# huggingface/open-muse

Hardware: AMD Instinct MI355X
Metric: images/sec/node (MaskGit train step, 256^2, bs=64/GPU) (higher is better)
Workload: dtype bf16 (transformer GEMM/attention operands; f32 accumulate, residual, norms, loss) + bf16x3 tokenizer (f32 activations, f32-class products as 3 bf16 MFMAs); parity of this mode was not measured in this run (a --full run measures it); 1 GPU; MaskGit train step: MaskGitVQGAN f16-256 encode (bf16x3) + cosine mask + MaskGitTransformer config B (configs/imagenet.yaml: hidden 768, 24 layers, 16 heads, vocab 2048, seq 257) fwd+bwd (bf16 MFMA, f32 accum/residual) + AdamW; global_batch=64, per_gpu_batch=64, resolution=256, seq_len=257, parallelism=dp1, vqgan_dtype=bf16x3, random_init=True, wgrad_stream=True

## Files before the change

include/muse_hip.h:

```cpp
#ifndef MUSE_HIP_H
#define MUSE_HIP_H
#include <stdint.h>

#ifdef __cplusplus
extern "C" {
#endif

enum { MUSE_F32 = 0, MUSE_BF16 = 1, MUSE_F16 = 2  };
enum { MUSE_ERR_BAD_ARG = -1, MUSE_ERR_ALIGN = -2, MUSE_ERR_UNSUPPORTED = -3 };

int muse_version(void);

typedef struct muse_gemm_desc {
  const void* A;
  const void* B;
  void* C;
  const void* bias;
  const void* rowvec;
  const void* residual;
  int32_t dtype;
  int32_t out_dtype;
  int32_t layout_a, layout_b;
  int32_t M, N, K;
  int32_t batch, zdiv;
// ... 44 lines not shown
  const void* v;
  void* o;
  int64_t ldq, ldk, ldv, ldo;
  int64_t bsq, bsk, bsv, bso;
  int32_t batch, heads, head_dim, seq_q, seq_kv;
  float alpha;
} muse_attn_desc;
int muse_attention_seq_pad(int32_t seq);
int muse_attention_fwd_ex(const muse_attn_desc* d, float* lse, void* stream);
int muse_attention_bwd_ex(const muse_attn_desc* d, const void* d_o, int64_t lddo, int64_t bsdo, const float* lse, float* dsum,
                          void* dq, int64_t lddq, int64_t bsdq, void* dk, int64_t lddk, int64_t bsdk, void* dv, int64_t lddv,
                          int64_t bsdv, void* stream);
int muse_attention_x3_fwd(const muse_attn_desc* d, float* lse, void* o_planes, int64_t o_lo, int32_t half, float scale, int32_t* stats,
                          void* stream);
int muse_attention_x3_bwd(const muse_attn_desc* d, const void* d_o, int64_t lddo, int64_t bsdo, const float* lse, void* dq,
                          int64_t lddq, int64_t bsdq, void* dk, int64_t lddk, int64_t bsdk, void* dv, int64_t lddv, int64_t bsdv,
                          void* dq_planes, int64_t dq_lo, void* dk_planes, int64_t dk_lo, void* dv_planes, int64_t dv_lo, int32_t half,
                          float scale, int32_t* stats, void* stream);
int muse_attention_x3_fwd_stream(const muse_attn_desc* d, float* lse, void* o_planes, int64_t o_lo, int32_t half, float scale,
                                 int32_t* stats, void* stream);
int muse_attention_x3_bwd_stream(const muse_attn_desc* d, const float* d_o, int64_t lddo, int64_t bsdo, const float* lse, float* dsum,
                                 float* dq, int64_t lddq, int64_t bsdq, float* dk, int64_t lddk, int64_t bsdk, float* dv, int64_t lddv,
                                 int64_t bsdv, void* dq_planes, int64_t dq_lo, void* dk_planes, int64_t dk_lo, void* dv_planes, int64_t dv_lo,
                                 int32_t half, float scale, int32_t* stats, void* stream);
int muse_attention_x3_merge(const float* part, int64_t part_stride, const float* lp, int64_t lp_stride, int32_t nk, float* out, float* lse,
                            void* out_planes, int64_t out_lo, int32_t batch, int32_t seq, int32_t heads, int32_t half, float scale,
                            int32_t* stats, void* stream);
int muse_sum_parts_strided(const float* parts, int64_t part_stride, int32_t n, int64_t rows, int32_t cols, float* out, int64_t ldo,
                           int32_t accumulate, void* stream);
int muse_attention_fwd(const void* qkv, void* ctx, float* lse, int32_t batch, int32_t seq, int32_t heads,
                       int32_t head_dim, float alpha, void* stream);
int muse_attention_bwd(const void* qkv, const void* ctx, const void* dctx, const float* lse, float* dsum, void* dqkv,
                       int32_t batch, int32_t seq, int32_t heads, int32_t head_dim, float alpha, void* stream);

int muse_glu_fwd(const void* ab, void* h, int32_t dtype, int64_t rows, int32_t inter, void* stream);
int muse_glu_bwd(const void* ab, const void* dh, void* dab, int32_t dtype, int64_t rows, int32_t inter, void* stream);
int muse_glu_fwd_x3(const float* ab, float* h, void* planes, int64_t rows, int32_t inter, int32_t half, float scale, int32_t* stats,
                    void* stream);
int muse_glu_bwd_x3(const float* ab, const float* dh, float* dab, void* planes, int64_t rows, int32_t inter, int32_t half, float scale,
                    int32_t* stats, void* stream);
int muse_ffn_mid_rows_per_block(void);
int muse_ffn_mid_fwd(const void* ab, const float* w, void* h, void* hm, float* mean, float* rstd, int32_t dtype,
                     int32_t rows, int32_t inter, float eps, void* stream);
int muse_ffn_mid_bwd(const void* dhm, const void* h, const void* ab, const float* w, const float* mean, const float* rstd,
                     void* dab, float* dw_partial, int32_t dtype, int32_t rows, int32_t inter, void* stream);
int muse_gelu_fwd(const void* x, void* y, int32_t dtype, int64_t n, void* stream);
int muse_gelu_bwd(const void* x, const void* dy, void* dx, int32_t dtype, int64_t n, void* stream);
int muse_gelu_bwd_f32_bf16(const float* x, const float* dy, void* dx_bf16, int64_t n, void* stream);

int muse_embed_fwd(const int64_t* ids, const float* word, const float* pos, float* out, int32_t batch, int32_t seq,
                   int32_t hidden, int32_t vocab, void* stream);
int muse_embed_bwd(const int64_t* ids, const float* dout, float* dword, float* dpos, float* scratch, int32_t batch,
                   int32_t seq, int32_t hidden, int32_t vocab, int32_t accumulate, void* stream);
int64_t muse_embed_bwd_scratch_floats(int32_t hidden, int32_t vocab);
int muse_embed_bwd2(const int64_t* ids, const float* dout, float* dword, float* dpos, void* scratch, int64_t scratch_bytes,
                    int32_t batch, int32_t seq, int32_t hidden, int32_t vocab, int32_t accumulate, void* stream);
int64_t muse_embed_bwd2_scratch_bytes(int32_t batch, int32_t seq, int32_t hidden, int32_t vocab);

int muse_cross_entropy_fwd(const void* logits, int32_t dtype, const int64_t* labels, float* row_loss, float* lse,
                           float* loss_out, int64_t rows, int32_t vocab, int64_t ld, float label_smoothing, void* stream);
int muse_cross_entropy_bwd(const void* logits, int32_t dtype, const int64_t* labels, const float* lse,
                           const float* loss_out, const float* grad_out, void* dlogits, int32_t dl_dtype, int64_t rows,
                           int32_t vocab, int64_t ld, float label_smoothing, void* stream);
int muse_soft_ce_fwd(const float* logits, const int64_t* labels, const float* soft, float* row_loss, float* lse, float* psum,
                     float* loss_out, int64_t rows, int32_t seq1, int32_t K, int64_t ld, void* stream);
int muse_soft_ce_bwd(const float* logits, const int64_t* labels, const float* soft, const float* lse, const float* psum,
                     const float* loss_out, const float* grad_out, void* dlogits, int32_t dl_dtype, int64_t rows, int32_t seq1,
                     int32_t K, int64_t ld, int64_t ldo, void* stream);

int muse_adamw_flat(float* p, const float* g, float* m, float* v, void* p_bf16, int64_t n, float lr, float beta1,
                    float beta2, float eps, float weight_decay, int32_t step, float grad_scale, const int32_t* skip, void* stream);
int muse_ema_multi(const int64_t* table, const int32_t* chunk_first, int32_t num_tensors, int32_t num_chunks, float one_minus_decay,
                   void* stream);
int muse_adamw_multi(const int64_t* table, const int32_t* chunk_first, int32_t num_tensors, int32_t num_chunks, float lr,
                     float beta1, float beta2, float eps, float weight_decay, int32_t step, float grad_scale, const int32_t* skip,
                     void* stream);
int muse_adamw_flat_groups(float* p, const float* g, float* m, float* v, void* p_bf16, int64_t n, int64_t base,
                           const int64_t* seg_end, const int32_t* seg_group, int32_t nseg, const float* group_hyper,
                           int32_t ngroups, int32_t step, float grad_scale, const int32_t* skip, void* stream);
int muse_adamw_multi_groups(const int64_t* table, const int32_t* chunk_first, int32_t num_tensors, int32_t num_chunks,
                            const float* group_hyper, int32_t ngroups, int32_t step, float grad_scale, const int32_t* skip, void* stream);

int muse_gradnorm_flat(const float* g_flat, int64_t base, int64_t n, const int64_t* ptab_host, const int32_t* chunk_first_host,
                       const int64_t* ptab, const int32_t* chunk_first, int32_t num_params, double* slab, void* stream);
int muse_gradnorm_multi(const int64_t* table, int32_t ncol, const int32_t* chunk_first, int32_t num_tensors, int32_t num_chunks,
                        double* slab, void* stream);
int muse_gradnorm_finalize(const double* slab, const int32_t* chunk_first, int32_t num_tensors, double* psum, float grad_scale,
                           float max_norm, float* out, void* stream);
int muse_grad_scale_flat(float* g, int64_t n, const float* scale, void* stream);
int muse_grad_scale_multi(const int64_t* table, int32_t ncol, const int32_t* chunk_first, int32_t num_tensors, int32_t num_chunks,
                          const float* scale, void* stream);
int muse_adamw_flat_dev(float* p, const float* g, float* m, float* v, void* p_bf16, int64_t n, float lr, float beta1, float beta2,
                        float eps, float weight_decay, int32_t step, const float* scale_dev, const int32_t* skip, void* stream);
int muse_adamw_multi_dev(const int64_t* table, const int32_t* chunk_first, int32_t num_tensors, int32_t num_chunks, float lr,
                         float beta1, float beta2, float eps, float weight_decay, int32_t step, const float* scale_dev,
                         const int32_t* skip, void* stream);
int muse_adamw_flat_groups_dev(float* p, const float* g, float* m, float* v, void* p_bf16, int64_t n, int64_t base,
                               const int64_t* seg_end, const int32_t* seg_group, int32_t nseg, const float* group_hyper,
                               int32_t ngroups, int32_t step, const float* scale_dev, const int32_t* skip, void* stream);
int muse_adamw_multi_groups_dev(const int64_t* table, const int32_t* chunk_first, int32_t num_tensors, int32_t num_chunks,
                                const float* group_hyper, int32_t ngroups, int32_t step, const float* scale_dev, const int32_t* skip,
                                void* stream);
int muse_sum_slices(const float* ws, float* out, int32_t nslices, int64_t n, int64_t stride, int32_t accumulate, void* stream);
int muse_sum_multi(const void* const* ws, void* const* out, const int32_t* nslices, const int64_t* n, const int64_t* stride,
                   const int32_t* accumulate, const int32_t* kind, int32_t njobs, void* stream);
int muse_split_f32_to_bf16x2(const float* in, void* hi, void* lo, int64_t n, void* stream);
int muse_sum_slices_epilogue(const float* ws, int32_t nslices, int64_t stride, const float* bias, const void* residual, int64_t ldr,
                             void* out, int32_t out_dtype, int64_t ldc, int64_t rows, int32_t cols, void* stream);
int muse_split_f32_to_bf16_cat3(const float* in, void* out, int64_t rows, int32_t cols, int64_t ld_in, int64_t ld_out, int32_t mode,
                                int32_t lo_pos, void* stream);
int muse_cast_f32_to_bf16(const float* in, void* out, int64_t n, void* stream);
int muse_cast_f32_to_f16(const float* in, void* out, int64_t n, float scale, int32_t* stats, void* stream);
int muse_cast_bf16_to_f32(const void* in, float* out, int64_t n, void* stream);

int muse_mask_sample(const int64_t* tokens, const int64_t* class_ids, const float* timesteps, const float* noise,
                     int64_t* input_ids, int64_t* labels, float* mask_prob, int32_t batch, int32_t seq, int64_t mask_id,
                     int64_t codebook_size, float min_masking_rate, void* stream);

int muse_sample_step(const float* cond_logits, const float* uncond_logits, float guidance_scale, int64_t img_stride, int64_t ld,
                     int32_t vocab,
                     const int64_t* input_ids, int64_t mask_id, const float* noise_exp, const float* noise_u, uint64_t seed,
                     uint32_t step, float temperature, int32_t sched_mask_len, int32_t batch, int32_t seq, int64_t* raw_sampled,
                     int64_t* sampled, int64_t* next_ids, float* conf_scratch, void* stream);

int muse_mask_tokens(const int64_t* tokens, const float* timesteps, const float* mask_prob_in, const float* noise,
                     const int32_t* rects, int64_t* input_ids, int64_t* labels, float* loss_weight, float* mask_prob,
                     int32_t batch, int32_t seq, int64_t mask_id, float min_masking_rate, int32_t all_labels, float weight_min,
                     void* stream);

int muse_dropout(const void* x, void* y, int32_t dtype, int64_t n, float p, uint64_t seed, uint64_t offset, void* stream);

int muse_cond_dropout(const float* x, const float* empty, const float* uniforms, float* out, int32_t batch, int64_t per_image,
                      float prob, void* stream);


int muse_conv2d_nhwc(const void* in, const void* weight, const float* bias, const void* residual, void* out,
                     int32_t dtype, int32_t batch, int32_t H, int32_t W, int32_t Cin, int32_t Cout, int32_t KS,
                     int32_t upsample, void* stream);
int muse_conv2d_nhwc_split(const float* in, const void* w_hi, const void* w_lo, const float* bias, const float* residual,
                           float* out, double* gn_partial, int32_t gn_groups, int32_t batch, int32_t H, int32_t W,
                           int32_t Cin, int32_t Cout, int32_t KS, int32_t upsample, void* stream);
int muse_conv2d_nhwc_split2(const void* in_hi, const void* in_lo, const void* w_hi, const void* w_lo, const float* bias,
                            const float* residual, float* out, double* gn_partial, int32_t gn_groups, int32_t batch,
                            int32_t H, int32_t W, int32_t Cin, int32_t Cout, int32_t KS, void* stream);
int muse_groupnorm_silu_nhwc(const void* x, void* y, int32_t dtype, const float* gamma, const float* beta,
                             double* partial, int32_t batch, int32_t HW, int32_t C, int32_t groups, float eps,
                             int32_t apply_silu, void* stream);
int muse_groupnorm_nchunk(int32_t HW);
int muse_conv2d_nhwc_gn_split2_ok(int32_t batch, int32_t H, int32_t W, int32_t Cin, int32_t Cout, int32_t KS);
int muse_conv2d_nhwc_gn_split2(const float* x, const float* gn_scale, const float* gn_shift, const void* w_hi, const void* w_lo,
                               const float* bias, const float* residual, float* out, double* gn_partial, int32_t gn_groups,
                               int32_t batch, int32_t H, int32_t W, int32_t Cin, int32_t Cout, int32_t KS, int32_t persistent,
                               void* stream);
int muse_groupnorm_scale_shift(const double* partial, int32_t nchunk, const float* gamma, const float* beta, float* scale,
                               float* shift, int32_t batch, int32_t HW, int32_t C, int32_t groups, float eps, void* stream);
int muse_conv_in_direct(const float* x, const float* w4, const float* bias, float* out, double* gn_partial, int32_t gn_groups,
                        int32_t batch, int32_t H, int32_t W, int32_t Cin, int32_t Cpad, int32_t Cout, void* stream);
int muse_conv_out_direct(const float* x, const float* scale, const float* shift, const float* w, const float* bias, float* out,
                         int32_t batch, int32_t H, int32_t W, int32_t C, int32_t Cout, void* stream);
int muse_upsample2x_nhwc(const void* x, void* y, int32_t dtype, int32_t batch, int32_t H, int32_t W, int32_t C, void* stream);
int muse_upsample2x_split_nhwc(const float* x, void* y_hi, void* y_lo, int32_t batch, int32_t H, int32_t W, int32_t C, void* stream);
int muse_groupnorm_silu_nhwc_split(const float* x, void* y_hi, void* y_lo, const float* gamma, const float* beta,
                                   double* partial, int32_t stats_nchunk, int32_t batch, int32_t HW, int32_t C,
                                   int32_t groups, float eps, int32_t apply_silu, void* stream);
int muse_avgpool2x2_nhwc(const void* x, void* y, int32_t dtype, int32_t batch, int32_t H, int32_t W, int32_t C,
                         void* stream);
int muse_avgpool2x2_nhwc_stats(const float* x, float* y, double* partial, int32_t groups, int32_t batch, int32_t H, int32_t W,
                               int32_t C, void* stream);
int muse_nchw_to_nhwc(const float* in, void* out, int32_t out_dtype, int32_t batch, int32_t C, int32_t HW, int32_t Cpad,
                      void* stream);
int muse_nhwc_to_nchw(const void* in, int32_t in_dtype, float* out, int32_t batch, int32_t C, int32_t HW, int32_t Cpad,
                      void* stream);
int muse_argmin_rows(const float* dist, int64_t* idx, int64_t rows, int32_t ncodes, int64_t ld, void* stream);
int muse_row_sumsq(const float* x, float* out, int64_t rows, int32_t cols, int64_t ld, void* stream);
int muse_gather_rows(const float* table, const int64_t* idx, void* out, int32_t out_dtype, int64_t rows, int32_t cols,
                     void* stream);

int muse_probe_tr16(const int32_t* addr, int32_t* out, void* stream);

int muse_norm_res_fwd(const float* x, const float* res, const float* w, float* y, float* pre, int64_t rows, int32_t cols,
                      float eps, int32_t mode, void* stream);
int muse_adaln_fwd(const float* x, const float* ss, float* y, int32_t batch, int64_t rows_per_batch, int32_t C, void* stream);
int muse_adaln_fwd_ex(const float* x, const float* ss, float* y, void* y_bf16, int32_t batch, int64_t rows_per_batch, int32_t C,
                      void* stream);
int muse_silu_fwd(const float* x, float* y, int64_t n, void* stream);
int muse_dwconv3x3_nhwc(const float* x, const float* w, float* y, int32_t batch, int32_t H, int32_t W, int32_t C, void* stream);
int muse_space_to_depth2_nhwc(const float* x, float* y, int32_t batch, int32_t H, int32_t W, int32_t C, int32_t inverse, void* stream);
int muse_grn_fwd(const float* x, const float* gamma, const float* beta, float* y, float* scratch, int32_t batch, int64_t S,
                 int32_t C, void* stream);
int muse_grn_fwd_ex(const float* x, const float* gamma, const float* beta, float* y, void* y_bf16, float* scratch, int32_t batch,
                    int64_t S, int32_t C, void* stream);
int muse_sinusoidal_encode(const float* f, float* out, int64_t n, int32_t dim, float max_positions, void* stream);
int muse_weighted_mean(const float* v, const float* w, float* out, int64_t n, void* stream);
int muse_norm_res_bwd_nblk(int64_t rows);
int muse_norm_res_bwd(const float* dy, const float* dpre, const float* v, const float* w, float* dv, float* dw_partial,
                      int64_t rows, int32_t cols, float eps, int32_t mode, void* stream);
int muse_norm_res_bwd_ex(const float* dy, const float* dpre, const float* v, const float* w, float* dv, void* dv_bf16,
                         float* dw_partial, int64_t rows, int32_t cols, float eps, int32_t mode, void* stream);
int muse_norm_adaln_fwd(const float* x, const float* res, const float* w, const float* ss, float* pre, float* m, void* m_bf16,
                        int32_t batch, int64_t rows_per_batch, int32_t cols, float eps, int32_t mode, void* stream);
int muse_norm_adaln_bwd(const float* dm, const float* dpre, const float* v, const float* w, const float* ss, float* dv, void* dv_bf16,
                        float* dw_partial, float* dss_partial, int32_t batch, int64_t rows_per_batch, int32_t cols, float eps,
                        int32_t mode, void* stream);
int muse_norm_adaln_fwd_x3(const float* x, const float* res, const float* w, const float* ss, float* pre, float* m, void* planes,
                           int32_t batch, int64_t rows_per_batch, int32_t cols, float eps, int32_t mode, int32_t half, float scale,
                           int32_t* stats, void* stream);
int muse_norm_adaln_bwd_x3(const float* dm, const float* dpre, const float* v, const float* w, const float* ss, float* dv, void* planes,
                           float* dw_partial, float* dss_partial, int32_t batch, int64_t rows_per_batch, int32_t cols, float eps,
                           int32_t mode, int32_t half, float scale, int32_t* stats, void* stream);
int muse_colsum_segments(const float* part, float* out, int32_t nseg, int32_t seg_rows, int32_t cols, void* stream);
int muse_adaln_bwd(const float* dy, const float* x, const float* ss, float* dx, float* dss, int32_t batch,
                   int64_t rows_per_batch, int32_t C, void* stream);
int muse_silu_bwd(const float* x, const float* dy, float* dx, int64_t n, void* stream);
int muse_dwconv3x3_bwd_nchunk(int64_t pixels);
int muse_dwconv3x3_bwd(const float* dy, const float* x, const float* w, float* dx, float* dw_partial, int32_t batch, int32_t H,
                       int32_t W, int32_t C, void* stream);
int muse_grn_bwd(const float* dy, const float* x, const float* gamma, const float* stats, float* dx, float* work,
                 int32_t batch, int64_t S, int32_t C, void* stream);
int muse_scale_rows(float* x, const float* w, const float* num, const float* den, int64_t rows, int32_t cols, int64_t ld,
                    void* stream);

#ifdef __cplusplus
}
#endif
#endif
```

open-muse_amd/csrc/conv_dma.hip:

```cpp
#include "gemm256.h"
#include "../../include/muse_hip.h"

namespace cdma {
using g256::lds_read128;
using g256::lds_void_t;

constexpr int BM = 256, BN = 128, BK = 32, NT = 512, MI = 4, NI = 4, NSTAGE = 3;
constexpr int AH = 0, AL = 16384, BH = 32768, BL = 40960, STAGE = 49152, LDS_BYTES = NSTAGE * STAGE;

struct Params {
  const bf16_t *xh, *xl, *wh, *wl;
  const float* bias;
  const float* residual;
  float* out;
  double* gn_partial;
  int gn_cpg, gn_groups;
  int M, N, K, H, W, Cin;
  const float *xf, *gsc, *gsh;
};

__device__ __forceinline__ int sw4(int q) { return (4 - q) & 3; }

struct Frag16 { bf16x8 ah[MI], al[MI], bh[NI], bl[NI]; };

// ... 100 lines not shown
#endif
#ifndef CDMA_ABLATE_NO_DMA
#define CDMA_ISSUE(S, Q)                             \
  if constexpr ((Q) == 0) issue_a((S) * STAGE, 0);   \
  if constexpr ((Q) == 1) issue_a((S) * STAGE, 1);   \
  if constexpr ((Q) == 2) issue_b((S) * STAGE);
#define CDMA_TOP_WAIT "s_waitcnt vmcnt(6) lgkmcnt(0)"
#else
#define CDMA_ISSUE(S, Q)
#define CDMA_TOP_WAIT "s_waitcnt vmcnt(0) lgkmcnt(0)"
#endif
#define CDMA_SLOT(CUR, NXT, S, SN, Q)                          \
  CDMA_PAIR(CUR, Q)                                            \
  __builtin_amdgcn_sched_barrier(0);                           \
  CDMA_ISSUE(S, Q)                                             \
  CDMA_READ(NXT, SN, Q)                                        \
  __builtin_amdgcn_sched_barrier(0);
#define CDMA_TILE(CUR, NXT, S, SN)                                                     \
  asm volatile(CDMA_TOP_WAIT ::: "memory");                                            \
  __builtin_amdgcn_s_barrier();                                                        \
  __builtin_amdgcn_sched_barrier(0);                                                   \
  CDMA_SLOT(CUR, NXT, S, SN, 0) CDMA_SLOT(CUR, NXT, S, SN, 1) CDMA_SLOT(CUR, NXT, S, SN, 2) CDMA_SLOT(CUR, NXT, S, SN, 3)     \
  CDMA_SLOT(CUR, NXT, S, SN, 4) CDMA_SLOT(CUR, NXT, S, SN, 5) CDMA_SLOT(CUR, NXT, S, SN, 6) CDMA_SLOT(CUR, NXT, S, SN, 7)     \
  CDMA_SLOT(CUR, NXT, S, SN, 8) CDMA_SLOT(CUR, NXT, S, SN, 9) CDMA_SLOT(CUR, NXT, S, SN, 10) CDMA_SLOT(CUR, NXT, S, SN, 11)   \
  CDMA_SLOT(CUR, NXT, S, SN, 12) CDMA_SLOT(CUR, NXT, S, SN, 13) CDMA_SLOT(CUR, NXT, S, SN, 14) CDMA_SLOT(CUR, NXT, S, SN, 15)

  issue_a(0 * STAGE, 0); issue_a(0 * STAGE, 1); issue_b(0 * STAGE);
  issue_a(1 * STAGE, 0); issue_a(1 * STAGE, 1); issue_b(1 * STAGE);
  issue_a(2 * STAGE, 0); issue_a(2 * STAGE, 1); issue_b(2 * STAGE);
  asm volatile("s_waitcnt vmcnt(12)" ::: "memory");
  __builtin_amdgcn_s_barrier();
  __builtin_amdgcn_sched_barrier(0);
  CDMA_READ(f0, 0, 0) CDMA_READ(f0, 0, 1) CDMA_READ(f0, 0, 2) CDMA_READ(f0, 0, 3)
  CDMA_READ(f0, 0, 4) CDMA_READ(f0, 0, 5) CDMA_READ(f0, 0, 6) CDMA_READ(f0, 0, 7)
  CDMA_READ(f0, 0, 8) CDMA_READ(f0, 0, 9) CDMA_READ(f0, 0, 10) CDMA_READ(f0, 0, 11)
  CDMA_READ(f0, 0, 12) CDMA_READ(f0, 0, 13) CDMA_READ(f0, 0, 14) CDMA_READ(f0, 0, 15)
  __builtin_amdgcn_sched_barrier(0);

  const int nkt = (p.K + BK - 1) / BK, ngroups = (nkt + 5) / 6;
  for (int grp = 0; grp < ngroups; ++grp) {
    CDMA_TILE(f0, f1, 0, 1)
    CDMA_TILE(f1, f0, 1, 2)
    CDMA_TILE(f0, f1, 2, 0)
    CDMA_TILE(f1, f0, 0, 1)
    CDMA_TILE(f0, f1, 1, 2)
    CDMA_TILE(f1, f0, 2, 0)
  }
#undef CDMA_TILE
#undef CDMA_ISSUE
#undef CDMA_TOP_WAIT
#undef CDMA_SLOT
#undef CDMA_PAIR
#undef CDMA_READ
  asm volatile("s_waitcnt vmcnt(0) lgkmcnt(0)" ::: "memory");
  __builtin_amdgcn_sched_barrier(0);

  constexpr int CST = BN * 4 + 16;
  float bias_v[NI][4];
#pragma unroll
  for (int j = 0; j < NI; ++j)
#pragma unroll
    for (int r = 0; r < 4; ++r) {
      const int n = n0 + wn * 64 + j * 16 + 4 * (lane >> 4) + r;
      bias_v[j][r] = (p.bias && n < p.N) ? p.bias[n] : 0.f;
    }
  double gs = 0.0, gq = 0.0;
  __syncthreads();
#pragma unroll
  for (int i = 0; i < MI; ++i) {
    const int lr = wm * 64 + i * 16 + (lane & 15);
#pragma unroll
    for (int j = 0; j < NI; ++j) {
      const int nl = wn * 64 + j * 16 + 4 * (lane >> 4);
      const f32x4 v = {acc[i][j][0] + bias_v[j][0], acc[i][j][1] + bias_v[j][1], acc[i][j][2] + bias_v[j][2], acc[i][j][3] + bias_v[j][3]};
      *(f32x4*)(smem + lr * CST + nl * 4) = v;
    }
  }
  __syncthreads();
  constexpr int NIT = (BM * 32) / NT;
  const int col = (threadIdx.x & 31) * 4, n = n0 + col, rbase = threadIdx.x >> 5;
  if (n < p.N) {
    f32x4 rv[NIT];
    if (p.residual) {
#pragma unroll
      for (int it = 0; it < NIT; ++it) {
        const int m = m0 + rbase + 16 * it;
        rv[it] = m < p.M ? *(const f32x4*)(p.residual + (long)m * p.N + n) : f32x4{0.f, 0.f, 0.f, 0.f};
      }
    }
#pragma unroll
    for (int it = 0; it < NIT; ++it) {
      const int row = rbase + 16 * it, m = m0 + row;
      if (m < p.M) {
        f32x4 w = *(const f32x4*)(smem + row * CST + col * 4);
        if (p.residual) w += rv[it];
        *(f32x4*)(p.out + (long)m * p.N + n) = w;
        if (p.gn_partial) {
#pragma unroll
          for (int e = 0; e < 4; ++e) { gs += (double)w[e]; gq += (double)w[e] * (double)w[e]; }
        }
      }
    }
  }
  if (p.gn_partial) {
    gs += __shfl_xor(gs, 32, 64);
    gq += __shfl_xor(gq, 32, 64);
    __syncthreads();
    double* red = (double*)smem;
    if (lane < 32) { red[(wave * 32 + lane) * 2] = gs; red[(wave * 32 + lane) * 2 + 1] = gq; }
    __syncthreads();
    if (threadIdx.x < 32) {
      double cs = 0.0, cq = 0.0;
#pragma unroll
      for (int w8 = 0; w8 < 8; ++w8) { cs += red[(w8 * 32 + threadIdx.x) * 2]; cq += red[(w8 * 32 + threadIdx.x) * 2 + 1]; }
      const int cpc = p.gn_cpg >> 2;
      for (int o = 1; o < cpc; o <<= 1) { cs += __shfl_xor(cs, o, 64); cq += __shfl_xor(cq, o, 64); }
      const int n = n0 + (int)threadIdx.x * 4;
      if ((threadIdx.x & (cpc - 1)) == 0 && n < p.N) {
        const int hw = p.H * p.W, b = m0 / hw, chunk = (m0 - b * hw) >> 8, nchunk = hw >> 8;
        double* o2 = p.gn_partial + (((long)b * nchunk + chunk) * p.gn_groups + n / p.gn_cpg) * 2;
        o2[0] = cs; o2[1] = cq;
      }
    }
  }
}

}


namespace cslab {
using g256::lds_read128;
using g256::lds_void_t;
using cdma::Params;
using cdma::sw4;

constexpr int BM = 256, BN = 128, NT = 512, MI = 4, NI = 4;
constexpr int PLANE = 21 * 1024;
constexpr int SLAB = 2 * PLANE;
constexpr int B_BASE = 2 * SLAB, BSTAGE = 16384;
constexpr int CST = BN * 4 + 16;
constexpr int LDS_BYTES = BM * CST;
static_assert(B_BASE + 3 * BSTAGE <= LDS_BYTES, "LDS map");

struct Frag16 { bf16x8 ah[MI], al[MI], bh[NI], bl[NI]; };

#ifdef CDMA_TIMESTAMPS
__device__ long* g_conv_ts = nullptr;
#define CDMA_TS(IDX) if (g_conv_ts && threadIdx.x == 0) g_conv_ts[(long)blockIdx.x * 8 + (IDX)] = (long)__builtin_amdgcn_s_memtime();
#define CDMA_TSV(V, IDX) if (g_conv_ts && threadIdx.x == 0) g_conv_ts[(long)(V) * 8 + (IDX)] = (long)__builtin_amdgcn_s_memtime();
#else
#define CDMA_TS(IDX)
#define CDMA_TSV(V, IDX)
#endif
template <bool GN>
__global__ __launch_bounds__(512, 2) void conv_slab_kernel(Params p) {
  extern __shared__ __attribute__((aligned(16))) unsigned char smem[];
  CDMA_TS(0)
  const int H = p.H, W = p.W, Cin = p.Cin;
  const int tpr = W >> 4, tpi = (H >> 4) * tpr;
  const int ntm = p.M >> 8, ntn = (p.N + BN - 1) / BN, ntiles = ntm * ntn;
  const int bq = ntiles >> 3, br = ntiles & 7, xcd = blockIdx.x & 7, bi = blockIdx.x >> 3;
  const int tid_ = (xcd < br ? xcd * (bq + 1) : br * (bq + 1) + (xcd - br) * bq) + bi;
  const int mt = tid_ / ntn, n0 = (tid_ % ntn) * BN;
  const int img = mt / tpi, prem = mt - img * tpi, ty = prem / tpr, tx = prem - ty * tpr;
  const int y0 = ty << 4, x0 = tx << 4;

  const int lane = threadIdx.x & 63, wave = __builtin_amdgcn_readfirstlane(threadIdx.x >> 6);
  const int wm = wave >> 1, wn = wave & 1;

  constexpr int XE = GN ? 4 : 2;
  const unsigned bytesA = (unsigned)((long)p.M * Cin * XE);
  const rsrc_t rs_xh = make_rsrc(GN ? (const void*)p.xf : (const void*)p.xh, bytesA), rs_xl = make_rsrc(GN ? (const void*)p.xf : (const void*)p.xl, bytesA);
  const unsigned oobA = (bytesA + 15u) & ~15u;
  unsigned slab_off[3];
  int slab_piece[3];
  const int srcchunk = (lane & 3) ^ (((lane >> 4) & 1) << 1);
  {
#pragma unroll
    for (int k = 0; k < 3; ++k) {
      int piece = wave + 8 * k;
      if (piece > 20) piece -= 8;
      slab_piece[k] = piece;
      const int r = piece * 16 + (lane >> 2), sy = r / 18, sx = r - sy * 18;
      const int y = y0 - 1 + sy, x = x0 - 1 + sx;
      const bool ok = r < 324 && y >= 0 && y < H && x >= 0 && x < W;
      slab_off[k] = ok ? (unsigned)(((((long)img * H + y) * W + x) * Cin + srcchunk * 8) * XE) : oobA;
    }
  }
  float* const gss = (float*)(smem + LDS_BYTES);
  if constexpr (GN) {
    for (int c = threadIdx.x; c < Cin; c += NT) { gss[c] = p.gsc[(long)img * Cin + c]; gss[Cin + c] = p.gsh[(long)img * Cin + c]; }
    __syncthreads();
  }
  u32x4 xr[2];
  float scv[4], shv[4];
  auto issue_slab_f = [&](u32x4 (&r)[2], int k, int chunk) {
    const unsigned vo = chunk * 32 < Cin ? slab_off[k] : oobA;
    r[0] = buf_load16(rs_xh, vo, (unsigned)(chunk * 128));
    r[1] = buf_load16(rs_xh, vo + 16u, (unsigned)(chunk * 128));
  };
  auto load_gss = [&](int chunk, int h) {
    const float* q = gss + chunk * 32 + srcchunk * 8 + h * 4;
#pragma unroll
#ifndef GNX_CONST_SS
    for (int j = 0; j < 4; ++j) { scv[j] = q[j]; shv[j] = q[Cin + j]; }
#else
    for (int j = 0; j < 4; ++j) { scv[j] = 1.25f; shv[j] = 0.125f; }
    (void)q;
#endif
  };
  auto xform_elem = [&](u32x4 (&r)[2], int e) {
    float t = fmaf(__uint_as_float(r[e >> 2][e & 3]), scv[e & 3], shv[e & 3]);
#ifndef GNX_NO_SILU
    t = gn_silu(t);
#endif
    asm volatile("" : "+v"(t));
    r[e >> 2][e & 3] = __float_as_uint(t);
  };
  auto store_slab_f = [&](u32x4 (&r)[2], int buf, int k) {
    u32x4 hi4, lo4;
#pragma unroll
    for (int h = 0; h < 2; ++h) {
      u32x2 hi, lo;
      split4(r[h], hi, lo);
      hi4[2 * h] = hi[0]; hi4[2 * h + 1] = hi[1];
      lo4[2 * h] = lo[0]; lo4[2 * h + 1] = lo[1];
    }
    if (slab_off[k] == oobA) { hi4 = u32x4{0u, 0u, 0u, 0u}; lo4 = hi4; }
    unsigned char* dst = smem + buf * SLAB + slab_piece[k] * 1024 + lane * 16;
    *(u32x4*)dst = hi4;
    *(u32x4*)(dst + PLANE) = lo4;
  };

  auto issue_slab = [&](int buf, int k, int chunk) {
    const unsigned vo = chunk * 32 < Cin ? slab_off[k] : oobA;
    const int soff = chunk * 64;
    unsigned char* dst = smem + buf * SLAB + slab_piece[k] * 1024;
    __builtin_amdgcn_raw_ptr_buffer_load_lds(rs_xh, (lds_void_t*)dst, 16, (int)vo, soff, 0, 0);
    __builtin_amdgcn_raw_ptr_buffer_load_lds(rs_xl, (lds_void_t*)(dst + PLANE), 16, (int)vo, soff, 0, 0);
  };

  const int wimg = wave >> 2;
  const unsigned bytesB = (unsigned)((long)p.N * p.K * 2);
  const rsrc_t rs_w = make_rsrc(wimg ? p.wl : p.wh, bytesB);
  const unsigned oobB = (bytesB + 15u) & ~15u;
  unsigned voffB[2];
  {
    const int srcchunk = (lane & 3) ^ sw4((lane >> 4) & 3);
#pragma unroll
    for (int j = 0; j < 2; ++j) {
      const int n = n0 + ((wave & 3) * 2 + j) * 16 + (lane >> 2);
      voffB[j] = n < p.N ? (unsigned)(((long)n * p.K + srcchunk * 8) * 2) : oobB;
    }
  }
  auto issue_b = [&](int stage, int chunk, int tap) {
    const bool ok = chunk * 32 < Cin;
    const int soff = (tap * Cin + chunk * 32) * 2;
#pragma unroll
    for (int j = 0; j < 2; ++j)
      __builtin_amdgcn_raw_ptr_buffer_load_lds(rs_w, (lds_void_t*)(smem + B_BASE + stage * BSTAGE + wimg * 8192 + ((wave & 3) * 2 + j) * 1024),
                                               16, (int)(ok ? voffB[j] : oobB), soff, 0, 0);
  };

  unsigned baseA[4][2], addrB;
  {
    const int pr = lane & 15, g = lane >> 4, P = 72 * wm + pr;
#pragma unroll
    for (int e = 0; e < 4; ++e)
#pragma unroll
      for (int b = 0; b < 2; ++b) {
        const int bit2 = ((P >> 2) & 1) ^ (((P & 3) + e) >> 2) ^ b;
        baseA[e][b] = (unsigned)((P << 6) | ((g << 4) ^ (bit2 << 5)));
      }
    addrB = (unsigned)(B_BASE + (wn * 64 + pr) * 64 + ((g ^ sw4((pr >> 2) & 3)) << 4));
  }

  auto flip_base = [&](int d) {
#pragma unroll
    for (int e = 0; e < 4; ++e) { baseA[e][0] += d; baseA[e][1] += d; }
  };

  f32x4 acc[MI][NI];
#pragma unroll
  for (int i = 0; i < MI; ++i)
#pragma unroll
    for (int j = 0; j < NI; ++j) acc[i][j] = f32x4{0.f, 0.f, 0.f, 0.f};
  Frag16 f0, f1;

#define SLAB_CP(TAP, I) (((I) + (TAP) / 3) * 18 + (TAP) % 3)
#define SLAB_READ(F, ST, TAP, Q)                                                                                             \
  {                                                                                                                               \
    constexpr int q_ = (Q) & 3;                                                                                                   \
    constexpr int cp_ = SLAB_CP(TAP, q_);                                                                                         \
    if constexpr ((Q) < 4) lds_read128<cp_ * 64>(F.ah[q_], baseA[cp_ & 3][(cp_ >> 2) & 1]);                                       \
    else if constexpr ((Q) < 8) lds_read128<PLANE + cp_ * 64>(F.al[q_], baseA[cp_ & 3][(cp_ >> 2) & 1]);                          \
    else if constexpr ((Q) < 12) lds_read128<(ST) * BSTAGE + q_ * 1024>(F.bh[q_], addrB);                                         \
    else lds_read128<(ST) * BSTAGE + 8192 + q_ * 1024>(F.bl[q_], addrB);                                                          \
  }
#if defined(CDMA_TWO_PRODUCTS)
#define SLAB_PAIR(F, Q)                                                                                                        \
  {                                                                                                                            \
    constexpr int i_ = (Q) >> 2, j_ = (Q) & 3;                                                                                 \
    if constexpr (CDMA_TWO_PRODUCTS == 1) acc[i_][j_] = __builtin_amdgcn_mfma_f32_16x16x32_bf16(F.bh[j_], F.al[i_], acc[i_][j_], 0, 0, 0);   \
    else acc[i_][j_] = __builtin_amdgcn_mfma_f32_16x16x32_bf16(F.bl[j_], F.ah[i_], acc[i_][j_], 0, 0, 0);                        \
    acc[i_][j_] = __builtin_amdgcn_mfma_f32_16x16x32_bf16(F.bh[j_], F.ah[i_], acc[i_][j_], 0, 0, 0);                            \
  }
#elif !defined(CDMA_ABLATE_NO_MFMA)
#define SLAB_PAIR(F, Q)                                                                                                        \
  {                                                                                                                            \
    constexpr int i_ = (Q) >> 2, j_ = (Q) & 3;                                                                                 \
    acc[i_][j_] = __builtin_amdgcn_mfma_f32_16x16x32_bf16(F.bl[j_], F.ah[i_], acc[i_][j_], 0, 0, 0);                            \
    acc[i_][j_] = __builtin_amdgcn_mfma_f32_16x16x32_bf16(F.bh[j_], F.al[i_], acc[i_][j_], 0, 0, 0);                            \
    acc[i_][j_] = __builtin_amdgcn_mfma_f32_16x16x32_bf16(F.bh[j_], F.ah[i_], acc[i_][j_], 0, 0, 0);                            \
  }
#else
#define SLAB_PAIR(F, Q) asm volatile("" ::"v"(F.ah[(Q) >> 2]), "v"(F.al[(Q) >> 2]), "v"(F.bh[(Q) & 3]), "v"(F.bl[(Q) & 3]));
#endif
#ifndef CDMA_ABLATE_NO_DMA
#define SLAB_ISSUE(T, Q)                                                                          \
  if constexpr (!GN && (Q) == 0 && ((T) % 9) < 3) issue_slab(1 - (T) / 9, (T) % 9, chunk0 + (T) / 9 + 1);  \
  if constexpr (GN && (Q) == 0 && ((T) % 9) == 0) issue_slab_f(xr, 0, chunk0 + (T) / 9 + 1);           \
  if constexpr (GN && (Q) == 12 && (((T) % 9) == 2 || ((T) % 9) == 4)) issue_slab_f(xr, ((T) % 9) / 2, chunk0 + (T) / 9 + 1);  \
  if constexpr ((Q) == 2) issue_b(((T) + 3) % 3, chunk0 + ((T) + 3) / 9, ((T) + 3) % 9);
#define SLAB_XF(T, Q)                                                                             \
  if constexpr (GN && ((T) % 9) >= 2 && ((T) % 9) <= 6 && ((T) % 9) % 2 == 0) {                    \
    constexpr int k_ = ((T) % 9) / 2 - 1;                                                         \
    if constexpr ((Q) == 1) load_gss(chunk0 + (T) / 9 + 1, 0);                                    \
    if constexpr ((Q) >= 2 && (Q) < 6) xform_elem(xr, (Q) - 2);                                   \
    if constexpr ((Q) == 6) load_gss(chunk0 + (T) / 9 + 1, 1);                                    \
    if constexpr ((Q) >= 7 && (Q) < 11) xform_elem(xr, (Q) - 3);                                  \
    if constexpr ((Q) == 11) store_slab_f(xr, 1 - (T) / 9, k_);                                   \
  }
#else
#define SLAB_ISSUE(T, Q)
#define SLAB_XF(T, Q)
#endif
#define SLAB_SLOT(CUR, NXT, T, Q)                                                   \
  SLAB_PAIR(CUR, Q)                                                                 \
  __builtin_amdgcn_sched_barrier(0);                                                \
  SLAB_ISSUE(T, Q)                                                                  \
  SLAB_READ(NXT, (((T) + 1) % 3), (((T) + 1) % 9), Q)                               \
  SLAB_XF(T, Q)                                                                     \
  __builtin_amdgcn_sched_barrier(0);
#ifndef CDMA_ABLATE_NO_DMA
#define SLAB_WAIT(T)                                                                     \
  if constexpr (GN ? (((T) % 9) == 1 || (((T) % 9) >= 3 && ((T) % 9) <= 6)) : (((T) % 9) >= 1 && ((T) % 9) <= 3))  \
    asm volatile("s_waitcnt vmcnt(4) lgkmcnt(0)" ::: "memory");                          \
  else asm volatile("s_waitcnt vmcnt(2) lgkmcnt(0)" ::: "memory");
#else
#define SLAB_WAIT(T) asm volatile("s_waitcnt vmcnt(0) lgkmcnt(0)" ::: "memory");
#endif
#define SLAB_TAP(CUR, NXT, T)                                                                         \
  SLAB_WAIT(T)                                                                                        \
  __builtin_amdgcn_s_barrier();                                                                       \
  if constexpr ((T) == 8) flip_base(SLAB);                                                            \
  if constexpr ((T) == 17) flip_base(-SLAB);                                                          \
  __builtin_amdgcn_sched_barrier(0);                                                                  \
  SLAB_SLOT(CUR, NXT, T, 0) SLAB_SLOT(CUR, NXT, T, 1) SLAB_SLOT(CUR, NXT, T, 2) SLAB_SLOT(CUR, NXT, T, 3)     \
  SLAB_SLOT(CUR, NXT, T, 4) SLAB_SLOT(CUR, NXT, T, 5) SLAB_SLOT(CUR, NXT, T, 6) SLAB_SLOT(CUR, NXT, T, 7)     \
  SLAB_SLOT(CUR, NXT, T, 8) SLAB_SLOT(CUR, NXT, T, 9) SLAB_SLOT(CUR, NXT, T, 10) SLAB_SLOT(CUR, NXT, T, 11)   \
  SLAB_SLOT(CUR, NXT, T, 12) SLAB_SLOT(CUR, NXT, T, 13) SLAB_SLOT(CUR, NXT, T, 14) SLAB_SLOT(CUR, NXT, T, 15)

  int chunk0 = 0;
  u32x4 pr[GN ? 3 : 1][2];
  if constexpr (GN) { issue_slab_f(pr[0], 0, 0); issue_slab_f(pr[GN ? 1 : 0], 1, 0); issue_slab_f(pr[GN ? 2 : 0], 2, 0); }
  else { issue_slab(0, 0, 0); issue_slab(0, 1, 0); issue_slab(0, 2, 0); }
  issue_b(0, 0, 0); issue_b(1, 0, 1); issue_b(2, 0, 2);
  CDMA_TS(1)
  if constexpr (GN) {
#pragma unroll
    for (int h = 0; h < 2; ++h) {
      load_gss(0, h);
#pragma unroll
      for (int k = 0; k < 3; ++k)
#pragma unroll
        for (int e = 0; e < 4; ++e) xform_elem(pr[GN ? k : 0], h * 4 + e);
    }
#pragma unroll
    for (int k = 0; k < 3; ++k) store_slab_f(pr[GN ? k : 0], 0, k);
  }
  asm volatile("s_waitcnt vmcnt(4) lgkmcnt(0)" ::: "memory");
  __builtin_amdgcn_s_barrier();
  __builtin_amdgcn_sched_barrier(0);
  CDMA_TS(2)
  SLAB_READ(f0, 0, 0, 0) SLAB_READ(f0, 0, 0, 1) SLAB_READ(f0, 0, 0, 2) SLAB_READ(f0, 0, 0, 3)
  SLAB_READ(f0, 0, 0, 4) SLAB_READ(f0, 0, 0, 5) SLAB_READ(f0, 0, 0, 6) SLAB_READ(f0, 0, 0, 7)
  SLAB_READ(f0, 0, 0, 8) SLAB_READ(f0, 0, 0, 9) SLAB_READ(f0, 0, 0, 10) SLAB_READ(f0, 0, 0, 11)
  SLAB_READ(f0, 0, 0, 12) SLAB_READ(f0, 0, 0, 13) SLAB_READ(f0, 0, 0, 14) SLAB_READ(f0, 0, 0, 15)
  __builtin_amdgcn_sched_barrier(0);

  const int nchunks = Cin >> 5;
  for (; chunk0 < nchunks; chunk0 += 2) {
    SLAB_TAP(f0, f1, 0) SLAB_TAP(f1, f0, 1) SLAB_TAP(f0, f1, 2) SLAB_TAP(f1, f0, 3) SLAB_TAP(f0, f1, 4) SLAB_TAP(f1, f0, 5)
    SLAB_TAP(f0, f1, 6) SLAB_TAP(f1, f0, 7) SLAB_TAP(f0, f1, 8) SLAB_TAP(f1, f0, 9) SLAB_TAP(f0, f1, 10) SLAB_TAP(f1, f0, 11)
    SLAB_TAP(f0, f1, 12) SLAB_TAP(f1, f0, 13) SLAB_TAP(f0, f1, 14) SLAB_TAP(f1, f0, 15) SLAB_TAP(f0, f1, 16) SLAB_TAP(f1, f0, 17)
  }
#undef SLAB_TAP
#undef SLAB_WAIT
#undef SLAB_SLOT
#undef SLAB_XF
#undef SLAB_ISSUE
#undef SLAB_PAIR
#undef SLAB_READ
#undef SLAB_CP
  asm volatile("s_waitcnt vmcnt(0) lgkmcnt(0)" ::: "memory");
  __builtin_amdgcn_sched_barrier(0);
  CDMA_TS(3)

  float bias_v[NI][4];
#pragma unroll
  for (int j = 0; j < NI; ++j)
#pragma unroll
    for (int r = 0; r < 4; ++r) {
      const int n = n0 + wn * 64 + j * 16 + 4 * (lane >> 4) + r;
      bias_v[j][r] = (p.bias && n < p.N) ? p.bias[n] : 0.f;
    }
  double gs = 0.0, gq = 0.0;
  __syncthreads();
#pragma unroll
  for (int i = 0; i < MI; ++i) {
    const int lr = wm * 64 + i * 16 + (lane & 15);
#pragma unroll
    for (int j = 0; j < NI; ++j) {
      const int nl = wn * 64 + j * 16 + 4 * (lane >> 4);
      const f32x4 v = {acc[i][j][0] + bias_v[j][0], acc[i][j][1] + bias_v[j][1], acc[i][j][2] + bias_v[j][2], acc[i][j][3] + bias_v[j][3]};
      *(f32x4*)(smem + lr * CST + nl * 4) = v;
    }
  }
  __syncthreads();
  CDMA_TS(4)
  constexpr int NIT = (BM * 32) / NT;
  const int col = (threadIdx.x & 31) * 4, n = n0 + col, rbase = threadIdx.x >> 5;
  const long pix0 = ((long)img * H + y0) * W + x0 + rbase;
  if (n < p.N) {
    f32x4 rv[NIT];
    if (p.residual) {
#pragma unroll
      for (int it = 0; it < NIT; ++it) rv[it] = *(const f32x4*)(p.residual + (pix0 + (long)it * W) * p.N + n);
    }
#pragma unroll
    for (int it = 0; it < NIT; ++it) {
      f32x4 w = *(const f32x4*)(smem + (rbase + 16 * it) * CST + col * 4);
      if (p.residual) w += rv[it];
#ifndef CDMA_ABLATE_NO_STORE
      *(f32x4*)(p.out + (pix0 + (long)it * W) * p.N + n) = w;
#else
      if (w[0] == 123.456f) p.out[0] = w[1];
#endif
      if (p.gn_partial) {
#pragma unroll
        for (int e = 0; e < 4; ++e) { gs += (double)w[e]; gq += (double)w[e] * (double)w[e]; }
      }
    }
  }
  if (p.gn_partial) {
    gs += __shfl_xor(gs, 32, 64);
    gq += __shfl_xor(gq, 32, 64);
    __syncthreads();
    double* red = (double*)smem;
    if (lane < 32) { red[(wave * 32 + lane) * 2] = gs; red[(wave * 32 + lane) * 2 + 1] = gq; }
    __syncthreads();
    if (threadIdx.x < 32) {
      double cs = 0.0, cq = 0.0;
#pragma unroll
      for (int w8 = 0; w8 < 8; ++w8) { cs += red[(w8 * 32 + threadIdx.x) * 2]; cq += red[(w8 * 32 + threadIdx.x) * 2 + 1]; }
      const int cpc = p.gn_cpg >> 2;
      for (int o = 1; o < cpc; o <<= 1) { cs += __shfl_xor(cs, o, 64); cq += __shfl_xor(cq, o, 64); }
      const int nn = n0 + (int)threadIdx.x * 4;
      if ((threadIdx.x & (cpc - 1)) == 0 && nn < p.N) {
        double* o2 = p.gn_partial + (((long)img * tpi + prem) * p.gn_groups + nn / p.gn_cpg) * 2;
        o2[0] = cs; o2[1] = cq;
      }
    }
  }
  CDMA_TS(5)
}


constexpr int P_BUF1 = 92160, P_BBASE = 43008, P_STAGING = P_BUF1, P_HALF_ROWS = 128;
constexpr int P_LDS_BYTES = P_STAGING + P_HALF_ROWS * CST;
constexpr int P_GSS = P_LDS_BYTES, P_GSS_MAX_CIN = 256, P_LDS_BYTES_GN = P_LDS_BYTES + 2 * 2 * P_GSS_MAX_CIN * 4;
__host__ __device__ constexpr int p_stage_off(int st) { return st == 0 ? 32768 : (st - 1) * 16384; }
static_assert(P_BBASE + 3 * BSTAGE == P_BUF1 && P_BUF1 + SLAB <= P_LDS_BYTES && P_LDS_BYTES_GN <= 163840, "LDS map");

template <bool GN>
__global__ __launch_bounds__(512, 2) void conv_slab_persist_kernel(Params p) {
  extern __shared__ __attribute__((aligned(16))) unsigned char smem[];
  const int H = p.H, W = p.W, Cin = p.Cin;
  const int tpr = W >> 4, tpi = (H >> 4) * tpr;
  const int ntm = p.M >> 8, ntn = (p.N + BN - 1) / BN, ntiles = ntm * ntn;
  const int bq = ntiles >> 3, br = ntiles & 7;
  const int nblocks = gridDim.x;

  const int lane = threadIdx.x & 63, wave = __builtin_amdgcn_readfirstlane(threadIdx.x >> 6);
  const int wm = wave >> 1, wn = wave & 1;

  constexpr int XE = GN ? 4 : 2;
  const unsigned bytesA = (unsigned)((long)p.M * Cin * XE);
  const rsrc_t rs_xh = make_rsrc(GN ? (const void*)p.xf : (const void*)p.xh, bytesA), rs_xl = make_rsrc(GN ? (const void*)p.xf : (const void*)p.xl, bytesA);
  const unsigned oobA = (bytesA + 15u) & ~15u;
  const int wimg = wave >> 2;
  const unsigned bytesB = (unsigned)((long)p.N * p.K * 2);
  const rsrc_t rs_w = make_rsrc(wimg ? p.wl : p.wh, bytesB);
  const unsigned oobB = (bytesB + 15u) & ~15u;
  const int nchunks = Cin >> 5;
  const unsigned bytesO = (unsigned)((long)p.M * p.N * 4);
  const rsrc_t rs_out = make_rsrc(p.out, bytesO), rs_res = make_rsrc(p.residual ? (const void*)p.residual : (const void*)p.out, bytesO);

  int slab_piece[3];
#pragma unroll
  for (int k = 0; k < 3; ++k) { int piece = wave + 8 * k; if (piece > 20) piece -= 8; slab_piece[k] = piece; }
  const int srcchunkA = (lane & 3) ^ (((lane >> 4) & 1) << 1);

  struct Geo { int img, prem, y0, x0, n0; };
  auto geo_of = [&](int v) {
    const int xcd = v & 7, bi = v >> 3;
    const int tid_ = (xcd < br ? xcd * (bq + 1) : br * (bq + 1) + (xcd - br) * bq) + bi;
    const int mt = tid_ / ntn;
    Geo g;
    g.n0 = (tid_ - mt * ntn) * BN;
    g.img = mt / tpi; g.prem = mt - g.img * tpi;
    const int ty = g.prem / tpr, tx = g.prem - ty * tpr;
    g.y0 = ty << 4; g.x0 = tx << 4;
    return g;
  };
  auto offsets_of = [&](const Geo& g, bool valid, unsigned (&so)[3], unsigned (&vb)[2], int ln) {
    const int srcchunkA = (ln & 3) ^ (((ln >> 4) & 1) << 1);
    const int srcchunkB = (ln & 3) ^ sw4((ln >> 4) & 3);
#pragma unroll
    for (int k = 0; k < 3; ++k) {
      const int r = slab_piece[k] * 16 + (ln >> 2), sy = r / 18, sx = r - sy * 18;
      const int y = g.y0 - 1 + sy, x = g.x0 - 1 + sx;
      const bool ok = valid && r < 324 && y >= 0 && y < H && x >= 0 && x < W;
      so[k] = ok ? (unsigned)(((((long)g.img * H + y) * W + x) * Cin + srcchunkA * 8) * XE) : oobA;
    }
#pragma unroll
    for (int j = 0; j < 2; ++j) {
      const int n = g.n0 + ((wave & 3) * 2 + j) * 16 + (ln >> 2);
      vb[j] = (valid && n < p.N) ? (unsigned)(((long)n * p.K + srcchunkB * 8) * 2) : oobB;
    }
  };

  unsigned slab_off[3], voffB[2], slab_off_n[3], voffB_n[2];
  auto issue_slab = [&](int buf, int k, int chunk) {
    const bool cur = chunk < nchunks;
    const unsigned vo = cur ? slab_off[k] : slab_off_n[k];
    const int soff = cur ? chunk * 64 : 0;
    unsigned char* dst = smem + (buf ? P_BUF1 : 0) + slab_piece[k] * 1024;
    __builtin_amdgcn_raw_ptr_buffer_load_lds(rs_xh, (lds_void_t*)dst, 16, (int)vo, soff, 0, 0);
    __builtin_amdgcn_raw_ptr_buffer_load_lds(rs_xl, (lds_void_t*)(dst + PLANE), 16, (int)vo, soff, 0, 0);
  };
  auto issue_b = [&](int stage_off, int chunk, int tap) {
    const bool cur = chunk < nchunks;
    const int soff = (tap * Cin + (cur ? chunk * 32 : 0)) * 2;
#pragma unroll
    for (int j = 0; j < 2; ++j)
      __builtin_amdgcn_raw_ptr_buffer_load_lds(rs_w, (lds_void_t*)(smem + P_BBASE + stage_off + wimg * 8192 + ((wave & 3) * 2 + j) * 1024),
                                               16, (int)(cur ? voffB[j] : voffB_n[j]), soff, 0, 0);
  };

  float* gss_cur = (float*)(smem + P_GSS);
  float* gss_nxt = gss_cur + 2 * P_GSS_MAX_CIN;
  u32x4 xr[2];
  float scv[4], shv[4];
  auto issue_slab_f = [&](u32x4 (&r)[2], int k, int chunk) {
    const bool cur = chunk < nchunks;
    const unsigned vo = cur ? slab_off[k] : slab_off_n[k];
    const unsigned soff = cur ? (unsigned)(chunk * 128) : 0u;
    r[0] = buf_load16(rs_xh, vo, soff);
    r[1] = buf_load16(rs_xh, vo + 16u, soff);
  };
  auto load_gss = [&](int chunk, int h) {
    const float* q = (chunk < nchunks ? gss_cur + chunk * 32 : gss_nxt) + srcchunkA * 8 + h * 4;
#pragma unroll
    for (int j = 0; j < 4; ++j) { scv[j] = q[j]; shv[j] = q[Cin + j]; }
  };
  auto xform_elem = [&](u32x4 (&r)[2], int e) {
    float t = fmaf(__uint_as_float(r[e >> 2][e & 3]), scv[e & 3], shv[e & 3]);
    t = gn_silu(t);
    asm volatile("" : "+v"(t));
    r[e >> 2][e & 3] = __float_as_uint(t);
  };
  auto store_slab_f = [&](u32x4 (&r)[2], int buf, int k, int chunk) {
    u32x4 hi4, lo4;
#pragma unroll
    for (int h = 0; h < 2; ++h) {
      u32x2 hi, lo;
      split4(r[h], hi, lo);
      hi4[2 * h] = hi[0]; hi4[2 * h + 1] = hi[1];
      lo4[2 * h] = lo[0]; lo4[2 * h + 1] = lo[1];
    }
    if ((chunk < nchunks ? slab_off[k] : slab_off_n[k]) == oobA) { hi4 = u32x4{0u, 0u, 0u, 0u}; lo4 = hi4; }
    unsigned char* dst = smem + (buf ? P_BUF1 : 0) + slab_piece[k] * 1024 + lane * 16;
    *(u32x4*)dst = hi4;
    *(u32x4*)(dst + PLANE) = lo4;
  };
  auto issue_gss = [&](float* dst, int img) {
    const int npc = Cin >> 6, piece = wave % (2 * npc), isshift = piece >= npc ? 1 : 0, pc = piece - isshift * npc;
    const int batch = p.M / (H * W);
    const rsrc_t rs = make_rsrc(isshift ? p.gsh : p.gsc, (unsigned)((long)batch * Cin * 4));
    __builtin_amdgcn_raw_ptr_buffer_load_lds(rs, (lds_void_t*)(dst + isshift * Cin + pc * 64), 4, (int)((unsigned)((long)img * Cin + pc * 64 + lane) * 4u), 0, 0, 0);
  };

  unsigned baseA[4][2], addrB;
  {
    const int pr = lane & 15, g = lane >> 4, P = 72 * wm + pr;
#pragma unroll
    for (int e = 0; e < 4; ++e)
#pragma unroll
      for (int b = 0; b < 2; ++b) {
        const int bit2 = ((P >> 2) & 1) ^ (((P & 3) + e) >> 2) ^ b;
        baseA[e][b] = (unsigned)((P << 6) | ((g << 4) ^ (bit2 << 5)));
      }
    addrB = (unsigned)(P_BBASE + (wn * 64 + pr) * 64 + ((g ^ sw4((pr >> 2) & 3)) << 4));
  }
  auto flip_base = [&](int d) {
#pragma unroll
    for (int e = 0; e < 4; ++e) { baseA[e][0] += d; baseA[e][1] += d; }
  };

  auto lds_barrier = [&]() {
    asm volatile("s_waitcnt lgkmcnt(0)" ::: "memory");
    __builtin_amdgcn_s_barrier();
    __builtin_amdgcn_sched_barrier(0);
  };

  f32x4 acc[MI][NI];
  Frag16 f0, f1;

#define SLAB_CP(TAP, I) (((I) + (TAP) / 3) * 18 + (TAP) % 3)
#define SLAB_READ(F, ST, TAP, Q)                                                                                                  \
  {                                                                                                                               \
    constexpr int q_ = (Q) & 3;                                                                                                   \
    constexpr int cp_ = SLAB_CP(TAP, q_);                                                                                         \
    if constexpr ((Q) < 4) lds_read128<cp_ * 64>(F.ah[q_], baseA[cp_ & 3][(cp_ >> 2) & 1]);                                       \
    else if constexpr ((Q) < 8) lds_read128<PLANE + cp_ * 64>(F.al[q_], baseA[cp_ & 3][(cp_ >> 2) & 1]);                          \
    else if constexpr ((Q) < 12) lds_read128<p_stage_off(ST) + q_ * 1024>(F.bh[q_], addrB);                                       \
    else lds_read128<p_stage_off(ST) + 8192 + q_ * 1024>(F.bl[q_], addrB);                                                        \
  }
#define SLAB_PAIR(F, Q)                                                                                                        \
  {                                                                                                                            \
    constexpr int i_ = (Q) >> 2, j_ = (Q) & 3;                                                                                 \
    acc[i_][j_] = __builtin_amdgcn_mfma_f32_16x16x32_bf16(F.bl[j_], F.ah[i_], acc[i_][j_], 0, 0, 0);                            \
    acc[i_][j_] = __builtin_amdgcn_mfma_f32_16x16x32_bf16(F.bh[j_], F.al[i_], acc[i_][j_], 0, 0, 0);                            \
    acc[i_][j_] = __builtin_amdgcn_mfma_f32_16x16x32_bf16(F.bh[j_], F.ah[i_], acc[i_][j_], 0, 0, 0);                            \
  }
#define SLAB_ISSUE(T, Q)                                                                          \
  if constexpr (!GN && (Q) == 0 && ((T) % 9) < 3) issue_slab(1 - (T) / 9, (T) % 9, chunk0 + (T) / 9 + 1);  \
  if constexpr (GN && (Q) == 0 && ((T) % 9) == 0) issue_slab_f(xr, 0, chunk0 + (T) / 9 + 1);           \
  if constexpr (GN && (Q) == 12 && (((T) % 9) == 2 || ((T) % 9) == 4)) issue_slab_f(xr, ((T) % 9) / 2, chunk0 + (T) / 9 + 1);  \
  if constexpr (GN && (T) == 3 && (Q) == 5) { if (first) issue_gss(gss_nxt, gn.img); }               \
  if constexpr ((Q) == 2) issue_b(p_stage_off(((T) + 3) % 3), chunk0 + ((T) + 3) / 9, ((T) + 3) % 9);
#define SLAB_XF(T, Q)                                                                             \
  if constexpr (GN && ((T) % 9) >= 2 && ((T) % 9) <= 6 && ((T) % 9) % 2 == 0) {                    \
    constexpr int k_ = ((T) % 9) / 2 - 1;                                                         \
    if constexpr ((Q) == 1) load_gss(chunk0 + (T) / 9 + 1, 0);                                    \
    if constexpr ((Q) >= 2 && (Q) < 6) xform_elem(xr, (Q) - 2);                                   \
    if constexpr ((Q) == 6) load_gss(chunk0 + (T) / 9 + 1, 1);                                    \
    if constexpr ((Q) >= 7 && (Q) < 11) xform_elem(xr, (Q) - 3);                                  \
    if constexpr ((Q) == 11) store_slab_f(xr, 1 - (T) / 9, k_, chunk0 + (T) / 9 + 1);             \
  }
#define SLAB_SLOT(CUR, NXT, T, Q)                                                   \
  SLAB_PAIR(CUR, Q)                                                                 \
  __builtin_amdgcn_sched_barrier(0);                                                \
  SLAB_ISSUE(T, Q)                                                                  \
  SLAB_READ(NXT, (((T) + 1) % 3), (((T) + 1) % 9), Q)                               \
  SLAB_XF(T, Q)                                                                     \
  __builtin_amdgcn_sched_barrier(0);
#define SLAB_WAIT(T)                                                                                                        \
  if constexpr ((T) < 2) {                                                                                                  \
    if (first) asm volatile("s_waitcnt lgkmcnt(0)" ::: "memory");                                                          \
    else if constexpr ((T) == 1) asm volatile("s_waitcnt vmcnt(4) lgkmcnt(0)" ::: "memory");                               \
    else asm volatile("s_waitcnt vmcnt(2) lgkmcnt(0)" ::: "memory");                                                        \
  } else if constexpr (GN ? (((T) % 9) == 1 || (((T) % 9) >= 3 && ((T) % 9) <= 6)) : (((T) % 9) >= 1 && ((T) % 9) <= 3))   \
    asm volatile("s_waitcnt vmcnt(4) lgkmcnt(0)" ::: "memory");                                                             \
  else asm volatile("s_waitcnt vmcnt(2) lgkmcnt(0)" ::: "memory");
#define SLAB_TAP(CUR, NXT, T)                                                                         \
  SLAB_WAIT(T)                                                                                        \
  __builtin_amdgcn_s_barrier();                                                                       \
  if constexpr ((T) == 8) flip_base(P_BUF1);                                                          \
  if constexpr ((T) == 17) flip_base(-P_BUF1);                                                        \
  __builtin_amdgcn_sched_barrier(0);                                                                  \
  SLAB_SLOT(CUR, NXT, T, 0) SLAB_SLOT(CUR, NXT, T, 1) SLAB_SLOT(CUR, NXT, T, 2) SLAB_SLOT(CUR, NXT, T, 3)     \
  SLAB_SLOT(CUR, NXT, T, 4) SLAB_SLOT(CUR, NXT, T, 5) SLAB_SLOT(CUR, NXT, T, 6) SLAB_SLOT(CUR, NXT, T, 7)     \
  SLAB_SLOT(CUR, NXT, T, 8) SLAB_SLOT(CUR, NXT, T, 9) SLAB_SLOT(CUR, NXT, T, 10) SLAB_SLOT(CUR, NXT, T, 11)   \
  SLAB_SLOT(CUR, NXT, T, 12) SLAB_SLOT(CUR, NXT, T, 13) SLAB_SLOT(CUR, NXT, T, 14) SLAB_SLOT(CUR, NXT, T, 15)

  int v = blockIdx.x;
  Geo g = geo_of(v);
  offsets_of(g, true, slab_off_n, voffB_n, lane);
  if constexpr (GN) {
    for (int c = threadIdx.x; c < Cin; c += NT) { gss_nxt[c] = p.gsc[(long)g.img * Cin + c]; gss_nxt[Cin + c] = p.gsh[(long)g.img * Cin + c]; }
    u32x4 pr[3][2];
    issue_slab_f(pr[0], 0, nchunks); issue_slab_f(pr[1], 1, nchunks); issue_slab_f(pr[2], 2, nchunks);
    issue_b(p_stage_off(0), nchunks, 0); issue_b(p_stage_off(1), nchunks, 1); issue_b(p_stage_off(2), nchunks, 2);
    __syncthreads();
#pragma unroll
    for (int h = 0; h < 2; ++h) {
      load_gss(nchunks, h);
#pragma unroll
      for (int k = 0; k < 3; ++k)
#pragma unroll
        for (int e = 0; e < 4; ++e) xform_elem(pr[k], h * 4 + e);
    }
#pragma unroll
    for (int k = 0; k < 3; ++k) store_slab_f(pr[k], 0, k, nchunks);
  } else {
    issue_slab(0, 0, nchunks); issue_slab(0, 1, nchunks); issue_slab(0, 2, nchunks);
    issue_b(p_stage_off(0), nchunks, 0); issue_b(p_stage_off(1), nchunks, 1); issue_b(p_stage_off(2), nchunks, 2);
  }
  asm volatile("s_waitcnt vmcnt(0) lgkmcnt(0)" ::: "memory");
  __builtin_amdgcn_s_barrier();
  __builtin_amdgcn_sched_barrier(0);
  SLAB_READ(f0, 0, 0, 0) SLAB_READ(f0, 0, 0, 1) SLAB_READ(f0, 0, 0, 2) SLAB_READ(f0, 0, 0, 3)
  SLAB_READ(f0, 0, 0, 4) SLAB_READ(f0, 0, 0, 5) SLAB_READ(f0, 0, 0, 6) SLAB_READ(f0, 0, 0, 7)
  SLAB_READ(f0, 0, 0, 8) SLAB_READ(f0, 0, 0, 9) SLAB_READ(f0, 0, 0, 10) SLAB_READ(f0, 0, 0, 11)
  SLAB_READ(f0, 0, 0, 12) SLAB_READ(f0, 0, 0, 13) SLAB_READ(f0, 0, 0, 14) SLAB_READ(f0, 0, 0, 15)
  __builtin_amdgcn_sched_barrier(0);

  for (;;) {
#pragma unroll
    for (int k = 0; k < 3; ++k) slab_off[k] = slab_off_n[k];
    voffB[0] = voffB_n[0]; voffB[1] = voffB_n[1];
    if constexpr (GN) { float* t = gss_cur; gss_cur = gss_nxt; gss_nxt = t; }
    const int vn = v + nblocks;
    const bool has_next = vn < ntiles;
    const Geo gn = geo_of(has_next ? vn : v);
    {
      int ln = lane;
      asm volatile("" : "+v"(ln));
      offsets_of(gn, has_next, slab_off_n, voffB_n, ln);
    }
#pragma unroll
    for (int i = 0; i < MI; ++i)
#pragma unroll
      for (int j = 0; j < NI; ++j) acc[i][j] = f32x4{0.f, 0.f, 0.f, 0.f};

    CDMA_TSV(v, 0)
    bool first = true;
    for (int chunk0 = 0; chunk0 < nchunks; chunk0 += 2) {
      SLAB_TAP(f0, f1, 0) SLAB_TAP(f1, f0, 1) SLAB_TAP(f0, f1, 2) SLAB_TAP(f1, f0, 3) SLAB_TAP(f0, f1, 4) SLAB_TAP(f1, f0, 5)
      SLAB_TAP(f0, f1, 6) SLAB_TAP(f1, f0, 7) SLAB_TAP(f0, f1, 8) SLAB_TAP(f1, f0, 9) SLAB_TAP(f0, f1, 10) SLAB_TAP(f1, f0, 11)
      SLAB_TAP(f0, f1, 12) SLAB_TAP(f1, f0, 13) SLAB_TAP(f0, f1, 14) SLAB_TAP(f1, f0, 15) SLAB_TAP(f0, f1, 16) SLAB_TAP(f1, f0, 17)
      first = false;
    }

    CDMA_TSV(v, 1)
    const int n0 = g.n0;
    constexpr int NITH = (P_HALF_ROWS * 32) / NT;
    int tx = threadIdx.x;
    asm volatile("" : "+v"(tx));
    const int lane_e = tx & 63;
    const int col = (tx & 31) * 4, n = n0 + col, rbase = tx >> 5;
    const long pixp = ((long)g.img * H + g.y0) * W + g.x0;
    const unsigned obase = (unsigned)(((pixp + rbase) * p.N + n) * 4);
    const unsigned rowstep = (unsigned)((long)W * p.N * 4);
    asm volatile("s_waitcnt vmcnt(0) lgkmcnt(0)" ::: "memory");
    __builtin_amdgcn_sched_barrier(0);
    CDMA_TSV(v, 2)
    {
      const int nf = n0 + wn * 64 + 4 * (lane_e >> 4);
      f32x4 bj[NI];
#pragma unroll
      for (int j = 0; j < NI; ++j)
        bj[j] = (p.bias && (nf + j * 16) < p.N) ? *(const f32x4*)(p.bias + nf + j * 16) : f32x4{0.f, 0.f, 0.f, 0.f};
      if (p.residual) {
        const unsigned fbase = (unsigned)((((pixp + (long)(wm * 4) * W + (lane_e & 15)) * p.N) + nf) * 4);
        u32x4 rr[2][NI];
#pragma unroll
        for (int j = 0; j < NI; ++j)
          rr[0][j] = (nf + j * 16) < p.N ? __builtin_amdgcn_raw_buffer_load_b128(rs_res, (int)(fbase + j * 64), 0, 0) : u32x4{0u, 0u, 0u, 0u};
#pragma unroll
        for (int i = 0; i < MI; ++i) {
          if (i + 1 < MI) {
#pragma unroll
            for (int j = 0; j < NI; ++j)
              rr[(i + 1) & 1][j] = (nf + j * 16) < p.N ? __builtin_amdgcn_raw_buffer_load_b128(rs_res, (int)(fbase + j * 64), (int)(rowstep * (i + 1)), 0)
                                                       : u32x4{0u, 0u, 0u, 0u};
          }
#pragma unroll
          for (int j = 0; j < NI; ++j) acc[i][j] = (acc[i][j] + bj[j]) + __builtin_bit_cast(f32x4, rr[i & 1][j]);
        }
      } else {
#pragma unroll
        for (int i = 0; i < MI; ++i)
#pragma unroll
          for (int j = 0; j < NI; ++j) acc[i][j] += bj[j];
      }
    }
    __builtin_amdgcn_s_waitcnt(0x0F70);
    __builtin_amdgcn_sched_barrier(0);
    CDMA_TSV(v, 3)
    double gs = 0.0, gq = 0.0;
#pragma unroll
    for (int half = 0; half < 2; ++half) {
      lds_barrier();
      if ((wm >> 1) == half) {
#pragma unroll
        for (int i = 0; i < MI; ++i) {
          const int lr = (wm & 1) * 64 + i * 16 + (lane_e & 15);
#pragma unroll
          for (int j = 0; j < NI; ++j) {
            const int nl = wn * 64 + j * 16 + 4 * (lane_e >> 4);
            *(f32x4*)(smem + P_STAGING + lr * CST + nl * 4) = acc[i][j];
          }
        }
      }
      lds_barrier();
      if (n < p.N) {
#pragma unroll
        for (int it = 0; it < NITH; ++it) {
          const f32x4 w = *(const f32x4*)(smem + P_STAGING + (rbase + 16 * it) * CST + col * 4);
          __builtin_amdgcn_raw_buffer_store_b128(__builtin_bit_cast(u32x4, w), rs_out, (int)obase, (int)(rowstep * (half * NITH + it)), 0);
          if (p.gn_partial) {
#pragma unroll
            for (int e = 0; e < 4; ++e) { gs += (double)w[e]; gq += (double)w[e] * (double)w[e]; }
          }
        }
      }
    }
    CDMA_TSV(v, 4)
    if (p.gn_partial) {
      gs += __shfl_xor(gs, 32, 64);
      gq += __shfl_xor(gq, 32, 64);
      lds_barrier();
      double* red = (double*)(smem + P_STAGING);
      if (lane_e < 32) { red[(wave * 32 + lane_e) * 2] = gs; red[(wave * 32 + lane_e) * 2 + 1] = gq; }
      lds_barrier();
      if (tx < 32) {
        double cs = 0.0, cq = 0.0;
#pragma unroll
        for (int w8 = 0; w8 < 8; ++w8) { cs += red[(w8 * 32 + tx) * 2]; cq += red[(w8 * 32 + tx) * 2 + 1]; }
        const int cpc = p.gn_cpg >> 2;
        for (int o = 1; o < cpc; o <<= 1) { cs += __shfl_xor(cs, o, 64); cq += __shfl_xor(cq, o, 64); }
        const int nn = n0 + tx * 4;
        if ((tx & (cpc - 1)) == 0 && nn < p.N) {
          double* o2 = p.gn_partial + (((long)g.img * tpi + g.prem) * p.gn_groups + (nn >> __builtin_ctz(p.gn_cpg))) * 2;
          o2[0] = cs; o2[1] = cq;
        }
      }
    }
    CDMA_TSV(v, 5)
    if (!has_next) break;
    v = vn; g = gn;
    asm volatile("s_waitcnt lgkmcnt(0)" ::: "memory");
    __builtin_amdgcn_sched_barrier(0);
    SLAB_READ(f0, 0, 0, 0) SLAB_READ(f0, 0, 0, 1) SLAB_READ(f0, 0, 0, 2) SLAB_READ(f0, 0, 0, 3)
    SLAB_READ(f0, 0, 0, 4) SLAB_READ(f0, 0, 0, 5) SLAB_READ(f0, 0, 0, 6) SLAB_READ(f0, 0, 0, 7)
    SLAB_READ(f0, 0, 0, 8) SLAB_READ(f0, 0, 0, 9) SLAB_READ(f0, 0, 0, 10) SLAB_READ(f0, 0, 0, 11)
    SLAB_READ(f0, 0, 0, 12) SLAB_READ(f0, 0, 0, 13) SLAB_READ(f0, 0, 0, 14) SLAB_READ(f0, 0, 0, 15)
    __builtin_amdgcn_sched_barrier(0);
  }
#undef SLAB_TAP
#undef SLAB_WAIT
#undef SLAB_SLOT
#undef SLAB_XF
#undef SLAB_ISSUE
#undef SLAB_PAIR
#undef SLAB_READ
#undef SLAB_CP
}

}

#ifdef CDMA_TIMESTAMPS
extern "C" int muse_debug_conv_ts(long* buf) { return (int)hipMemcpyToSymbol(HIP_SYMBOL(cslab::g_conv_ts), &buf, sizeof(buf)); }
#endif
extern "C" int muse_conv2d_nhwc_split2(const void* in_hi, const void* in_lo, const void* w_hi, const void* w_lo, const float* bias,
                                       const float* residual, float* out, double* gn_partial, int32_t gn_groups, int32_t batch,
                                       int32_t H, int32_t W, int32_t Cin, int32_t Cout, int32_t KS, void* stream) {
  if (KS != 3) return MUSE_ERR_UNSUPPORTED;
  if ((Cin % 32) || (Cout % 4)) return MUSE_ERR_ALIGN;
  if ((((uintptr_t)in_hi) | ((uintptr_t)in_lo) | ((uintptr_t)w_hi) | ((uintptr_t)w_lo) | ((uintptr_t)out) | ((uintptr_t)residual)) & 15)
    return MUSE_ERR_ALIGN;
  const long M = (long)batch * H * W;
  if (M <= 0 || Cout <= 0) return 0;
  if (M * Cin * 2 >= (1L << 32) - 64 || (long)Cout * 9 * Cin * 2 >= (1L << 32) - 64 || M >= (1L << 31) - 256) return MUSE_ERR_UNSUPPORTED;
  cdma::Params p;
  p.xh = (const bf16_t*)in_hi; p.xl = (const bf16_t*)in_lo; p.wh = (const bf16_t*)w_hi; p.wl = (const bf16_t*)w_lo;
  p.bias = bias; p.residual = residual; p.out = out;
  p.gn_partial = gn_partial; p.gn_groups = gn_groups; p.gn_cpg = gn_groups > 0 ? Cout / gn_groups : 0;
  if (gn_partial) {
    const int cpg = p.gn_cpg;
    if (gn_groups <= 0 || (Cout % gn_groups) || ((H * W) % 256) || cpg < 4 || cpg > 128 || (cpg & (cpg - 1))) return MUSE_ERR_UNSUPPORTED;
  }
  p.M = (int)M; p.N = Cout; p.K = 9 * Cin; p.H = H; p.W = W; p.Cin = Cin;
  const int ntm = (p.M + cdma::BM - 1) / cdma::BM, ntn = (p.N + cdma::BN - 1) / cdma::BN;
  static const int use_slab = []() { const char* e = getenv("MUSE_CONV_SLAB"); return e ? atoi(e) : 1; }();
  if (use_slab && (H % 16) == 0 && (W % 16) == 0 && (Cin % 64) == 0) {
    set_max_dynamic_lds((const void*)cslab::conv_slab_kernel<false>, cslab::LDS_BYTES);
    const int nslab = (p.M >> 8) * ntn;
    if (use_slab >= 2 && (long)p.M * p.N * 4 < (1L << 32) - 64) {
      const int ncu = device_cus();
      if (!ncu) return MUSE_ERR_UNSUPPORTED;
      set_max_dynamic_lds((const void*)cslab::conv_slab_persist_kernel<false>, cslab::P_LDS_BYTES);
      hipLaunchKernelGGL(cslab::conv_slab_persist_kernel<false>, dim3(nslab < ncu ? nslab : ncu), dim3(512), cslab::P_LDS_BYTES, (hipStream_t)stream, p);
      return (int)hipGetLastError();
    }
    hipLaunchKernelGGL(cslab::conv_slab_kernel<false>, dim3(nslab), dim3(512), cslab::LDS_BYTES, (hipStream_t)stream, p);
    return (int)hipGetLastError();
  }
  set_max_dynamic_lds((const void*)cdma::conv_dma_kernel, cdma::LDS_BYTES);
  hipLaunchKernelGGL(cdma::conv_dma_kernel, dim3(ntm * ntn), dim3(512), cdma::LDS_BYTES, (hipStream_t)stream, p);
  return (int)hipGetLastError();
}

extern "C" int muse_conv2d_nhwc_gn_split2_ok(int32_t batch, int32_t H, int32_t W, int32_t Cin, int32_t Cout, int32_t KS) {
  const long M = (long)batch * H * W;
  return KS == 3 && (H % 16) == 0 && (W % 16) == 0 && (Cin % 64) == 0 && Cin <= 2048 && (Cout % 4) == 0 && M > 0 &&
         M * Cin * 4 < (1L << 32) - 64 && (long)Cout * 9 * Cin * 2 < (1L << 32) - 64 && M < (1L << 31) - 256;
}
extern "C" int muse_conv2d_nhwc_gn_split2(const float* x, const float* gn_scale, const float* gn_shift, const void* w_hi, const void* w_lo,
                                          const float* bias, const float* residual, float* out, double* gn_partial, int32_t gn_groups,
                                          int32_t batch, int32_t H, int32_t W, int32_t Cin, int32_t Cout, int32_t KS, int32_t persistent,
                                          void* stream) {
  const long M = (long)batch * H * W;
  if (M <= 0 || Cout <= 0) return 0;
  if (!muse_conv2d_nhwc_gn_split2_ok(batch, H, W, Cin, Cout, KS)) return MUSE_ERR_UNSUPPORTED;
  if ((((uintptr_t)x) | ((uintptr_t)w_hi) | ((uintptr_t)w_lo) | ((uintptr_t)out) | ((uintptr_t)residual)) & 15) return MUSE_ERR_ALIGN;
  cdma::Params p;
  p.xh = p.xl = nullptr; p.xf = x; p.gsc = gn_scale; p.gsh = gn_shift;
  p.wh = (const bf16_t*)w_hi; p.wl = (const bf16_t*)w_lo;
  p.bias = bias; p.residual = residual; p.out = out;
  p.gn_partial = gn_partial; p.gn_groups = gn_groups; p.gn_cpg = gn_groups > 0 ? Cout / gn_groups : 0;
  if (gn_partial) {
    const int cpg = p.gn_cpg;
    if (gn_groups <= 0 || (Cout % gn_groups) || cpg < 4 || cpg > 128 || (cpg & (cpg - 1))) return MUSE_ERR_UNSUPPORTED;
  }
  p.M = (int)M; p.N = Cout; p.K = 9 * Cin; p.H = H; p.W = W; p.Cin = Cin;
  const int ntn = (p.N + cslab::BN - 1) / cslab::BN;
  if (persistent && Cin <= cslab::P_GSS_MAX_CIN && (long)p.M * p.N * 4 < (1L << 32) - 64) {
    static const int grid_env = []() { const char* e = getenv("MUSE_CONV_PERSIST_GRID"); return e ? (atoi(e) < 1 ? 1 : atoi(e)) : 0; }();
    static const char* const min_env = getenv("MUSE_CONV_PERSIST_MIN");
    static const int min_tiles = min_env ? atoi(min_env) : 2, min_given = min_env != nullptr;
    const int ncu = device_cus();
    if (!ncu) return MUSE_ERR_UNSUPPORTED;
    const int grid = grid_env ? grid_env : ncu;
    set_max_dynamic_lds((const void*)cslab::conv_slab_persist_kernel<true>, cslab::P_LDS_BYTES_GN);
    const int nslab = (p.M >> 8) * ntn;
    static const int per_wg = []() { const char* e = getenv("MUSE_CONV_PERSIST_TILES"); return e ? atoi(e) : 0; }();
    if (per_wg > 0) {
      if (nslab >= (min_given ? (min_tiles > 1 ? min_tiles : 1) * per_wg : 2 * per_wg * ncu)) {
        hipLaunchKernelGGL(cslab::conv_slab_persist_kernel<true>, dim3((nslab + per_wg - 1) / per_wg), dim3(512), cslab::P_LDS_BYTES_GN, (hipStream_t)stream, p);
        return (int)hipGetLastError();
      }
    } else if (nslab >= min_tiles * grid) {
      hipLaunchKernelGGL(cslab::conv_slab_persist_kernel<true>, dim3(nslab < grid ? nslab : grid), dim3(512), cslab::P_LDS_BYTES_GN, (hipStream_t)stream, p);
      return (int)hipGetLastError();
    }
  }
  set_max_dynamic_lds((const void*)cslab::conv_slab_kernel<true>, cslab::LDS_BYTES + 2 * 2048 * 4);
  hipLaunchKernelGGL(cslab::conv_slab_kernel<true>, dim3((p.M >> 8) * ntn), dim3(512), cslab::LDS_BYTES + 2 * Cin * 4, (hipStream_t)stream, p);
  return (int)hipGetLastError();
}
```

open-muse_amd/csrc/vqgan.hip:

```cpp
#include "gemm_core.h"
#include "../../include/muse_hip.h"

extern "C" int muse_conv2d_nhwc(const void* in, const void* weight, const float* bias, const void* residual, void* out,
                                int32_t dtype, int32_t batch, int32_t H, int32_t W, int32_t Cin, int32_t Cout, int32_t KS,
                                int32_t upsample, void* stream) {
  const int esz = dtype == MUSE_BF16 ? 2 : 4, ch = 16 / esz;
  if (Cin % ch) return MUSE_ERR_ALIGN;
  if ((((uintptr_t)in) & 15) || (((uintptr_t)weight) & 15)) return MUSE_ERR_ALIGN;
  if (KS != 1 && KS != 3) return MUSE_ERR_UNSUPPORTED;
  if (upsample < 0 || upsample > 2 || (upsample == 2 && KS != 3)) return MUSE_ERR_BAD_ARG;
  if (upsample == 1 && ((H | W) & 1)) return MUSE_ERR_BAD_ARG;
  GemmParams p;
  p.A = in; p.B = weight; p.C = out;
  p.bias = bias; p.rowvec = nullptr; p.residual = residual;
  p.M = batch * H * W; p.N = Cout; p.K = KS * KS * Cin;
  p.lda = 0; p.ldb = p.K; p.ldc = Cout; p.ldr = Cout;
  p.zdiv = 1; p.sA0 = p.sA1 = p.sB0 = p.sB1 = p.sC0 = p.sC1 = 0;
  p.alpha = 1.0f; p.accumulate = 0; p.act = 0; p.split_k = 1; p.split_stride = 0;
  p.cH = H; p.cW = W; p.cCin = Cin; p.cKS = KS; p.cUps = upsample;
  p.cCinShift = -1;
  if ((Cin & (Cin - 1)) == 0) { int sh = 0; while ((1 << sh) < Cin) ++sh; p.cCinShift = sh; }
  hipStream_t s = (hipStream_t)stream;
  const bool big = use_bm256(p, 1);
  if (dtype == MUSE_BF16)
// ... 186 lines not shown
  } else {
    hipLaunchKernelGGL((gn_stats_kernel<bf16_t, 8>), grid, dim3(256), 0, s, (const bf16_t*)x, partial, HW, C, groups);
    hipLaunchKernelGGL((gn_apply_kernel<bf16_t, 8>), grid, dim3(256), 0, s, (const bf16_t*)x, (bf16_t*)y, gamma, beta,
                       (const double*)partial, HW, C, groups, nchunk, eps, apply_silu, (bf16_t*)nullptr, (bf16_t*)nullptr);
  }
  return (int)hipGetLastError();
}

__global__ __launch_bounds__(256) void gn_apply_split8_kernel(const float* __restrict__ x, const float* __restrict__ gamma,
                                                              const float* __restrict__ beta, const double* __restrict__ partial,
                                                              int HW, int C, int G, int nchunk, float eps, int silu,
                                                              bf16_t* __restrict__ y_hi, bf16_t* __restrict__ y_lo) {
  __shared__ float sc[1024], sh[1024];
  __shared__ float gmean[64], grstd[64];
  __shared__ double gs_[64], gq_[64];
  const int chunk = blockIdx.x, b = blockIdx.y;
  const int cpg = C / G;
  {
    const int tpg = 256 / G, g = threadIdx.x / tpg, sub = threadIdx.x % tpg;
    double s = 0.0, q = 0.0;
    for (int c = sub; c < nchunk; c += tpg) {
      const double* o = partial + (((long)b * nchunk + c) * G + g) * 2;
      s += o[0]; q += o[1];
    }
    for (int o = 1; o < tpg; o <<= 1) { s += __shfl_xor(s, o, 64); q += __shfl_xor(q, o, 64); }
    if (sub == 0) { gs_[g] = s; gq_[g] = q; }
  }
  __syncthreads();
  if (threadIdx.x < G) {
    const double s = gs_[threadIdx.x], q = gq_[threadIdx.x];
    const double n = (double)HW * (double)cpg;
    const double mean = s / n;
    double var = q / n - mean * mean;
    if (var < 0.0) var = 0.0;
    gmean[threadIdx.x] = (float)mean;
    grstd[threadIdx.x] = (float)(1.0 / sqrt(var + (double)eps));
  }
  __syncthreads();
  for (int c = threadIdx.x; c < C; c += 256) {
    const int g = c / cpg;
    const float scale = grstd[g] * gamma[c];
    sc[c] = scale;
    sh[c] = beta[c] - scale * gmean[g];
  }
  __syncthreads();
  const int vpp = C >> 3, vc = threadIdx.x % vpp, ppi = 256 / vpp;
  float scv[8], shv[8];
#pragma unroll
  for (int j = 0; j < 8; ++j) { scv[j] = sc[vc * 8 + j]; shv[j] = sh[vc * 8 + j]; }
  const int p0 = chunk * GN_PIX_PER_CHUNK, p1 = min(HW, p0 + GN_PIX_PER_CHUNK);
  constexpr int UN = 4;
  for (int pb = p0 + threadIdx.x / vpp; pb < p1; pb += UN * ppi) {
    f32x4 v[UN][2];
#pragma unroll
    for (int u = 0; u < UN; ++u) {
      const int p = pb + u * ppi;
      if (p < p1) {
        const float* src = x + ((long)b * HW + p) * C + vc * 8;
        v[u][0] = *(const f32x4*)src;
        v[u][1] = *(const f32x4*)(src + 4);
      }
    }
#pragma unroll
    for (int u = 0; u < UN; ++u) {
      const int p = pb + u * ppi;
      if (p >= p1) break;
      const long off = ((long)b * HW + p) * C + vc * 8;
      u32x4 hi4, lo4;
#pragma unroll
      for (int h = 0; h < 2; ++h) {
        u32x4 raw;
#pragma unroll
        for (int j = 0; j < 4; ++j) {
          float t = fmaf(v[u][h][j], scv[h * 4 + j], shv[h * 4 + j]);
          if (silu) t = gn_silu(t);
          raw[j] = __float_as_uint(t);
        }
        u32x2 hi, lo;
        split4(raw, hi, lo);
        hi4[2 * h] = hi[0]; hi4[2 * h + 1] = hi[1];
        lo4[2 * h] = lo[0]; lo4[2 * h + 1] = lo[1];
      }
      *(u32x4*)(y_hi + off) = hi4;
      *(u32x4*)(y_lo + off) = lo4;
    }
  }
}

__global__ __launch_bounds__(256) void gn_scale_shift_kernel(const double* __restrict__ partial, const float* __restrict__ gamma,
                                                             const float* __restrict__ beta, float* __restrict__ scale,
                                                             float* __restrict__ shift, int HW, int C, int G, int nchunk, float eps) {
  __shared__ float gmean[64], grstd[64];
  __shared__ double gs_[64], gq_[64];
  const int b = blockIdx.x, cpg = C / G;
  {
    const int tpg = 256 / G, g = threadIdx.x / tpg, sub = threadIdx.x % tpg;
    double s = 0.0, q = 0.0;
    for (int c = sub; c < nchunk; c += tpg) {
      const double* o = partial + (((long)b * nchunk + c) * G + g) * 2;
      s += o[0]; q += o[1];
    }
    for (int o = 1; o < tpg; o <<= 1) { s += __shfl_xor(s, o, 64); q += __shfl_xor(q, o, 64); }
    if (sub == 0) { gs_[g] = s; gq_[g] = q; }
  }
  __syncthreads();
  if (threadIdx.x < G) {
    const double s = gs_[threadIdx.x], q = gq_[threadIdx.x];
    const double n = (double)HW * (double)cpg;
    const double mean = s / n;
    double var = q / n - mean * mean;
    if (var < 0.0) var = 0.0;
    gmean[threadIdx.x] = (float)mean;
    grstd[threadIdx.x] = (float)(1.0 / sqrt(var + (double)eps));
  }
  __syncthreads();
  for (int c = threadIdx.x; c < C; c += 256) {
    const int g = c / cpg;
    const float sc = grstd[g] * gamma[c];
    scale[(long)b * C + c] = sc;
    shift[(long)b * C + c] = beta[c] - sc * gmean[g];
  }
}
extern "C" int muse_groupnorm_scale_shift(const double* partial, int32_t nchunk, const float* gamma, const float* beta, float* scale,
                                          float* shift, int32_t batch, int32_t HW, int32_t C, int32_t groups, float eps, void* stream) {
  if ((groups != 32 && groups != 64) || (C % groups) || nchunk <= 0) return MUSE_ERR_UNSUPPORTED;
  if (batch <= 0) return 0;
  hipLaunchKernelGGL(gn_scale_shift_kernel, dim3(batch), dim3(256), 0, (hipStream_t)stream, partial, gamma, beta, scale, shift, HW, C,
                     groups, nchunk, eps);
  return (int)hipGetLastError();
}

extern "C" int muse_groupnorm_silu_nhwc_split(const float* x, void* y_hi, void* y_lo, const float* gamma, const float* beta,
                                              double* partial, int32_t stats_nchunk, int32_t batch, int32_t HW, int32_t C,
                                              int32_t groups, float eps, int32_t apply_silu, void* stream) {
  if ((groups != 32 && groups != 64) || C > 1024 || (C % groups) || (C % 4)) return MUSE_ERR_UNSUPPORTED;
  const int vpp = C / 4;
  if (256 % vpp) return MUSE_ERR_UNSUPPORTED;
  if (batch <= 0) return 0;
  hipStream_t s = (hipStream_t)stream;
  const int nchunk = muse_groupnorm_nchunk(HW);
  dim3 grid(nchunk, batch);
  if (stats_nchunk <= 0) hipLaunchKernelGGL((gn_stats_kernel<float, 4>), grid, dim3(256), 0, s, x, partial, HW, C, groups);
  static const int wide = []() { const char* e = getenv("MUSE_GN_SPLIT8"); return e ? atoi(e) : 1; }();
  if (wide && (C % 8) == 0 && (256 % (C / 8)) == 0 && !((((uintptr_t)x) | ((uintptr_t)y_hi) | ((uintptr_t)y_lo)) & 15))
    hipLaunchKernelGGL(gn_apply_split8_kernel, grid, dim3(256), 0, s, x, gamma, beta, (const double*)partial, HW, C, groups,
                       stats_nchunk > 0 ? stats_nchunk : nchunk, eps, apply_silu, (bf16_t*)y_hi, (bf16_t*)y_lo);
  else
    hipLaunchKernelGGL((gn_apply_kernel<float, 4>), grid, dim3(256), 0, s, x, (float*)nullptr, gamma, beta, (const double*)partial,
                       HW, C, groups, stats_nchunk > 0 ? stats_nchunk : nchunk, eps, apply_silu, (bf16_t*)y_hi, (bf16_t*)y_lo);
  return (int)hipGetLastError();
}

typedef __attribute__((ext_vector_type(2))) float f32x2_t;
template <int CIN>
__global__ __launch_bounds__(256) void conv_in_direct_kernel(const float* __restrict__ x, const float* __restrict__ w4,
                                                             const float* __restrict__ bias, float* __restrict__ out,
                                                             double* __restrict__ gn_partial, int H, int W, int Cpad, int Cout) {
  __shared__ double red[2][256];
  const int qpp = Cout >> 2;
  const int cq = threadIdx.x % qpp, px0 = threadIdx.x / qpp, pstep = 256 / qpp;
  const int row = blockIdx.x, yy = row % H;
  f32x2_t wk[9][CIN][2];
#pragma unroll
  for (int t = 0; t < 9; ++t)
#pragma unroll
    for (int c = 0; c < CIN; ++c)
#pragma unroll
      for (int jp = 0; jp < 2; ++jp)
        wk[t][c][jp] = f32x2_t{w4[((long)(cq * 4 + 2 * jp) * 9 + t) * 4 + c], w4[((long)(cq * 4 + 2 * jp + 1) * 9 + t) * 4 + c]};
  f32x4 bv = {0.f, 0.f, 0.f, 0.f};
  if (bias) bv = *(const f32x4*)(bias + cq * 4);
  extern __shared__ __attribute__((aligned(16))) unsigned char cin_smem[];
  f32x4* xs = (f32x4*)cin_smem;
  for (int i = threadIdx.x; i < 3 * (W + 2); i += 256) {
    const int ky = i / (W + 2), ix = i - ky * (W + 2) - 1;
    const bool ok = (ky == 1 || (ky == 0 ? yy > 0 : yy + 1 < H)) && ix >= 0 && ix < W;
    xs[i] = ok ? *(const f32x4*)(x + ((long)(row + ky - 1) * W + ix) * Cpad) : f32x4{0.f, 0.f, 0.f, 0.f};
  }
  __syncthreads();
  double gs = 0.0, gq = 0.0;
  auto pixel = [&](int xx) {
    f32x2_t a01 = {bv[0], bv[1]}, a23 = {bv[2], bv[3]};
#pragma unroll
    for (int ky = 0; ky < 3; ++ky)
#pragma unroll
      for (int kx = 0; kx < 3; ++kx) {
        const f32x4 v = xs[ky * (W + 2) + xx + kx];
#pragma unroll
        for (int c = 0; c < CIN; ++c) {
          const f32x2_t in2 = {v[c], v[c]};
          a01 = __builtin_elementwise_fma(in2, wk[ky * 3 + kx][c][0], a01);
          a23 = __builtin_elementwise_fma(in2, wk[ky * 3 + kx][c][1], a23);
        }
      }
    const f32x4 acc = {a01[0], a01[1], a23[0], a23[1]};
    *(f32x4*)(out + ((long)row * W + xx) * Cout + cq * 4) = acc;
    if (gn_partial) {
#pragma unroll
      for (int j = 0; j < 4; ++j) { gs += (double)acc[j]; gq += (double)acc[j] * (double)acc[j]; }
    }
  };
  for (int xx = px0; xx < W; xx += pstep) pixel(xx);
  if (gn_partial) {
    red[0][threadIdx.x] = gs; red[1][threadIdx.x] = gq;
    __syncthreads();
    if (threadIdx.x < qpp) {
      double s = 0.0, q = 0.0;
      for (int k = 0; k < pstep; ++k) { s += red[0][k * qpp + threadIdx.x]; q += red[1][k * qpp + threadIdx.x]; }
      double* o = gn_partial + ((long)row * qpp + threadIdx.x) * 2;
      o[0] = s; o[1] = q;
    }
  }
}
extern "C" int muse_conv_in_direct(const float* x, const float* w4, const float* bias, float* out, double* gn_partial, int32_t gn_groups,
                                   int32_t batch, int32_t H, int32_t W, int32_t Cin, int32_t Cpad, int32_t Cout, void* stream) {
  const int qpp = Cout >> 2;
  if ((Cout & 3) || qpp > 256 || (256 % qpp) || Cpad < 4 || (Cpad & 3) || Cin < 1 || Cin > 4) return MUSE_ERR_UNSUPPORTED;
  if (gn_partial && gn_groups * 4 != Cout) return MUSE_ERR_UNSUPPORTED;
  if ((((uintptr_t)x) | ((uintptr_t)w4) | ((uintptr_t)bias) | ((uintptr_t)out)) & 15) return MUSE_ERR_ALIGN;
  if ((long)batch * H <= 0) return 0;
  if ((long)batch * H >= (1L << 31)) return MUSE_ERR_UNSUPPORTED;
  const size_t lds = (size_t)3 * (W + 2) * 16;
  if (lds > 48 * 1024) return MUSE_ERR_UNSUPPORTED;
#define CID(N) hipLaunchKernelGGL(conv_in_direct_kernel<N>, dim3((unsigned)(batch * H)), dim3(256), lds, (hipStream_t)stream, x, w4, bias, out, \
                                  gn_partial, H, W, Cpad, Cout)
  if (Cin == 3) CID(3); else if (Cin == 4) CID(4); else if (Cin == 1) CID(1); else CID(2);
#undef CID
  return (int)hipGetLastError();
}

template <int COUT>
__global__ __launch_bounds__(256) void conv_out_direct_kernel(const float* __restrict__ x, const float* __restrict__ scale,
                                                              const float* __restrict__ shift, const float* __restrict__ w,
                                                              const float* __restrict__ bias, float* __restrict__ out,
                                                              int H, int W, int C) {
  constexpr int PS = 36;
  __shared__ __attribute__((aligned(16))) float xs[18 * 18 * PS];
  __shared__ __attribute__((aligned(16))) float ws[COUT * 9 * 32];
  const int tiles_x = W >> 4, tiles_y = H >> 4;
  const int t = blockIdx.x, b = t / (tiles_x * tiles_y), ti = t - b * (tiles_x * tiles_y);
  const int y0 = (ti / tiles_x) << 4, x0 = (ti % tiles_x) << 4;
  const int py = threadIdx.x >> 4, px = threadIdx.x & 15;
  float acc[COUT];
#pragma unroll
  for (int o = 0; o < COUT; ++o) acc[o] = bias ? bias[o] : 0.f;
  for (int c0 = 0; c0 < C; c0 += 32) {
    __syncthreads();
    for (int i = threadIdx.x; i < 18 * 18 * 8; i += 256) {
      const int pix = i >> 3, q = i & 7;
      const int yy = y0 + pix / 18 - 1, xx = x0 + pix % 18 - 1;
      f32x4 v = {0.f, 0.f, 0.f, 0.f};
      if (yy >= 0 && yy < H && xx >= 0 && xx < W) {
        const f32x4 r = *(const f32x4*)(x + (((long)b * H + yy) * W + xx) * C + c0 + q * 4);
        const f32x4 sc = *(const f32x4*)(scale + (long)b * C + c0 + q * 4);
        const f32x4 sh = *(const f32x4*)(shift + (long)b * C + c0 + q * 4);
#pragma unroll
        for (int j = 0; j < 4; ++j) v[j] = gn_silu(fmaf(r[j], sc[j], sh[j]));
      }
      *(f32x4*)(xs + pix * PS + q * 4) = v;
    }
    for (int i = threadIdx.x; i < COUT * 9 * 8; i += 256) {
      const int ot = i >> 3, q = i & 7;
      *(f32x4*)(ws + ot * 32 + q * 4) = *(const f32x4*)(w + (long)ot * C + c0 + q * 4);
    }
    __syncthreads();
#pragma unroll
    for (int ky = 0; ky < 3; ++ky)
#pragma unroll
      for (int kx = 0; kx < 3; ++kx) {
        const float* xp = xs + ((py + ky) * 18 + px + kx) * PS;
#pragma unroll
        for (int q = 0; q < 8; ++q) {
          const f32x4 v = *(const f32x4*)(xp + q * 4);
#pragma unroll
          for (int o = 0; o < COUT; ++o) {
            const f32x4 wv = *(const f32x4*)(ws + (o * 9 + ky * 3 + kx) * 32 + q * 4);
            acc[o] = fmaf(v[0], wv[0], acc[o]);
            acc[o] = fmaf(v[1], wv[1], acc[o]);
            acc[o] = fmaf(v[2], wv[2], acc[o]);
            acc[o] = fmaf(v[3], wv[3], acc[o]);
          }
        }
      }
  }
  float* op = out + (((long)b * H + y0 + py) * W + x0 + px) * COUT;
#pragma unroll
  for (int o = 0; o < COUT; ++o) op[o] = acc[o];
}
extern "C" int muse_conv_out_direct(const float* x, const float* scale, const float* shift, const float* w, const float* bias, float* out,
                                    int32_t batch, int32_t H, int32_t W, int32_t C, int32_t Cout, void* stream) {
  if ((H & 15) || (W & 15) || (C & 31) || C < 32 || Cout < 1 || Cout > 4) return MUSE_ERR_UNSUPPORTED;
  if ((((uintptr_t)x) | ((uintptr_t)scale) | ((uintptr_t)shift) | ((uintptr_t)w)) & 15) return MUSE_ERR_ALIGN;
  const long tiles = (long)batch * (H >> 4) * (W >> 4);
  if (tiles <= 0) return 0;
  if (tiles >= (1L << 31)) return MUSE_ERR_UNSUPPORTED;
#define COD(N) hipLaunchKernelGGL(conv_out_direct_kernel<N>, dim3((unsigned)tiles), dim3(256), 0, (hipStream_t)stream, x, scale, shift, w, bias, out, H, W, C)
  if (Cout == 3) COD(3); else if (Cout == 4) COD(4); else if (Cout == 1) COD(1); else COD(2);
#undef COD
  return (int)hipGetLastError();
}

__global__ __launch_bounds__(256) void upsample2x_split_kernel(const float* __restrict__ x, bf16_t* __restrict__ y_hi,
                                                               bf16_t* __restrict__ y_lo, long npix, int H, int W, int C) {
  const int vpp = C >> 3;
  const long n = npix * vpp;
  for (long i = (long)blockIdx.x * 256 + threadIdx.x; i < n; i += (long)gridDim.x * 256) {
    const int vc = (int)(i % vpp);
    long p = i / vpp;
    const int xx = (int)(p % W); p /= W;
    const int yy = (int)(p % H);
    const long b = p / H;
    const float* src = x + (((b * H + yy) * W + xx) * (long)C) + vc * 8;
    const u32x4 v0 = *(const u32x4*)src, v1 = *(const u32x4*)(src + 4);
    u32x2 h0, l0, h1, l1;
    split4(v0, h0, l0);
    split4(v1, h1, l1);
    const u32x4 hv = {h0[0], h0[1], h1[0], h1[1]}, lv = {l0[0], l0[1], l1[0], l1[1]};
    const long W2 = 2L * W;
    const long o00 = (((b * 2 * H + 2 * yy) * W2 + 2 * xx) * (long)C) + vc * 8;
#pragma unroll
    for (int dy = 0; dy < 2; ++dy)
#pragma unroll
      for (int dx = 0; dx < 2; ++dx) {
        const long o = o00 + ((long)dy * W2 + dx) * C;
        *(u32x4*)(y_hi + o) = hv;
        *(u32x4*)(y_lo + o) = lv;
      }
  }
}
template <typename T, int VEC>
__global__ __launch_bounds__(256) void upsample2x_kernel(const T* __restrict__ x, T* __restrict__ y, long npix, int H, int W, int C) {
  const int vpp = C / VEC;
  const long n = npix * vpp;
  for (long i = (long)blockIdx.x * 256 + threadIdx.x; i < n; i += (long)gridDim.x * 256) {
    const int vc = (int)(i % vpp);
    long p = i / vpp;
    const int xx = (int)(p % W); p /= W;
    const int yy = (int)(p % H);
    const long b = p / H;
    const u32x4 v = *(const u32x4*)(x + (((b * H + yy) * W + xx) * (long)C) + vc * VEC);
    const long W2 = 2L * W;
    const long o00 = (((b * 2 * H + 2 * yy) * W2 + 2 * xx) * (long)C) + vc * VEC;
#pragma unroll
    for (int dy = 0; dy < 2; ++dy)
#pragma unroll
      for (int dx = 0; dx < 2; ++dx) *(u32x4*)(y + o00 + ((long)dy * W2 + dx) * C) = v;
  }
}
extern "C" int muse_upsample2x_nhwc(const void* x, void* y, int32_t dtype, int32_t batch, int32_t H, int32_t W, int32_t C, void* stream) {
  const int vec = dtype == MUSE_BF16 ? 8 : 4;
  if (C % vec) return MUSE_ERR_UNSUPPORTED;
  if ((((uintptr_t)x) | ((uintptr_t)y)) & 15) return MUSE_ERR_ALIGN;
  const long npix = (long)batch * H * W;
  if (npix <= 0) return 0;
  long g = (npix * (C / vec) + 255) / 256; if (g > 65536) g = 65536;
  if (dtype == MUSE_F32) hipLaunchKernelGGL((upsample2x_kernel<float, 4>), dim3((unsigned)g), dim3(256), 0, (hipStream_t)stream, (const float*)x, (float*)y, npix, H, W, C);
  else hipLaunchKernelGGL((upsample2x_kernel<bf16_t, 8>), dim3((unsigned)g), dim3(256), 0, (hipStream_t)stream, (const bf16_t*)x, (bf16_t*)y, npix, H, W, C);
  return (int)hipGetLastError();
}
extern "C" int muse_upsample2x_split_nhwc(const float* x, void* y_hi, void* y_lo, int32_t batch, int32_t H, int32_t W, int32_t C,
                                          void* stream) {
  if (C & 7) return MUSE_ERR_UNSUPPORTED;
  if ((((uintptr_t)x) | ((uintptr_t)y_hi) | ((uintptr_t)y_lo)) & 15) return MUSE_ERR_ALIGN;
  const long npix = (long)batch * H * W;
  if (npix <= 0) return 0;
  long g = (npix * (C >> 3) + 255) / 256; if (g > 65536) g = 65536;
  hipLaunchKernelGGL(upsample2x_split_kernel, dim3((unsigned)g), dim3(256), 0, (hipStream_t)stream, x, (bf16_t*)y_hi, (bf16_t*)y_lo, npix, H, W, C);
  return (int)hipGetLastError();
}

template <typename T, int VEC>
__global__ void avgpool_kernel(const T* __restrict__ x, T* __restrict__ y, int B, int H, int W, int C) {
  const int oh = H >> 1, ow = W >> 1, vpp = C / VEC;
  const long n = (long)B * oh * ow * vpp;
  for (long i = (long)blockIdx.x * blockDim.x + threadIdx.x; i < n; i += (long)gridDim.x * blockDim.x) {
    const int vc = (int)(i % vpp);
    long t = i / vpp;
    const int ox = (int)(t % ow); t /= ow;
// ... 206 lines not shown
```

open-muse_amd/muse/_hip.py:

```python
from __future__ import annotations

import ctypes as C
import os

import torch

F32, BF16, F16 = 0, 1, 2
_HERE = os.path.dirname(os.path.abspath(__file__))
LIB_PATH = os.environ.get("MUSE_HIP_LIB") or os.path.join(_HERE, "libmuse_hip.so")
_lib = None

c_void_p, c_int, c_i64, c_float = C.c_void_p, C.c_int32, C.c_int64, C.c_float


class GemmDesc(C.Structure):
    _fields_ = [
        ("A", c_void_p), ("B", c_void_p), ("C", c_void_p),
        ("bias", c_void_p), ("rowvec", c_void_p), ("residual", c_void_p),
        ("dtype", c_int), ("out_dtype", c_int), ("layout_a", c_int), ("layout_b", c_int),
        ("M", c_int), ("N", c_int), ("K", c_int), ("batch", c_int), ("zdiv", c_int),
        ("lda", c_i64), ("ldb", c_i64), ("ldc", c_i64), ("ldr", c_i64),
        ("sA0", c_i64), ("sA1", c_i64), ("sB0", c_i64), ("sB1", c_i64), ("sC0", c_i64), ("sC1", c_i64),
        ("alpha", c_float), ("accumulate", c_int), ("act", c_int), ("split_k", c_int), ("split_stride", c_i64),
    ]


class AttnDesc(C.Structure):
    _fields_ = [
        ("q", c_void_p), ("k", c_void_p), ("v", c_void_p), ("o", c_void_p),
        ("ldq", c_i64), ("ldk", c_i64), ("ldv", c_i64), ("ldo", c_i64),
        ("bsq", c_i64), ("bsk", c_i64), ("bsv", c_i64), ("bso", c_i64),
        ("batch", c_int), ("heads", c_int), ("head_dim", c_int), ("seq_q", c_int), ("seq_kv", c_int),
        ("alpha", c_float),
    ]


_IMG = (c_int, c_float, c_void_p)

SIGNATURES = {
    "muse_version": [],
    "muse_gemm": [C.POINTER(GemmDesc), c_void_p],
    "muse_gemm_x3": [C.POINTER(GemmDesc), c_i64, c_i64, c_void_p],
    "muse_gemm_tile": [C.POINTER(GemmDesc)],
    "muse_gemm_path": [C.POINTER(GemmDesc)],
    "muse_transpose": [c_void_p, c_void_p, c_int, c_int, c_int, c_i64, c_i64, c_int, c_i64, c_i64, c_void_p],
    "muse_layernorm_fwd": [c_void_p, c_int, c_void_p, c_void_p, c_void_p, c_int, c_void_p, c_void_p, c_int, c_int,
                           c_float, c_void_p],
    "muse_layernorm_bwd": [c_void_p, c_int, c_void_p, c_int, c_void_p, c_void_p, c_void_p, c_void_p, c_void_p, c_int,
                           c_void_p, c_void_p, c_int, c_int, c_int, c_void_p],
    "muse_layernorm_bwd_nblk": [c_int],
    "muse_layernorm_pair_fwd": [c_void_p] * 10 + [c_int, c_int, c_float, c_void_p],
    "muse_layernorm_pair_bwd": [c_void_p] * 14 + [c_int, c_int, c_int, c_void_p],
    "muse_colsum": [c_void_p, c_void_p, c_int, c_int, c_int, c_void_p],
    "muse_add_rowvec": [c_void_p, c_void_p, c_i64, c_int, c_void_p],
    "muse_bias_grad_rows_per_block": [],
    "muse_bias_grad_partial": [c_void_p, c_int, c_void_p, c_i64, c_int, c_i64, c_void_p],
    "muse_softmax_fwd": [c_void_p, c_void_p, c_int, c_i64, c_int, c_i64, c_void_p],
    "muse_softmax_bwd": [c_void_p, c_void_p, c_void_p, c_int, c_i64, c_int, c_i64, c_void_p],
    "muse_attention_seq_pad": [c_int],
    "muse_attention_fwd_ex": [C.POINTER(AttnDesc), c_void_p, c_void_p],
    "muse_attention_bwd_ex": [C.POINTER(AttnDesc), c_void_p, c_i64, c_i64, c_void_p, c_void_p, c_void_p, c_i64, c_i64, c_void_p,
                              c_i64, c_i64, c_void_p, c_i64, c_i64, c_void_p],
    "muse_attention_x3_fwd": [C.POINTER(AttnDesc), c_void_p, c_void_p, c_i64, *_IMG, c_void_p],
    "muse_attention_x3_bwd": [C.POINTER(AttnDesc), c_void_p, c_i64, c_i64, c_void_p, c_void_p, c_i64, c_i64, c_void_p, c_i64, c_i64, c_void_p,
                              c_i64, c_i64, c_void_p, c_i64, c_void_p, c_i64, c_void_p, c_i64, *_IMG, c_void_p],
    "muse_attention_x3_fwd_stream": [C.POINTER(AttnDesc), c_void_p, c_void_p, c_i64, *_IMG, c_void_p],
    "muse_attention_x3_bwd_stream": [C.POINTER(AttnDesc), c_void_p, c_i64, c_i64, c_void_p, c_void_p, c_void_p, c_i64, c_i64, c_void_p, c_i64, c_i64,
                                     c_void_p, c_i64, c_i64, c_void_p, c_i64, c_void_p, c_i64, c_void_p, c_i64, *_IMG, c_void_p],
    "muse_attention_x3_merge": [c_void_p, c_i64, c_void_p, c_i64, c_int, c_void_p, c_void_p, c_void_p, c_i64, c_int, c_int, c_int, *_IMG,
                                c_void_p],
    "muse_sum_parts_strided": [c_void_p, c_i64, c_int, c_i64, c_int, c_void_p, c_i64, c_int, c_void_p],
    "muse_attention_fwd": [c_void_p, c_void_p, c_void_p, c_int, c_int, c_int, c_int, c_float, c_void_p],
    "muse_attention_bwd": [c_void_p, c_void_p, c_void_p, c_void_p, c_void_p, c_void_p, c_int, c_int, c_int, c_int, c_float,
                           c_void_p],
    "muse_glu_fwd": [c_void_p, c_void_p, c_int, c_i64, c_int, c_void_p],
    "muse_glu_bwd": [c_void_p, c_void_p, c_void_p, c_int, c_i64, c_int, c_void_p],
    "muse_glu_fwd_x3": [c_void_p, c_void_p, c_void_p, c_i64, c_int, *_IMG, c_void_p],
    "muse_glu_bwd_x3": [c_void_p, c_void_p, c_void_p, c_void_p, c_i64, c_int, *_IMG, c_void_p],
    "muse_ffn_mid_rows_per_block": [],
    "muse_ffn_mid_fwd": [c_void_p, c_void_p, c_void_p, c_void_p, c_void_p, c_void_p, c_int, c_int, c_int, c_float, c_void_p],
    "muse_ffn_mid_bwd": [c_void_p, c_void_p, c_void_p, c_void_p, c_void_p, c_void_p, c_void_p, c_void_p, c_int, c_int, c_int,
                         c_void_p],
    "muse_gelu_fwd": [c_void_p, c_void_p, c_int, c_i64, c_void_p],
    "muse_gelu_bwd": [c_void_p, c_void_p, c_void_p, c_int, c_i64, c_void_p],
    "muse_gelu_bwd_f32_bf16": [c_void_p, c_void_p, c_void_p, c_i64, c_void_p],
    "muse_embed_fwd": [c_void_p, c_void_p, c_void_p, c_void_p, c_int, c_int, c_int, c_int, c_void_p],
    "muse_embed_bwd": [c_void_p, c_void_p, c_void_p, c_void_p, c_void_p, c_int, c_int, c_int, c_int, c_int, c_void_p],
    "muse_embed_bwd_scratch_floats": [c_int, c_int],
    "muse_embed_bwd2": [c_void_p, c_void_p, c_void_p, c_void_p, c_void_p, c_i64, c_int, c_int, c_int, c_int, c_int, c_void_p],
    "muse_embed_bwd2_scratch_bytes": [c_int, c_int, c_int, c_int],
    "muse_cross_entropy_fwd": [c_void_p, c_int, c_void_p, c_void_p, c_void_p, c_void_p, c_i64, c_int, c_i64, c_float,
                               c_void_p],
    "muse_cross_entropy_bwd": [c_void_p, c_int, c_void_p, c_void_p, c_void_p, c_void_p, c_void_p, c_int, c_i64, c_int,
                               c_i64, c_float, c_void_p],
    "muse_soft_ce_fwd": [c_void_p, c_void_p, c_void_p, c_void_p, c_void_p, c_void_p, c_void_p, c_i64, c_int, c_int, c_i64, c_void_p],
    "muse_soft_ce_bwd": [c_void_p, c_void_p, c_void_p, c_void_p, c_void_p, c_void_p, c_void_p, c_void_p, c_int, c_i64, c_int, c_int,
                         c_i64, c_i64, c_void_p],
    "muse_adamw_flat": [c_void_p, c_void_p, c_void_p, c_void_p, c_void_p, c_i64, c_float, c_float, c_float, c_float,
                        c_float, c_int, c_float, c_void_p, c_void_p],
    "muse_adamw_multi": [c_void_p, c_void_p, c_int, c_int, c_float, c_float, c_float, c_float, c_float, c_int, c_float, c_void_p,
                         c_void_p],
    "muse_ema_multi": [c_void_p, c_void_p, c_int, c_int, c_float, c_void_p],
    "muse_adamw_flat_groups": [c_void_p, c_void_p, c_void_p, c_void_p, c_void_p, c_i64, c_i64, c_void_p, c_void_p, c_int, c_void_p,
                               c_int, c_int, c_float, c_void_p, c_void_p],
    "muse_adamw_multi_groups": [c_void_p, c_void_p, c_int, c_int, c_void_p, c_int, c_int, c_float, c_void_p, c_void_p],
    "muse_gradnorm_flat": [c_void_p, c_i64, c_i64, c_void_p, c_void_p, c_void_p, c_void_p, c_int, c_void_p, c_void_p],
    "muse_gradnorm_multi": [c_void_p, c_int, c_void_p, c_int, c_int, c_void_p, c_void_p],
    "muse_gradnorm_finalize": [c_void_p, c_void_p, c_int, c_void_p, c_float, c_float, c_void_p, c_void_p],
    "muse_grad_scale_flat": [c_void_p, c_i64, c_void_p, c_void_p],
    "muse_grad_scale_multi": [c_void_p, c_int, c_void_p, c_int, c_int, c_void_p, c_void_p],
    "muse_adamw_flat_dev": [c_void_p, c_void_p, c_void_p, c_void_p, c_void_p, c_i64, c_float, c_float, c_float, c_float,
                            c_float, c_int, c_void_p, c_void_p, c_void_p],
    "muse_adamw_multi_dev": [c_void_p, c_void_p, c_int, c_int, c_float, c_float, c_float, c_float, c_float, c_int, c_void_p, c_void_p,
                             c_void_p],
    "muse_adamw_flat_groups_dev": [c_void_p, c_void_p, c_void_p, c_void_p, c_void_p, c_i64, c_i64, c_void_p, c_void_p, c_int, c_void_p,
                                   c_int, c_int, c_void_p, c_void_p, c_void_p],
    "muse_adamw_multi_groups_dev": [c_void_p, c_void_p, c_int, c_int, c_void_p, c_int, c_int, c_void_p, c_void_p, c_void_p],
    "muse_gemm_group_ok": [c_void_p, c_int, c_int],
    "muse_gemm_group": [c_void_p, c_int, c_int, c_void_p],
    "muse_sum_multi": [c_void_p, c_void_p, c_void_p, c_void_p, c_void_p, c_void_p, c_void_p, c_int, c_void_p],
    "muse_conv_out_direct": [c_void_p, c_void_p, c_void_p, c_void_p, c_void_p, c_void_p, c_int, c_int, c_int, c_int, c_int, c_void_p],
    "muse_upsample2x_split_nhwc": [c_void_p, c_void_p, c_void_p, c_int, c_int, c_int, c_int, c_void_p],
    "muse_split_f32_to_bf16x2": [c_void_p, c_void_p, c_void_p, c_i64, c_void_p],
    "muse_upsample2x_nhwc": [c_void_p, c_void_p, c_int, c_int, c_int, c_int, c_int, c_void_p],
    "muse_sum_slices_epilogue": [c_void_p, c_int, c_i64, c_void_p, c_void_p, c_i64, c_void_p, c_int, c_i64, c_i64, c_int, c_void_p],
    "muse_split_f32_to_bf16_cat3": [c_void_p, c_void_p, c_i64, c_int, c_i64, c_i64, c_int, c_int, c_void_p],
    "muse_sum_slices": [c_void_p, c_void_p, c_int, c_i64, c_i64, c_int, c_void_p],
    "muse_cast_f32_to_bf16": [c_void_p, c_void_p, c_i64, c_void_p],
    "muse_cast_bf16_to_f32": [c_void_p, c_void_p, c_i64, c_void_p],
    "muse_cast_f32_to_f16": [c_void_p, c_void_p, c_i64, c_float, c_void_p, c_void_p],
    "muse_mask_sample": [c_void_p, c_void_p, c_void_p, c_void_p, c_void_p, c_void_p, c_void_p, c_int, c_int, c_i64,
                         c_i64, c_float, c_void_p],
    "muse_sample_step": [c_void_p, c_void_p, c_float, c_i64, c_i64, c_int, c_void_p, c_i64, c_void_p, c_void_p, C.c_uint64, C.c_uint32,
                         c_float, c_int, c_int, c_int, c_void_p, c_void_p, c_void_p, c_void_p, c_void_p],
    "muse_mask_tokens": [c_void_p, c_void_p, c_void_p, c_void_p, c_void_p, c_void_p, c_void_p, c_void_p, c_void_p, c_int, c_int,
                         c_i64, c_float, c_int, c_float, c_void_p],
    "muse_dropout": [c_void_p, c_void_p, c_int, c_i64, c_float, C.c_uint64, C.c_uint64, c_void_p],
    "muse_cond_dropout": [c_void_p, c_void_p, c_void_p, c_void_p, c_int, c_i64, c_float, c_void_p],
    "muse_conv2d_nhwc": [c_void_p, c_void_p, c_void_p, c_void_p, c_void_p, c_int, c_int, c_int, c_int, c_int, c_int,
                         c_int, c_int, c_void_p],
    "muse_conv2d_nhwc_split": [c_void_p, c_void_p, c_void_p, c_void_p, c_void_p, c_void_p, c_void_p, c_int, c_int, c_int, c_int,
                               c_int, c_int, c_int, c_int, c_void_p],
    "muse_conv2d_nhwc_split2": [c_void_p, c_void_p, c_void_p, c_void_p, c_void_p, c_void_p, c_void_p, c_void_p, c_int, c_int, c_int,
                                c_int, c_int, c_int, c_int, c_void_p],
    "muse_conv_in_direct": [c_void_p, c_void_p, c_void_p, c_void_p, c_void_p, c_int, c_int, c_int, c_int, c_int, c_int, c_int, c_void_p],
    "muse_conv2d_nhwc_gn_split2_ok": [c_int, c_int, c_int, c_int, c_int, c_int],
    "muse_conv2d_nhwc_gn_split2": [c_void_p] * 9 + [c_int] * 8 + [c_void_p],
    "muse_groupnorm_scale_shift": [c_void_p, c_int, c_void_p, c_void_p, c_void_p, c_void_p, c_int, c_int, c_int, c_int, c_float, c_void_p],
    "muse_groupnorm_silu_nhwc_split": [c_void_p, c_void_p, c_void_p, c_void_p, c_void_p, c_void_p, c_int, c_int, c_int, c_int,
                                       c_int, c_float, c_int, c_void_p],
    "muse_groupnorm_silu_nhwc": [c_void_p, c_void_p, c_int, c_void_p, c_void_p, c_void_p, c_int, c_int, c_int, c_int,
                                 c_float, c_int, c_void_p],
    "muse_groupnorm_nchunk": [c_int],
    "muse_avgpool2x2_nhwc": [c_void_p, c_void_p, c_int, c_int, c_int, c_int, c_int, c_void_p],
    "muse_avgpool2x2_nhwc_stats": [c_void_p, c_void_p, c_void_p, c_int, c_int, c_int, c_int, c_int, c_void_p],
    "muse_nchw_to_nhwc": [c_void_p, c_void_p, c_int, c_int, c_int, c_int, c_int, c_void_p],
    "muse_nhwc_to_nchw": [c_void_p, c_int, c_void_p, c_int, c_int, c_int, c_int, c_void_p],
    "muse_argmin_rows": [c_void_p, c_void_p, c_i64, c_int, c_i64, c_void_p],
    "muse_row_sumsq": [c_void_p, c_void_p, c_i64, c_int, c_i64, c_void_p],
    "muse_gather_rows": [c_void_p, c_void_p, c_void_p, c_int, c_i64, c_int, c_void_p],
    "muse_norm_res_fwd": [c_void_p, c_void_p, c_void_p, c_void_p, c_void_p, c_i64, c_int, c_float, c_int, c_void_p],
    "muse_adaln_fwd": [c_void_p, c_void_p, c_void_p, c_int, c_i64, c_int, c_void_p],
    "muse_adaln_fwd_ex": [c_void_p, c_void_p, c_void_p, c_void_p, c_int, c_i64, c_int, c_void_p],
    "muse_silu_fwd": [c_void_p, c_void_p, c_i64, c_void_p],
    "muse_dwconv3x3_nhwc": [c_void_p, c_void_p, c_void_p, c_int, c_int, c_int, c_int, c_void_p],
    "muse_space_to_depth2_nhwc": [c_void_p, c_void_p, c_int, c_int, c_int, c_int, c_int, c_void_p],
    "muse_grn_fwd": [c_void_p, c_void_p, c_void_p, c_void_p, c_void_p, c_int, c_i64, c_int, c_void_p],
    "muse_grn_fwd_ex": [c_void_p, c_void_p, c_void_p, c_void_p, c_void_p, c_void_p, c_int, c_i64, c_int, c_void_p],
    "muse_sinusoidal_encode": [c_void_p, c_void_p, c_i64, c_int, c_float, c_void_p],
    "muse_weighted_mean": [c_void_p, c_void_p, c_void_p, c_i64, c_void_p],
    "muse_norm_res_bwd_nblk": [c_i64],
    "muse_norm_res_bwd": [c_void_p, c_void_p, c_void_p, c_void_p, c_void_p, c_void_p, c_i64, c_int, c_float, c_int, c_void_p],
    "muse_norm_res_bwd_ex": [c_void_p, c_void_p, c_void_p, c_void_p, c_void_p, c_void_p, c_void_p, c_i64, c_int, c_float, c_int, c_void_p],
    "muse_adaln_bwd": [c_void_p, c_void_p, c_void_p, c_void_p, c_void_p, c_int, c_i64, c_int, c_void_p],
    "muse_norm_adaln_fwd": [c_void_p] * 7 + [c_int, c_i64, c_int, c_float, c_int, c_void_p],
    "muse_norm_adaln_bwd": [c_void_p] * 9 + [c_int, c_i64, c_int, c_float, c_int, c_void_p],
    "muse_norm_adaln_fwd_x3": [c_void_p] * 7 + [c_int, c_i64, c_int, c_float, c_int, *_IMG, c_void_p],
    "muse_norm_adaln_bwd_x3": [c_void_p] * 9 + [c_int, c_i64, c_int, c_float, c_int, *_IMG, c_void_p],
    "muse_colsum_segments": [c_void_p, c_void_p, c_int, c_int, c_int, c_void_p],
    "muse_silu_bwd": [c_void_p, c_void_p, c_void_p, c_i64, c_void_p],
    "muse_dwconv3x3_bwd_nchunk": [c_i64],
    "muse_dwconv3x3_bwd": [c_void_p, c_void_p, c_void_p, c_void_p, c_void_p, c_int, c_int, c_int, c_int, c_void_p],
    "muse_grn_bwd": [c_void_p, c_void_p, c_void_p, c_void_p, c_void_p, c_void_p, c_int, c_i64, c_int, c_void_p],
    "muse_scale_rows": [c_void_p, c_void_p, c_void_p, c_void_p, c_i64, c_int, c_i64, c_void_p],
    "muse_probe_tr16": [c_void_p, c_void_p, c_void_p],
}
_RESTYPES = {"muse_embed_bwd_scratch_floats": c_i64, "muse_embed_bwd2_scratch_bytes": c_i64}


class MuseHipError(RuntimeError):
    pass


def lib():
    global _lib
    if _lib is None:
        if not os.path.exists(LIB_PATH):
            raise MuseHipError(
                f"{LIB_PATH} not found: build it with `python __graft_entry__.py` (or `make -C open-muse_amd/csrc`). "
                "This package has no CPU / eager fallback.")
        handle = C.CDLL(LIB_PATH)
        for name, argtypes in SIGNATURES.items():
            fn = getattr(handle, name)
            fn.argtypes = argtypes
            fn.restype = _RESTYPES.get(name, C.c_int)
        _lib = handle
    return _lib


def check(code: int, what: str) -> None:
    if code != 0:
        raise MuseHipError(f"{what} failed with code {code} "
                           f"({'hipError' if code > 0 else {-1: 'bad argument', -2: 'alignment', -3: 'unsupported'}.get(code, '?')})")


def stream() -> int:
    return torch.cuda.current_stream().cuda_stream


def dt(t: torch.Tensor) -> int:
    if t.dtype == torch.float32:
        return F32
    if t.dtype == torch.bfloat16:
        return BF16
    raise MuseHipError(f"unsupported dtype {t.dtype}")


def ptr(t):
    return None if t is None else t.data_ptr()


def require_gpu(*tensors):
    for t in tensors:
        if t is not None and not t.is_cuda:
            raise MuseHipError("muse (MI355X build): tensors must live on the GPU; there is no CPU compute path")
```

open-muse_amd/muse/modeling_maskgit_vqgan.py:

```python
from __future__ import annotations

import math
import os
from typing import Tuple

import torch
import torch.nn.functional as F
from torch import nn

from . import ops
from ._hip import MuseHipError
from .modeling_utils import ConfigMixin, ModelMixin, register_to_config


class _Conv(nn.Module):
    def __init__(self, cin, cout, k, bias):
        super().__init__()
        self.weight = nn.Parameter(torch.empty(cout, cin, k, k))
        self.bias = nn.Parameter(torch.empty(cout)) if bias else None
        nn.init.kaiming_uniform_(self.weight, a=math.sqrt(5))
        if bias:
            bound = 1.0 / math.sqrt(cin * k * k)
            nn.init.uniform_(self.bias, -bound, bound)


class _GNInput:
    __slots__ = ("x", "scale", "shift")

    def __init__(self, x, scale, shift):
        self.x, self.scale, self.shift = x, scale, shift


class _Norm(nn.Module):
    def __init__(self, c):
        super().__init__()
        self.weight = nn.Parameter(torch.ones(c))
        self.bias = nn.Parameter(torch.zeros(c))


class _Res(nn.Module):
    def __init__(self, cin, cout):
        super().__init__()
        self.norm1 = _Norm(cin)
        self.conv1 = _Conv(cin, cout, 3, False)
        self.norm2 = _Norm(cout)
        self.conv2 = _Conv(cout, cout, 3, False)
        if cin != cout:
            self.nin_shortcut = _Conv(cout, cout, 1, False)


class _Down(nn.Module):
    def __init__(self, cin, cout, nb):
        super().__init__()
        self.block = nn.ModuleList([_Res(cin if i == 0 else cout, cout) for i in range(nb)])


class _Up(nn.Module):
    def __init__(self, cin, cout, nb, upsample):
        super().__init__()
        self.block = nn.ModuleList([_Res(cin if i == 0 else cout, cout) for i in range(nb)])
        if upsample:
            self.upsample_conv = _Conv(cout, cout, 3, True)


class _Encoder(nn.Module):
    def __init__(self, cfg):
        super().__init__()
        hc, mult, nb = cfg.hidden_channels, tuple(cfg.channel_mult), cfg.num_res_blocks
        self.conv_in = _Conv(cfg.num_channels, hc, 3, False)
        in_mult = (1,) + mult
        self.down = nn.ModuleList([_Down(hc * in_mult[i], hc * mult[i], nb) for i in range(len(mult))])
        mid = hc * mult[-1]
        self.mid = nn.ModuleList([_Res(mid, mid) for _ in range(nb)])
        self.norm_out = _Norm(mid)
        self.conv_out = _Conv(mid, cfg.z_channels, 1, True)


class _Decoder(nn.Module):
    def __init__(self, cfg):
        super().__init__()
        hc, mult, nb = cfg.hidden_channels, tuple(cfg.channel_mult), cfg.num_res_blocks
        nres = len(mult)
        mid = hc * mult[-1]
        self.conv_in = _Conv(cfg.z_channels, mid, 3, True)
        self.mid = nn.ModuleList([_Res(mid, mid) for _ in range(nb)])
        ups = []
        for lvl in range(nres):
            cin = hc * mult[-1] if lvl == nres - 1 else hc * mult[lvl + 1]
            ups.append(_Up(cin, hc * mult[lvl], nb, lvl != 0))
        self.up = nn.ModuleList(ups)
        self.norm_out = _Norm(hc * mult[0])
        self.conv_out = _Conv(hc * mult[0], cfg.num_channels, 3, True)


class _Quantizer(nn.Module):
    def __init__(self, n, d):
        super().__init__()
        self.embedding = nn.Embedding(n, d)
        self.embedding.weight.data.uniform_(-1.0 / n, 1.0 / n)


class _ConvEngine:

    def _init_engine(self):
        self.compute_dtype = torch.float32
        self.fuse_gn_stats = True
        self.fuse_gn_apply = os.environ.get("MUSE_GN_FUSE", "1") != "0"
        self.direct_conv_in = os.environ.get("MUSE_CONV_IN_DIRECT", "1") != "0"
        self.dma_conv = True
        self.direct_conv_out = os.environ.get("MUSE_CONV_OUT_DIRECT", "1") != "0"
        self.upsample_split = os.environ.get("MUSE_UPSAMPLE_SPLIT", "1") != "0"
        self._packed = {}

    def _check(self, t):
        if not t.is_cuda:
            raise MuseHipError(f"{type(self).__name__} (MI355X build) has no CPU path: move the model and inputs to the GPU")

    def set_compute_dtype(self, dtype):
        if dtype not in (torch.float32, torch.bfloat16, "bf16x3"):
            raise ValueError('compute dtype must be torch.float32, torch.bfloat16 or "bf16x3"')
        self.compute_dtype = dtype
        return self

    def _act_dtype(self):
        return torch.bfloat16 if self.compute_dtype == torch.bfloat16 else torch.float32

    def _apply(self, fn, recurse=True):
        self._packed = {}
        return super()._apply(fn, recurse)

    def load_state_dict(self, state_dict, strict: bool = True, assign: bool = False):
        self._packed = {}
        return super().load_state_dict(state_dict, strict=strict, assign=assign)

    def _cpad(self, c, cd):
        q = 4 if cd == torch.float32 else 8
        return (c + q - 1) // q * q

    def _w(self, conv: _Conv, cd):
        key = (id(conv), cd)
        hit = self._packed.get(key)
        if hit is None:
            w = conv.weight.data
            cout, cin, k, _ = w.shape
            cp = self._cpad(cin, cd)
            wp = torch.zeros((cout, k, k, cp), dtype=torch.float32, device=w.device)
            wp[..., :cin] = w.permute(0, 2, 3, 1)
            wp = wp.contiguous()
            if cd == torch.bfloat16:
                wp = ops.cast_to_bf16(wp)
            elif cd == "bf16x3":
                wp = ops.split_bf16(wp)
            hit = (wp, cp, cout, k, None if conv.bias is None else conv.bias.data.float().contiguous())
            self._packed[key] = hit
        return hit

    def _conv_in(self, x, conv, B, H, W, cd, cpad):
        cout, cin, k, _ = conv.weight.shape
        if cd == "bf16x3" and self.direct_conv_in and ops.conv_in_direct_ok(cin, cout, k, cpad, W):
            key = (id(conv), "direct")
            hit = self._packed.get(key)
            if hit is None:
                w4 = torch.zeros((cout, 9, 4), dtype=torch.float32, device=conv.weight.device)
                w4[:, :, :cin] = conv.weight.data.float().permute(0, 2, 3, 1).reshape(cout, 9, cin)
                hit = (w4.contiguous(), None if conv.bias is None else conv.bias.data.float().contiguous())
                self._packed[key] = hit
            return ops.conv_in_direct(x, hit[0], B, H, W, cin, cpad, cout, bias=hit[1], gn_groups=32 if self.fuse_gn_stats else 0)
        return self._conv(x, conv, B, H, W, cd, gn_next=True)

    def _conv(self, x, conv, B, H, W, cd, residual=None, upsample=False, gn_next=False):
        wp, cp, cout, k, bias = self._w(conv, cd)
        if isinstance(x, _GNInput):
            return ops.conv2d_nhwc_gn_split2(x.x, x.scale, x.shift, wp[0], wp[1], B, H, W, cp, cout, bias=bias, residual=residual,
                                             gn_groups=32 if (gn_next and self.fuse_gn_stats) else 0)
        if isinstance(x, tuple):
            return ops.conv2d_nhwc_split2(x[0], x[1], wp[0], wp[1], B, H, W, cp, cout, bias=bias, residual=residual,
                                          gn_groups=32 if (gn_next and self.fuse_gn_stats) else 0)
        if cd == "bf16x3":
            if (self.dma_conv and self.upsample_split and not upsample and k == 3 and x.dtype == torch.float32 and x.is_contiguous()
                    and cp == x.shape[-1] and ops.conv_split2_ok(B, H, W, cp, cout, k) and ops.conv_slab_ok(H, W, cp)):
                hi, lo = ops.split_f32(x)
                return ops.conv2d_nhwc_split2(hi, lo, wp[0], wp[1], B, H, W, cp, cout, bias=bias, residual=residual,
                                              gn_groups=32 if (gn_next and self.fuse_gn_stats) else 0)
            return ops.conv2d_nhwc_split(x, wp[0], wp[1], B, H, W, cp, cout, k, bias=bias, residual=residual, upsample=upsample,
                                         gn_groups=32 if (gn_next and self.fuse_gn_stats) else 0)
        return ops.conv2d_nhwc(x, wp, B, H, W, cp, cout, k, bias=bias, residual=residual, upsample=upsample)

    def _upsample_conv(self, h, conv: _Conv, B, H, W, cd):
        cout, cin, k, _ = conv.weight.shape
        if (cd == "bf16x3" and self.dma_conv and self.upsample_split and cin % 8 == 0 and h.dtype == torch.float32
                and ops.conv_split2_ok(B, H, W, cin, cout, k)):
            planes = ops.upsample2x_split(h, B, H // 2, W // 2, cin)
            return self._conv(planes, conv, B, H, W, cd, gn_next=True)
        return self._conv(h, conv, B, H, W, cd, upsample=True, gn_next=True)

    def _conv_out(self, h, norm: _Norm, conv: _Conv, B, H, W, cd):
        cout, cin, k, _ = conv.weight.shape
        stats = getattr(h, "_gn_stats", None)
        if (cd == "bf16x3" and self.direct_conv_out and stats is not None and h.dtype == torch.float32
                and ops.conv_out_direct_ok(H, W, cin, cout, k)):
            key = (id(conv), "direct_out")
            hit = self._packed.get(key)
            if hit is None:
                hit = (conv.weight.data.float().permute(0, 2, 3, 1).reshape(cout, 9, cin).contiguous(),
                       None if conv.bias is None else conv.bias.data.float().contiguous())
                self._packed[key] = hit
            sc, sh = ops.groupnorm_scale_shift(stats, norm.weight.data, norm.bias.data, B, H * W, cin, groups=32, eps=1e-6)
            return ops.conv_out_direct(h, sc, sh, hit[0], hit[1], B, H, W, cin, cout)
        return self._conv(self._gn_for(h, norm, conv, B, H, W, cd), conv, B, H, W, cd)

    def _gn(self, x, norm: _Norm, B, HW, C, silu=True):
        return ops.groupnorm_silu_nhwc(x, norm.weight.data, norm.bias.data, B, HW, C, groups=32, eps=1e-6, silu=silu)

    def _gn_for(self, x, norm: _Norm, conv: _Conv, B, H, W, cd):
        cout, cin, k, _ = conv.weight.shape
        stats = getattr(x, "_gn_stats", None)
        if (cd == "bf16x3" and self.dma_conv and self.fuse_gn_apply and stats is not None and ops.conv_slab_ok(H, W, cin)
                and ops.conv_gn_split2_ok(B, H, W, cin, cout, k)):
            sc, sh = ops.groupnorm_scale_shift(stats, norm.weight.data, norm.bias.data, B, H * W, cin, groups=32, eps=1e-6)
            return _GNInput(x, sc, sh)
        if cd == "bf16x3" and self.dma_conv and ops.conv_split2_ok(B, H, W, cin, cout, k) and (256 % (cin // 4)) == 0:
            return ops.groupnorm_silu_nhwc_split(x, norm.weight.data, norm.bias.data, B, H * W, cin, groups=32, eps=1e-6, silu=True,
                                                 stats=getattr(x, "_gn_stats", None))
        return self._gn(x, norm, B, H * W, cin)


class MaskGitVQGAN(_ConvEngine, ModelMixin, ConfigMixin):
    _cast_selects_compute_mode = True

    def _compute_mode_for(self, dtype):
        if dtype is None or not dtype.is_floating_point:
            return False
        self.set_compute_dtype("bf16x3" if dtype in (torch.float16, torch.bfloat16) else torch.float32)
        return True

    @register_to_config
    def __init__(
        self,
        resolution: int = 256,
        num_channels: int = 3,
        hidden_channels: int = 128,
        channel_mult: Tuple = (1, 1, 2, 2, 4),
        num_res_blocks: int = 2,
        attn_resolutions: int = (16,),
        z_channels: int = 256,
        num_embeddings: int = 1024,
        quantized_embed_dim: int = 256,
        dropout: float = 0.0,
        resample_with_conv: bool = True,
        commitment_cost: float = 0.25,
    ):
        super().__init__()
        if dropout != 0.0:
            raise NotImplementedError("dropout > 0 in the VQGAN is outside the MI355X hot-path build")
        if z_channels != quantized_embed_dim:
            raise ValueError("z_channels must equal quantized_embed_dim")
        self.config.num_resolutions = len(channel_mult)
        self.config.reduction_factor = 2 ** (self.config.num_resolutions - 1)
        self.config.latent_size = resolution // self.config.reduction_factor
        self.encoder = _Encoder(self.config)
        self.decoder = _Decoder(self.config)
        self.quantize = _Quantizer(num_embeddings, quantized_embed_dim)
        self._init_engine()

    def _res(self, x, blk: _Res, B, H, W, cd):
        cin = blk.conv1.weight.shape[1]
        cout = blk.conv1.weight.shape[0]
        h = self._conv(self._gn_for(x, blk.norm1, blk.conv1, B, H, W, cd), blk.conv1, B, H, W, cd, gn_next=True)
        if cin == cout:
            return self._conv(self._gn_for(h, blk.norm2, blk.conv2, B, H, W, cd), blk.conv2, B, H, W, cd, residual=x, gn_next=True)
        h = self._conv(self._gn_for(h, blk.norm2, blk.conv2, B, H, W, cd), blk.conv2, B, H, W, cd)
        return self._conv(h, blk.nin_shortcut, B, H, W, cd, residual=h, gn_next=True)

    @torch.no_grad()
    def _encode_nhwc(self, pixel_values):
        self._check(pixel_values)
        cd = self.compute_dtype
        enc = self.encoder
        B, C, H, W = pixel_values.shape
        x = ops.nchw_to_nhwc(pixel_values.float(), self._act_dtype(), self._cpad(C, cd))
        h = self._conv_in(x, enc.conv_in, B, H, W, cd, self._cpad(C, cd))
        nres = self.config.num_resolutions
        for lvl, down in enumerate(enc.down):
            for blk in down.block:
                h = self._res(h, blk, B, H, W, cd)
            if lvl != nres - 1:
                h = ops.avgpool2x2_nhwc(h, B, H, W, h.shape[-1], gn_groups=32 if (cd == "bf16x3" and self.fuse_gn_stats) else 0)
                H, W = H // 2, W // 2
        for blk in enc.mid:
            h = self._res(h, blk, B, H, W, cd)
        h = self._gn_for(h, enc.norm_out, enc.conv_out, B, H, W, cd)
        z = self._conv(h, enc.conv_out, B, H, W, cd)
        z = z.view(B * H * W, -1)
        if z.dtype != torch.float32:
            z = ops.cast_to_f32(z)
        return z, (B, H, W)

    @torch.no_grad()
    def _decode_nhwc(self, zq, B, H, W):
        cd = self.compute_dtype
        dec = self.decoder
        nres = self.config.num_resolutions
        h = self._conv(zq, dec.conv_in, B, H, W, cd, gn_next=True)
        for blk in dec.mid:
            h = self._res(h, blk, B, H, W, cd)
        for lvl in reversed(range(nres)):
            up = dec.up[lvl]
            for blk in up.block:
                h = self._res(h, blk, B, H, W, cd)
            if lvl != 0:
                H, W = H * 2, W * 2
                h = self._upsample_conv(h, up.upsample_conv, B, H, W, cd)
        out = self._conv_out(h, dec.norm_out, dec.conv_out, B, H, W, cd)
        return ops.nhwc_to_nchw(out, self.config.num_channels)

    def _codebook(self):
        return self.quantize.embedding.weight.data

    @torch.no_grad()
    def encode(self, pixel_values, return_loss=False):
        z, (B, H, W) = self._encode_nhwc(pixel_values)
        cb = self._codebook()
        idx = ops.vq_nearest(z, cb)
        zq_rows = ops.gather_rows(cb, idx, torch.float32)
        zq = ops.nhwc_to_nchw(zq_rows.view(B, H, W, -1), zq_rows.shape[1])
        out = (zq, idx.view(B, H * W))
        if return_loss:
            zc = ops.nhwc_to_nchw(z.view(B, H, W, -1), z.shape[1])
            mse = torch.mean((zq - zc) ** 2)
            out = out + (mse + self.config.commitment_cost * mse,)
        return out

    @torch.no_grad()
    def decode(self, quantized_states):
        self._check(quantized_states)
        B, C, H, W = quantized_states.shape
        cd = self.compute_dtype
        zq = ops.nchw_to_nhwc(quantized_states.float(), self._act_dtype(), C)
        return self._decode_nhwc(zq, B, H, W)

    @torch.no_grad()
    def decode_code(self, codebook_indices):
        self._check(codebook_indices)
        B, T = codebook_indices.shape
        side = int(math.sqrt(T))
        zq = ops.gather_rows(self._codebook(), codebook_indices.contiguous().view(-1), self._act_dtype())
        return self._decode_nhwc(zq.view(B, side, side, -1), B, side, side)

    @torch.no_grad()
    def get_code(self, pixel_values):
        z, (B, H, W) = self._encode_nhwc(pixel_values)
        return ops.vq_nearest(z, self._codebook()).view(B, H * W)

    @torch.no_grad()
    def get_soft_code(self, pixel_values, temp=1.0, stochastic=False):
        z, (B, H, W) = self._encode_nhwc(pixel_values)
        cb = self._codebook()
        soft = ops.vq_neg_distances_scaled(z, cb, 1.0 / float(temp))
        ops.softmax_(soft, soft.shape[0], soft.shape[1], soft.shape[1])
        code = torch.multinomial(soft, 1) if stochastic else ops.vq_nearest(z, cb)
        return soft.view(B, H * W, -1), code.view(B, H * W)

    def forward(self, pixel_values, return_loss=False):
        enc = self.encode(pixel_values, return_loss)
        rec = self.decode(enc[0])
        out = (rec, enc[0], enc[1])
        if return_loss:
            out = out + (enc[2],)
        return out
```

open-muse_amd/muse/ops.py:

```python
from __future__ import annotations

import ctypes as C
import math
import os
import weakref

import torch

from . import _hip
from ._hip import BF16, F16, F32, GemmDesc, check, dt, lib, ptr, require_gpu, stream

USE_TR = os.environ.get("MUSE_GEMM_TR", "1") != "0"


def _esz(t):
    return t.element_size()


_PROF = None


PROF_BYTES = {}


# ... 1459 lines not shown
    input_ids = torch.empty((B, S + 1), dtype=torch.int64, device=tokens.device)
    labels = torch.empty((B, S + 1), dtype=torch.int64, device=tokens.device)
    mask_prob = torch.empty(B, dtype=torch.float32, device=tokens.device)
    check(lib().muse_mask_sample(tokens.data_ptr(), class_ids.data_ptr(), timesteps.data_ptr(), noise.data_ptr(),
                                 input_ids.data_ptr(), labels.data_ptr(), mask_prob.data_ptr(), B, S, mask_id, codebook_size,
                                 min_masking_rate, stream()), "muse_mask_sample")
    return input_ids, labels, mask_prob


def sample_step(cond_logits, input_ids, mask_id, vocab, temperature, sched_mask_len, *, uncond_logits=None, guidance_scale=0.0,
                noise_exp=None, noise_u=None, seed=0, step=0, want_raw=False):
    require_gpu(cond_logits, input_ids)
    B, S = input_ids.shape

    def layout(t):
        if t.dim() != 3 or t.shape[0] != B or t.shape[1] != S or t.stride(2) != 1 or t.dtype != torch.float32 or t.shape[2] < vocab:
            raise _hip.MuseHipError("sample_step: logits must be a float32 [B, S, >= vocab] view with a contiguous last dim")
        return t.stride(0), t.stride(1)

    lay = layout(cond_logits)
    if uncond_logits is not None and layout(uncond_logits) != lay:
        raise _hip.MuseHipError("sample_step: cond / uncond logits must share a layout")
    ids = input_ids.contiguous()
    sampled, nxt = torch.empty_like(ids), torch.empty_like(ids)
    raw = torch.empty_like(ids) if want_raw else None
    conf = torch.empty(B * S, dtype=torch.float32, device=ids.device)
    if noise_exp is not None:
        noise_exp = noise_exp.reshape(B * S, vocab).to(device=ids.device, dtype=torch.float32).contiguous()
    if noise_u is not None:
        noise_u = noise_u.reshape(B * S).to(device=ids.device, dtype=torch.float32).contiguous()
    check(lib().muse_sample_step(cond_logits.data_ptr(), ptr(uncond_logits), float(guidance_scale), lay[0], lay[1], int(vocab),
                                 ids.data_ptr(), int(mask_id), ptr(noise_exp), ptr(noise_u), int(seed) & (2 ** 64 - 1), int(step),
                                 float(temperature), int(sched_mask_len), B, S, ptr(raw), sampled.data_ptr(), nxt.data_ptr(),
                                 conf.data_ptr(), stream()), "muse_sample_step")
    return sampled, nxt, raw


def mask_tokens(tokens, mask_id, *, timesteps=None, mask_prob=None, noise=None, rects=None, min_masking_rate=0.0, all_labels=False,
                want_weight=False, weight_min=0.3):
    require_gpu(tokens)
    B, S = tokens.shape
    dev = tokens.device
    tokens = tokens.contiguous()
    input_ids, labels = torch.empty_like(tokens), torch.empty_like(tokens)
    lw = torch.empty((B, S), dtype=torch.float32, device=dev) if want_weight else None
    mp = torch.empty(B, dtype=torch.float32, device=dev)
    f = lambda t: None if t is None else t.to(device=dev, dtype=torch.float32).contiguous()
    timesteps, mask_prob, noise = f(timesteps), f(mask_prob), f(noise)
    if rects is not None:
        rects = rects.to(device=dev, dtype=torch.int32).contiguous()
    check(lib().muse_mask_tokens(tokens.data_ptr(), ptr(timesteps), ptr(mask_prob), ptr(noise), ptr(rects), input_ids.data_ptr(),
                                 labels.data_ptr(), ptr(lw), mp.data_ptr(), B, S, int(mask_id), float(min_masking_rate),
                                 1 if all_labels else 0, float(weight_min), stream()), "muse_mask_tokens")
    return input_ids, labels, lw, mp


def dropout(x, p, seed, offset, out=None):
    require_gpu(x)
    if not x.is_contiguous():
        raise _hip.MuseHipError("dropout expects a contiguous tensor")
    y = out if out is not None else torch.empty_like(x)
    check(lib().muse_dropout(x.data_ptr(), y.data_ptr(), dt(x), x.numel(), float(p), int(seed) & (2 ** 64 - 1), int(offset) & (2 ** 64 - 1),
                             stream()), "muse_dropout")
    return _touched(y) if out is not None else y


def cond_dropout(x, empty, uniforms, prob):
    require_gpu(x, empty, uniforms)
    B = x.shape[0]
    xc = x.float().contiguous()
    per = xc.numel() // B
    e = empty.float().contiguous()
    if e.numel() != per:
        raise _hip.MuseHipError("cond_dropout: the empty embedding must have the shape of one batch element")
    out = torch.empty_like(xc)
    check(lib().muse_cond_dropout(xc.data_ptr(), e.data_ptr(), uniforms.float().contiguous().data_ptr(), out.data_ptr(), B, per,
                                  float(prob), stream()), "muse_cond_dropout")
    return out


def conv2d_nhwc(x, w, B, H, W, Cin, Cout, KS, bias=None, residual=None, upsample=False):
    require_gpu(x, w)
    out = torch.empty((B, H, W, Cout), dtype=x.dtype, device=x.device)
    e0 = _prof_begin()
    check(lib().muse_conv2d_nhwc(x.data_ptr(), w.data_ptr(), ptr(bias), ptr(residual), out.data_ptr(), dt(x), B, H, W, Cin,
                                 Cout, KS, int(upsample), stream()), "muse_conv2d_nhwc")
    _prof_end(e0, f"conv_{'bf16' if x.dtype == torch.bfloat16 else 'f32'}", 2.0 * B * H * W * Cout * KS * KS * Cin)
    return out


def split_bf16(w):
    hi = cast_to_bf16(w.contiguous())
    lo = cast_to_bf16((w - cast_to_f32(hi)).contiguous())
    return hi, lo


def conv2d_nhwc_split(x, w_hi, w_lo, B, H, W, Cin, Cout, KS, bias=None, residual=None, upsample=False, gn_groups=0):
    require_gpu(x, w_hi, w_lo)
    out = torch.empty((B, H, W, Cout), dtype=torch.float32, device=x.device)
    part, nchunk = None, 0
    cpg = Cout // gn_groups if gn_groups else 0
    if gn_groups and Cout % gn_groups == 0 and cpg in (4, 8, 16, 32) and (H * W) % 128 == 0:
        nchunk = (H * W) // 128
        part = torch.empty(B * nchunk * gn_groups * 2, dtype=torch.float64, device=out.device)
    e0 = _prof_begin()
    check(lib().muse_conv2d_nhwc_split(x.data_ptr(), w_hi.data_ptr(), w_lo.data_ptr(), ptr(bias), ptr(residual), out.data_ptr(),
                                       ptr(part), gn_groups if part is not None else 0, B, H, W, Cin, Cout, KS,
                                       int(upsample), stream()), "muse_conv2d_nhwc_split")
    _prof_end(e0, "conv_bf16x3", 2.0 * B * H * W * Cout * KS * KS * Cin)
    if part is not None:
        out._gn_stats = (part, nchunk)
    return out


def conv2d_nhwc_split2(x_hi, x_lo, w_hi, w_lo, B, H, W, Cin, Cout, bias=None, residual=None, gn_groups=0):
    require_gpu(x_hi, x_lo, w_hi, w_lo)
    out = torch.empty((B, H, W, Cout), dtype=torch.float32, device=x_hi.device)
    part, nchunk = None, 0
    if gn_groups and conv_gn_stats_ok(H, W, Cout, gn_groups):
        nchunk = (H * W) // 256
        part = torch.empty(B * nchunk * gn_groups * 2, dtype=torch.float64, device=out.device)
    e0 = _prof_begin()
    check(lib().muse_conv2d_nhwc_split2(x_hi.data_ptr(), x_lo.data_ptr(), w_hi.data_ptr(), w_lo.data_ptr(), ptr(bias),
                                        ptr(residual), out.data_ptr(), ptr(part), gn_groups if part is not None else 0,
                                        B, H, W, Cin, Cout, 3, stream()), "muse_conv2d_nhwc_split2")
    _prof_end(e0, "conv_bf16x3_dma", 2.0 * B * H * W * Cout * 9 * Cin)
    if e0 is not None:
        PROF_BYTES["conv_bf16x3_dma"] = PROF_BYTES.get("conv_bf16x3_dma", 0.0) + _nbytes(x_hi, x_lo, w_hi, w_lo, residual, out)
    if part is not None:
        out._gn_stats = (part, nchunk)
    return out


def conv_in_direct_ok(Cin, Cout, KS, Cpad, W=256):
    return (KS == 3 and Cin <= 4 and Cpad % 4 == 0 and Cpad >= 4 and Cout % 4 == 0 and Cout // 4 <= 256 and 256 % (Cout // 4) == 0
            and W <= 1022)


def conv_in_direct(x, w4, B, H, W, Cin, Cpad, Cout, bias=None, gn_groups=0):
    require_gpu(x, w4)
    out = torch.empty((B, H, W, Cout), dtype=torch.float32, device=x.device)
    part = None
    if gn_groups and gn_groups * 4 == Cout:
        part = torch.empty(B * H * gn_groups * 2, dtype=torch.float64, device=x.device)
    e0 = _prof_begin()
    check(lib().muse_conv_in_direct(x.data_ptr(), w4.data_ptr(), ptr(bias), out.data_ptr(), ptr(part), gn_groups if part is not None else 0,
                                    B, H, W, Cin, Cpad, Cout, stream()), "muse_conv_in_direct")
    _prof_end(e0, "conv_in_direct", _nbytes(x, out), "byte")
    if part is not None:
        out._gn_stats = (part, H)
    return out


def conv_out_direct_ok(H, W, Cin, Cout, KS):
    return KS == 3 and Cout <= 4 and Cin % 32 == 0 and Cin >= 32 and H % 16 == 0 and W % 16 == 0


def conv_out_direct(x, scale, shift, w, bias, B, H, W, Cin, Cout):
    require_gpu(x, scale, shift, w)
    out = torch.empty((B, H, W, Cout), dtype=torch.float32, device=x.device)
    e0 = _prof_begin()
    check(lib().muse_conv_out_direct(x.data_ptr(), scale.data_ptr(), shift.data_ptr(), w.data_ptr(), ptr(bias), out.data_ptr(),
                                     B, H, W, Cin, Cout, stream()), "muse_conv_out_direct")
    _prof_end(e0, "conv_out_direct", _nbytes(x, out), "byte")
    return out


def upsample2x(x, B, H, W, C):
    require_gpu(x)
    y = torch.empty((B, 2 * H, 2 * W, C), dtype=x.dtype, device=x.device)
    check(lib().muse_upsample2x_nhwc(x.data_ptr(), y.data_ptr(), dt(x), B, H, W, C, stream()), "muse_upsample2x_nhwc")
    return y


def upsample2x_split(x, B, H, W, C):
    require_gpu(x)
    hi = torch.empty((B, 2 * H, 2 * W, C), dtype=torch.bfloat16, device=x.device)
    lo = torch.empty_like(hi)
    e0 = _prof_begin()
    check(lib().muse_upsample2x_split_nhwc(x.data_ptr(), hi.data_ptr(), lo.data_ptr(), B, H, W, C, stream()), "muse_upsample2x_split_nhwc")
    _prof_end(e0, "upsample2x_split", _nbytes(x, hi, lo), "byte")
    return hi, lo


_CONV_PERSISTENT = [os.environ.get("MUSE_CONV_PERSIST", "1") != "0"]


class conv_persistent:

    def __init__(self, on):
        self.on = bool(on)

    def __enter__(self):
        self.prev = _CONV_PERSISTENT[0]
        _CONV_PERSISTENT[0] = self.on
        return self

    def __exit__(self, *exc):
        _CONV_PERSISTENT[0] = self.prev
        return False


def conv_gn_split2_ok(B, H, W, Cin, Cout, KS):
    return bool(lib().muse_conv2d_nhwc_gn_split2_ok(B, H, W, Cin, Cout, KS))


def groupnorm_scale_shift(stats, gamma, beta, B, HW, C, groups=32, eps=1e-6):
    part, nchunk = stats
    require_gpu(part, gamma, beta)
    sc = torch.empty((B, C), dtype=torch.float32, device=part.device)
    sh = torch.empty((B, C), dtype=torch.float32, device=part.device)
    check(lib().muse_groupnorm_scale_shift(part.data_ptr(), nchunk, gamma.data_ptr(), beta.data_ptr(), sc.data_ptr(), sh.data_ptr(),
                                           B, HW, C, groups, eps, stream()), "muse_groupnorm_scale_shift")
    return sc, sh


def conv2d_nhwc_gn_split2(x, scale, shift, w_hi, w_lo, B, H, W, Cin, Cout, bias=None, residual=None, gn_groups=0):
    require_gpu(x, scale, shift, w_hi, w_lo)
    out = torch.empty((B, H, W, Cout), dtype=torch.float32, device=x.device)
    part, nchunk = None, 0
    if gn_groups and conv_gn_stats_ok(H, W, Cout, gn_groups):
        nchunk = (H * W) // 256
        part = torch.empty(B * nchunk * gn_groups * 2, dtype=torch.float64, device=out.device)
    e0 = _prof_begin()
    check(lib().muse_conv2d_nhwc_gn_split2(x.data_ptr(), scale.data_ptr(), shift.data_ptr(), w_hi.data_ptr(), w_lo.data_ptr(), ptr(bias),
                                           ptr(residual), out.data_ptr(), ptr(part), gn_groups if part is not None else 0,
                                           B, H, W, Cin, Cout, 3, int(_CONV_PERSISTENT[0]), stream()), "muse_conv2d_nhwc_gn_split2")
    _prof_end(e0, "conv_bf16x3_dma", 2.0 * B * H * W * Cout * 9 * Cin)
    if e0 is not None:
        PROF_BYTES["conv_bf16x3_dma"] = PROF_BYTES.get("conv_bf16x3_dma", 0.0) + _nbytes(x, w_hi, w_lo, residual, out)
    if part is not None:
        out._gn_stats = (part, nchunk)
    return out


def conv_split2_ok(B, H, W, Cin, Cout, KS):
    M = B * H * W
    return KS == 3 and Cin % 32 == 0 and Cout % 4 == 0 and M * Cin * 2 < (1 << 32) - 64 and M < (1 << 31) - 256


def conv_slab_ok(H, W, Cin):
    import os
    return H % 16 == 0 and W % 16 == 0 and Cin % 64 == 0 and os.environ.get("MUSE_CONV_SLAB", "1") != "0"


def conv_gn_stats_ok(H, W, Cout, groups):
    cpg = Cout // groups if groups else 0
    return groups in (32, 64) and Cout % groups == 0 and (H * W) % 256 == 0 and 4 <= cpg <= 128 and (cpg & (cpg - 1)) == 0


def groupnorm_silu_nhwc_split(x, gamma, beta, B, HW, C, groups=32, eps=1e-6, silu=True, stats=None):
    require_gpu(x, gamma, beta)
    hi = torch.empty(x.shape, dtype=torch.bfloat16, device=x.device)
    lo = torch.empty(x.shape, dtype=torch.bfloat16, device=x.device)
    if stats is not None:
        part, snc = stats
    else:
        nchunk = lib().muse_groupnorm_nchunk(HW)
        part, snc = torch.empty(B * nchunk * groups * 2, dtype=torch.float64, device=x.device), 0
    e0 = _prof_begin()
    check(lib().muse_groupnorm_silu_nhwc_split(x.data_ptr(), hi.data_ptr(), lo.data_ptr(), gamma.data_ptr(), beta.data_ptr(),
                                               part.data_ptr(), snc, B, HW, C, groups, eps, 1 if silu else 0, stream()),
          "muse_groupnorm_silu_nhwc_split")
    _prof_end(e0, "groupnorm_silu", _nbytes(x, hi, lo), "byte")
    return hi, lo


def groupnorm_silu_nhwc(x, gamma, beta, B, HW, C, groups=32, eps=1e-6, silu=True):
    require_gpu(x, gamma, beta)
    y = torch.empty_like(x)
    nchunk = lib().muse_groupnorm_nchunk(HW)
    part = torch.empty(B * nchunk * groups * 2, dtype=torch.float64, device=x.device)
    e0 = _prof_begin()
    check(lib().muse_groupnorm_silu_nhwc(x.data_ptr(), y.data_ptr(), dt(x), gamma.data_ptr(), beta.data_ptr(), part.data_ptr(),
                                         B, HW, C, groups, eps, 1 if silu else 0, stream()), "muse_groupnorm_silu_nhwc")
    _prof_end(e0, "groupnorm_silu", _nbytes(x, y), "byte")
    return y


def avgpool2x2_nhwc(x, B, H, W, C_, gn_groups=0):
    require_gpu(x)
    y = torch.empty((B, H // 2, W // 2, C_), dtype=x.dtype, device=x.device)
    e0 = _prof_begin()
    vpp = C_ // 4
    if gn_groups and x.dtype == torch.float32 and C_ % 4 == 0 and C_ % gn_groups == 0 and vpp <= 256 and 256 % vpp == 0:
        nchunk = lib().muse_groupnorm_nchunk((H // 2) * (W // 2))
        part = torch.empty(B * nchunk * gn_groups * 2, dtype=torch.float64, device=x.device)
        check(lib().muse_avgpool2x2_nhwc_stats(x.data_ptr(), y.data_ptr(), part.data_ptr(), gn_groups, B, H, W, C_, stream()),
              "muse_avgpool2x2_nhwc_stats")
        y._gn_stats = (part, nchunk)
    else:
        check(lib().muse_avgpool2x2_nhwc(x.data_ptr(), y.data_ptr(), dt(x), B, H, W, C_, stream()), "muse_avgpool2x2_nhwc")
    _prof_end(e0, "avgpool2x2", _nbytes(x, y), "byte")
    return y


def nchw_to_nhwc(x, out_dtype, cpad):
    require_gpu(x)
    B, C_, H, W = x.shape
    x = x.contiguous()
    out = torch.empty((B, H, W, cpad), dtype=out_dtype, device=x.device)
    check(lib().muse_nchw_to_nhwc(x.data_ptr(), out.data_ptr(), dt(out), B, C_, H * W, cpad, stream()), "muse_nchw_to_nhwc")
    return out


def nhwc_to_nchw(x, C_):
    require_gpu(x)
    B, H, W, cpad = x.shape
    out = torch.empty((B, C_, H, W), dtype=torch.float32, device=x.device)
    check(lib().muse_nhwc_to_nchw(x.data_ptr(), dt(x), out.data_ptr(), B, C_, H * W, cpad, stream()), "muse_nhwc_to_nchw")
    return out


def vq_nearest(z_flat, codebook, en=None, return_dist=False):
    require_gpu(z_flat, codebook)
    N, D = z_flat.shape
    Kc = codebook.shape[0]
    zn = torch.empty(N, dtype=torch.float32, device=z_flat.device)
    check(lib().muse_row_sumsq(z_flat.data_ptr(), zn.data_ptr(), N, D, z_flat.stride(0), stream()), "muse_row_sumsq")
    if en is None:
        en = torch.empty(Kc, dtype=torch.float32, device=z_flat.device)
        check(lib().muse_row_sumsq(codebook.data_ptr(), en.data_ptr(), Kc, D, codebook.stride(0), stream()), "muse_row_sumsq")
    dist = torch.empty((N, Kc), dtype=torch.float32, device=z_flat.device)
    gemm(z_flat, codebook, dist, N, Kc, D, la=0, lb=0, lda=z_flat.stride(0), ldb=codebook.stride(0), ldc=Kc, alpha=-2.0,
         bias=en, rowvec=zn)
    idx = torch.empty(N, dtype=torch.int64, device=z_flat.device)
    check(lib().muse_argmin_rows(dist.data_ptr(), idx.data_ptr(), N, Kc, Kc, stream()), "muse_argmin_rows")
    return (idx, dist) if return_dist else idx


def vq_neg_distances_scaled(z_flat, codebook, inv_temp):
    require_gpu(z_flat, codebook)
    N, D = z_flat.shape
    Kc = codebook.shape[0]
    zn = torch.empty(N, dtype=torch.float32, device=z_flat.device)
    en = torch.empty(Kc, dtype=torch.float32, device=z_flat.device)
    check(lib().muse_row_sumsq(z_flat.data_ptr(), zn.data_ptr(), N, D, z_flat.stride(0), stream()), "muse_row_sumsq")
    check(lib().muse_row_sumsq(codebook.data_ptr(), en.data_ptr(), Kc, D, codebook.stride(0), stream()), "muse_row_sumsq")
    out = torch.empty((N, Kc), dtype=torch.float32, device=z_flat.device)
    gemm(z_flat, codebook, out, N, Kc, D, la=0, lb=0, lda=z_flat.stride(0), ldb=codebook.stride(0), ldc=Kc, alpha=2.0 * inv_temp,
         bias=en.mul_(-inv_temp), rowvec=zn.mul_(-inv_temp))
    return out


def gather_rows(table, idx, out_dtype):
    require_gpu(table, idx)
    rows = idx.numel()
    cols = table.shape[1]
    out = torch.empty((rows, cols), dtype=out_dtype, device=table.device)
    check(lib().muse_gather_rows(table.data_ptr(), idx.data_ptr(), out.data_ptr(), dt(out), rows, cols, stream()), "muse_gather_rows")
    return out


def norm_res_fwd(x, w, eps, mode, residual=None, want_pre=False):
    require_gpu(x)
    rows, cols = x.shape
    y = torch.empty_like(x)
    pre = torch.empty_like(x) if want_pre else None
    check(lib().muse_norm_res_fwd(x.data_ptr(), ptr(residual), ptr(w), y.data_ptr(), ptr(pre), rows, cols, eps, mode, stream()),
          "muse_norm_res_fwd")
    return y, pre


def adaln_fwd(x, ss, batch, out_dtype=torch.float32):
    require_gpu(x, ss)
    rows, C_ = x.shape
    y = torch.empty((rows, C_), dtype=out_dtype, device=x.device)
    f32 = out_dtype == torch.float32
    check(lib().muse_adaln_fwd_ex(x.data_ptr(), ss.data_ptr(), y.data_ptr() if f32 else None, None if f32 else y.data_ptr(), batch,
                                  rows // batch, C_, stream()), "muse_adaln_fwd_ex")
    return y


def silu_fwd(x):
    require_gpu(x)
    y = torch.empty_like(x)
    check(lib().muse_silu_fwd(x.data_ptr(), y.data_ptr(), x.numel(), stream()), "muse_silu_fwd")
    return y


# ... 193 lines not shown
```

Before: 1221 images/s.

## Fuse 2x2 avgpool into VQGAN encoder conv epilogue and read NCHW input directly

Adds a POOL variant of the GN-fused bf16x3 slab conv kernels. Its epilogue averages 2x2 pixel quads from the LDS staging tile and writes the half-resolution output, with GN stats computed on the pooled values. This removes the separate avgpool kernel and the full-resolution write/read at each downsampling level. It also adds an NCHW-input variant of the direct conv_in kernel, which drops the standalone nchw_to_nhwc transpose, at the cost of strided per-channel loads.

```diff
diff --git a/include/muse_hip.h b/include/muse_hip.h
--- a/include/muse_hip.h
+++ b/include/muse_hip.h
@@ -220,10 +220,16 @@
                                const float* bias, const float* residual, float* out, double* gn_partial, int32_t gn_groups,
                                int32_t batch, int32_t H, int32_t W, int32_t Cin, int32_t Cout, int32_t KS, int32_t persistent,
                                void* stream);
+int muse_conv2d_nhwc_gn_split2_pool(const float* x, const float* gn_scale, const float* gn_shift, const void* w_hi, const void* w_lo,
+                                    const float* bias, const float* residual, float* out, double* gn_partial, int32_t gn_groups,
+                                    int32_t batch, int32_t H, int32_t W, int32_t Cin, int32_t Cout, int32_t KS, int32_t persistent,
+                                    void* stream);
 int muse_groupnorm_scale_shift(const double* partial, int32_t nchunk, const float* gamma, const float* beta, float* scale,
                                float* shift, int32_t batch, int32_t HW, int32_t C, int32_t groups, float eps, void* stream);
 int muse_conv_in_direct(const float* x, const float* w4, const float* bias, float* out, double* gn_partial, int32_t gn_groups,
                         int32_t batch, int32_t H, int32_t W, int32_t Cin, int32_t Cpad, int32_t Cout, void* stream);
+int muse_conv_in_direct_nchw(const float* x, const float* w4, const float* bias, float* out, double* gn_partial, int32_t gn_groups,
+                             int32_t batch, int32_t H, int32_t W, int32_t Cin, int32_t Cout, void* stream);
 int muse_conv_out_direct(const float* x, const float* scale, const float* shift, const float* w, const float* bias, float* out,
                          int32_t batch, int32_t H, int32_t W, int32_t C, int32_t Cout, void* stream);
 int muse_upsample2x_nhwc(const void* x, void* y, int32_t dtype, int32_t batch, int32_t H, int32_t W, int32_t C, void* stream);
diff --git a/open-muse_amd/csrc/conv_dma.hip b/open-muse_amd/csrc/conv_dma.hip
--- a/open-muse_amd/csrc/conv_dma.hip
+++ b/open-muse_amd/csrc/conv_dma.hip
@@ -276,7 +276,7 @@
 #define CDMA_TS(IDX)
 #define CDMA_TSV(V, IDX)
 #endif
-template <bool GN>
+template <bool GN, bool POOL = false>
 __global__ __launch_bounds__(512, 2) void conv_slab_kernel(Params p) {
   extern __shared__ __attribute__((aligned(16))) unsigned char smem[];
   CDMA_TS(0)
@@ -556,7 +556,34 @@
   constexpr int NIT = (BM * 32) / NT;
   const int col = (threadIdx.x & 31) * 4, n = n0 + col, rbase = threadIdx.x >> 5;
   const long pix0 = ((long)img * H + y0) * W + x0 + rbase;
-  if (n < p.N) {
+  if constexpr (POOL) {
+    const int qx = rbase & 7, qy0 = rbase >> 3, Wo = W >> 1;
+    const long pixf = ((long)img * H + y0 + 2 * qy0) * W + x0 + 2 * qx;
+    const long pixo = ((long)img * (H >> 1) + (y0 >> 1) + qy0) * Wo + (x0 >> 1) + qx;
+    if (n < p.N) {
+      f32x4 rv[NIT];
+      if (p.residual) {
+#pragma unroll
+        for (int it = 0; it < NIT; ++it)
+          rv[it] = *(const f32x4*)(p.residual + (pixf + (long)(4 * (it >> 2) + ((it >> 1) & 1)) * W + (it & 1)) * p.N + n);
+      }
+#pragma unroll
+      for (int k = 0; k < 4; ++k) {
+        f32x4 v[4];
+#pragma unroll
+        for (int d = 0; d < 4; ++d) {
+          v[d] = *(const f32x4*)(smem + ((2 * qy0 + 4 * k + (d >> 1)) * 16 + 2 * qx + (d & 1)) * CST + col * 4);
+          if (p.residual) v[d] += rv[4 * k + d];
+        }
+        const f32x4 w = (((v[0] + v[1]) + v[2]) + v[3]) * 0.25f;
+        *(f32x4*)(p.out + (pixo + (long)(2 * k) * Wo) * p.N + n) = w;
+        if (p.gn_partial) {
+#pragma unroll
+          for (int e = 0; e < 4; ++e) { gs += (double)w[e]; gq += (double)w[e] * (double)w[e]; }
+        }
+      }
+    }
+  } else if (n < p.N) {
     f32x4 rv[NIT];
     if (p.residual) {
 #pragma unroll
@@ -607,7 +634,7 @@
 __host__ __device__ constexpr int p_stage_off(int st) { return st == 0 ? 32768 : (st - 1) * 16384; }
 static_assert(P_BBASE + 3 * BSTAGE == P_BUF1 && P_BUF1 + SLAB <= P_LDS_BYTES && P_LDS_BYTES_GN <= 163840, "LDS map");
 
-template <bool GN>
+template <bool GN, bool POOL = false>
 __global__ __launch_bounds__(512, 2) void conv_slab_persist_kernel(Params p) {
   extern __shared__ __attribute__((aligned(16))) unsigned char smem[];
   const int H = p.H, W = p.W, Cin = p.Cin;
@@ -629,7 +656,9 @@
   const unsigned oobB = (bytesB + 15u) & ~15u;
   const int nchunks = Cin >> 5;
   const unsigned bytesO = (unsigned)((long)p.M * p.N * 4);
-  const rsrc_t rs_out = make_rsrc(p.out, bytesO), rs_res = make_rsrc(p.residual ? (const void*)p.residual : (const void*)p.out, bytesO);
+  const unsigned bytesOut = POOL ? bytesO >> 2 : bytesO;
+  const rsrc_t rs_out = make_rsrc(p.out, bytesOut);
+  const rsrc_t rs_res = make_rsrc(p.residual ? (const void*)p.residual : (const void*)p.out, p.residual ? bytesO : bytesOut);
 
   int slab_piece[3];
 #pragma unroll
@@ -931,7 +960,27 @@
         }
       }
       lds_barrier();
-      if (n < p.N) {
+      if constexpr (POOL) {
+        if (n < p.N) {
+          const int qx = rbase & 7, qy0 = rbase >> 3;
+          const long pixo = ((long)g.img * (H >> 1) + (g.y0 >> 1) + qy0) * (W >> 1) + (g.x0 >> 1) + qx;
+          const unsigned pbase = (unsigned)((pixo * p.N + n) * 4);
+          const unsigned prowstep = (unsigned)((long)(W >> 1) * p.N * 4);
+#pragma unroll
+          for (int k = 0; k < 2; ++k) {
+            f32x4 v[4];
+#pragma unroll
+            for (int d = 0; d < 4; ++d)
+              v[d] = *(const f32x4*)(smem + P_STAGING + ((2 * qy0 + 4 * k + (d >> 1)) * 16 + 2 * qx + (d & 1)) * CST + col * 4);
+            const f32x4 w = (((v[0] + v[1]) + v[2]) + v[3]) * 0.25f;
+            __builtin_amdgcn_raw_buffer_store_b128(__builtin_bit_cast(u32x4, w), rs_out, (int)pbase, (int)(prowstep * (half * 4 + 2 * k)), 0);
+            if (p.gn_partial) {
+#pragma unroll
+              for (int e = 0; e < 4; ++e) { gs += (double)w[e]; gq += (double)w[e] * (double)w[e]; }
+            }
+          }
+        }
+      } else if (n < p.N) {
 #pragma unroll
         for (int it = 0; it < NITH; ++it) {
           const f32x4 w = *(const f32x4*)(smem + P_STAGING + (rbase + 16 * it) * CST + col * 4);
@@ -1034,10 +1083,11 @@
   return KS == 3 && (H % 16) == 0 && (W % 16) == 0 && (Cin % 64) == 0 && Cin <= 2048 && (Cout % 4) == 0 && M > 0 &&
          M * Cin * 4 < (1L << 32) - 64 && (long)Cout * 9 * Cin * 2 < (1L << 32) - 64 && M < (1L << 31) - 256;
 }
-extern "C" int muse_conv2d_nhwc_gn_split2(const float* x, const float* gn_scale, const float* gn_shift, const void* w_hi, const void* w_lo,
-                                          const float* bias, const float* residual, float* out, double* gn_partial, int32_t gn_groups,
-                                          int32_t batch, int32_t H, int32_t W, int32_t Cin, int32_t Cout, int32_t KS, int32_t persistent,
-                                          void* stream) {
+template <bool POOL>
+static int conv_gn_split2_launch(const float* x, const float* gn_scale, const float* gn_shift, const void* w_hi, const void* w_lo,
+                                 const float* bias, const float* residual, float* out, double* gn_partial, int32_t gn_groups,
+                                 int32_t batch, int32_t H, int32_t W, int32_t Cin, int32_t Cout, int32_t KS, int32_t persistent,
+                                 void* stream) {
   const long M = (long)batch * H * W;
   if (M <= 0 || Cout <= 0) return 0;
   if (!muse_conv2d_nhwc_gn_split2_ok(batch, H, W, Cin, Cout, KS)) return MUSE_ERR_UNSUPPORTED;
@@ -1060,20 +1110,34 @@
     const int ncu = device_cus();
     if (!ncu) return MUSE_ERR_UNSUPPORTED;
     const int grid = grid_env ? grid_env : ncu;
-    set_max_dynamic_lds((const void*)cslab::conv_slab_persist_kernel<true>, cslab::P_LDS_BYTES_GN);
+    set_max_dynamic_lds((const void*)cslab::conv_slab_persist_kernel<true, POOL>, cslab::P_LDS_BYTES_GN);
     const int nslab = (p.M >> 8) * ntn;
     static const int per_wg = []() { const char* e = getenv("MUSE_CONV_PERSIST_TILES"); return e ? atoi(e) : 0; }();
     if (per_wg > 0) {
       if (nslab >= (min_given ? (min_tiles > 1 ? min_tiles : 1) * per_wg : 2 * per_wg * ncu)) {
-        hipLaunchKernelGGL(cslab::conv_slab_persist_kernel<true>, dim3((nslab + per_wg - 1) / per_wg), dim3(512), cslab::P_LDS_BYTES_GN, (hipStream_t)stream, p);
+        hipLaunchKernelGGL((cslab::conv_slab_persist_kernel<true, POOL>), dim3((nslab + per_wg - 1) / per_wg), dim3(512), cslab::P_LDS_BYTES_GN, (hipStream_t)stream, p);
         return (int)hipGetLastError();
       }
     } else if (nslab >= min_tiles * grid) {
-      hipLaunchKernelGGL(cslab::conv_slab_persist_kernel<true>, dim3(nslab < grid ? nslab : grid), dim3(512), cslab::P_LDS_BYTES_GN, (hipStream_t)stream, p);
+      hipLaunchKernelGGL((cslab::conv_slab_persist_kernel<true, POOL>), dim3(nslab < grid ? nslab : grid), dim3(512), cslab::P_LDS_BYTES_GN, (hipStream_t)stream, p);
       return (int)hipGetLastError();
     }
   }
-  set_max_dynamic_lds((const void*)cslab::conv_slab_kernel<true>, cslab::LDS_BYTES + 2 * 2048 * 4);
-  hipLaunchKernelGGL(cslab::conv_slab_kernel<true>, dim3((p.M >> 8) * ntn), dim3(512), cslab::LDS_BYTES + 2 * Cin * 4, (hipStream_t)stream, p);
+  set_max_dynamic_lds((const void*)cslab::conv_slab_kernel<true, POOL>, cslab::LDS_BYTES + 2 * 2048 * 4);
+  hipLaunchKernelGGL((cslab::conv_slab_kernel<true, POOL>), dim3((p.M >> 8) * ntn), dim3(512), cslab::LDS_BYTES + 2 * Cin * 4, (hipStream_t)stream, p);
   return (int)hipGetLastError();
 }
+extern "C" int muse_conv2d_nhwc_gn_split2(const float* x, const float* gn_scale, const float* gn_shift, const void* w_hi, const void* w_lo,
+                                          const float* bias, const float* residual, float* out, double* gn_partial, int32_t gn_groups,
+                                          int32_t batch, int32_t H, int32_t W, int32_t Cin, int32_t Cout, int32_t KS, int32_t persistent,
+                                          void* stream) {
+  return conv_gn_split2_launch<false>(x, gn_scale, gn_shift, w_hi, w_lo, bias, residual, out, gn_partial, gn_groups, batch, H, W, Cin, Cout,
+                                      KS, persistent, stream);
+}
+extern "C" int muse_conv2d_nhwc_gn_split2_pool(const float* x, const float* gn_scale, const float* gn_shift, const void* w_hi,
+                                               const void* w_lo, const float* bias, const float* residual, float* out, double* gn_partial,
+                                               int32_t gn_groups, int32_t batch, int32_t H, int32_t W, int32_t Cin, int32_t Cout, int32_t KS,
+                                               int32_t persistent, void* stream) {
+  return conv_gn_split2_launch<true>(x, gn_scale, gn_shift, w_hi, w_lo, bias, residual, out, gn_partial, gn_groups, batch, H, W, Cin, Cout,
+                                     KS, persistent, stream);
+}
diff --git a/open-muse_amd/csrc/vqgan.hip b/open-muse_amd/csrc/vqgan.hip
--- a/open-muse_amd/csrc/vqgan.hip
+++ b/open-muse_amd/csrc/vqgan.hip
@@ -362,7 +362,7 @@
 }
 
 typedef __attribute__((ext_vector_type(2))) float f32x2_t;
-template <int CIN>
+template <int CIN, bool NCHW = false>
 __global__ __launch_bounds__(256) void conv_in_direct_kernel(const float* __restrict__ x, const float* __restrict__ w4,
                                                              const float* __restrict__ bias, float* __restrict__ out,
                                                              double* __restrict__ gn_partial, int H, int W, int Cpad, int Cout) {
@@ -385,7 +385,17 @@
   for (int i = threadIdx.x; i < 3 * (W + 2); i += 256) {
     const int ky = i / (W + 2), ix = i - ky * (W + 2) - 1;
     const bool ok = (ky == 1 || (ky == 0 ? yy > 0 : yy + 1 < H)) && ix >= 0 && ix < W;
-    xs[i] = ok ? *(const f32x4*)(x + ((long)(row + ky - 1) * W + ix) * Cpad) : f32x4{0.f, 0.f, 0.f, 0.f};
+    if constexpr (NCHW) {
+      f32x4 v = {0.f, 0.f, 0.f, 0.f};
+      if (ok) {
+        const float* src = x + (((long)(row / H) * CIN) * H + (yy + ky - 1)) * W + ix;
+#pragma unroll
+        for (int c = 0; c < CIN; ++c) v[c] = src[(long)c * H * W];
+      }
+      xs[i] = v;
+    } else {
+      xs[i] = ok ? *(const f32x4*)(x + ((long)(row + ky - 1) * W + ix) * Cpad) : f32x4{0.f, 0.f, 0.f, 0.f};
+    }
   }
   __syncthreads();
   double gs = 0.0, gq = 0.0;
@@ -434,6 +444,23 @@
   if (lds > 48 * 1024) return MUSE_ERR_UNSUPPORTED;
 #define CID(N) hipLaunchKernelGGL(conv_in_direct_kernel<N>, dim3((unsigned)(batch * H)), dim3(256), lds, (hipStream_t)stream, x, w4, bias, out, \
                                   gn_partial, H, W, Cpad, Cout)
+  if (Cin == 3) CID(3); else if (Cin == 4) CID(4); else if (Cin == 1) CID(1); else CID(2);
+#undef CID
+  return (int)hipGetLastError();
+}
+
+extern "C" int muse_conv_in_direct_nchw(const float* x, const float* w4, const float* bias, float* out, double* gn_partial,
+                                        int32_t gn_groups, int32_t batch, int32_t H, int32_t W, int32_t Cin, int32_t Cout, void* stream) {
+  const int qpp = Cout >> 2;
+  if ((Cout & 3) || qpp > 256 || (256 % qpp) || Cin < 1 || Cin > 4) return MUSE_ERR_UNSUPPORTED;
+  if (gn_partial && gn_groups * 4 != Cout) return MUSE_ERR_UNSUPPORTED;
+  if (((((uintptr_t)w4) | ((uintptr_t)bias) | ((uintptr_t)out)) & 15) || (((uintptr_t)x) & 3)) return MUSE_ERR_ALIGN;
+  if ((long)batch * H <= 0) return 0;
+  if ((long)batch * H >= (1L << 31)) return MUSE_ERR_UNSUPPORTED;
+  const size_t lds = (size_t)3 * (W + 2) * 16;
+  if (lds > 48 * 1024) return MUSE_ERR_UNSUPPORTED;
+#define CID(N) hipLaunchKernelGGL((conv_in_direct_kernel<N, true>), dim3((unsigned)(batch * H)), dim3(256), lds, (hipStream_t)stream, x, w4, bias, \
+                                  out, gn_partial, H, W, 0, Cout)
   if (Cin == 3) CID(3); else if (Cin == 4) CID(4); else if (Cin == 1) CID(1); else CID(2);
 #undef CID
   return (int)hipGetLastError();
diff --git a/open-muse_amd/muse/_hip.py b/open-muse_amd/muse/_hip.py
--- a/open-muse_amd/muse/_hip.py
+++ b/open-muse_amd/muse/_hip.py
@@ -144,8 +144,10 @@
     "muse_conv2d_nhwc_split2": [c_void_p, c_void_p, c_void_p, c_void_p, c_void_p, c_void_p, c_void_p, c_void_p, c_int, c_int, c_int,
                                 c_int, c_int, c_int, c_int, c_void_p],
     "muse_conv_in_direct": [c_void_p, c_void_p, c_void_p, c_void_p, c_void_p, c_int, c_int, c_int, c_int, c_int, c_int, c_int, c_void_p],
+    "muse_conv_in_direct_nchw": [c_void_p, c_void_p, c_void_p, c_void_p, c_void_p, c_int, c_int, c_int, c_int, c_int, c_int, c_void_p],
     "muse_conv2d_nhwc_gn_split2_ok": [c_int, c_int, c_int, c_int, c_int, c_int],
     "muse_conv2d_nhwc_gn_split2": [c_void_p] * 9 + [c_int] * 8 + [c_void_p],
+    "muse_conv2d_nhwc_gn_split2_pool": [c_void_p] * 9 + [c_int] * 8 + [c_void_p],
     "muse_groupnorm_scale_shift": [c_void_p, c_int, c_void_p, c_void_p, c_void_p, c_void_p, c_int, c_int, c_int, c_int, c_float, c_void_p],
     "muse_groupnorm_silu_nhwc_split": [c_void_p, c_void_p, c_void_p, c_void_p, c_void_p, c_void_p, c_int, c_int, c_int, c_int,
                                        c_int, c_float, c_int, c_void_p],
diff --git a/open-muse_amd/muse/modeling_maskgit_vqgan.py b/open-muse_amd/muse/modeling_maskgit_vqgan.py
--- a/open-muse_amd/muse/modeling_maskgit_vqgan.py
+++ b/open-muse_amd/muse/modeling_maskgit_vqgan.py
@@ -107,6 +107,8 @@
         self.fuse_gn_stats = True
         self.fuse_gn_apply = os.environ.get("MUSE_GN_FUSE", "1") != "0"
         self.direct_conv_in = os.environ.get("MUSE_CONV_IN_DIRECT", "1") != "0"
+        self.conv_in_nchw = os.environ.get("MUSE_CONV_IN_NCHW", "1") != "0"
+        self.fuse_pool = os.environ.get("MUSE_POOL_FUSE", "1") != "0"
         self.dma_conv = True
         self.direct_conv_out = os.environ.get("MUSE_CONV_OUT_DIRECT", "1") != "0"
         self.upsample_split = os.environ.get("MUSE_UPSAMPLE_SPLIT", "1") != "0"
@@ -155,21 +157,39 @@
             self._packed[key] = hit
         return hit
 
+    def _conv_in_image(self, pixel_values, conv, B, H, W, cd):
+        C = pixel_values.shape[1]
+        cout, cin, k, _ = conv.weight.shape
+        cpad = self._cpad(C, cd)
+        x = pixel_values.float()
+        if (cd == "bf16x3" and self.direct_conv_in and self.conv_in_nchw and cin == C and ops.conv_in_direct_ok(cin, cout, k, cpad, W)):
+            w4, bias = self._w_conv_in_direct(conv)
+            return ops.conv_in_direct_nchw(x.contiguous(), w4, B, H, W, cin, cout, bias=bias, gn_groups=32 if self.fuse_gn_stats else 0)
+        return self._conv_in(ops.nchw_to_nhwc(x, self._act_dtype(), cpad), conv, B, H, W, cd, cpad)
+
+    def _w_conv_in_direct(self, conv):
+        cout, cin, k, _ = conv.weight.shape
+        key = (id(conv), "direct")
+        hit = self._packed.get(key)
+        if hit is None:
+            w4 = torch.zeros((cout, 9, 4), dtype=torch.float32, device=conv.weight.device)
+            w4[:, :, :cin] = conv.weight.data.float().permute(0, 2, 3, 1).reshape(cout, 9, cin)
+            hit = (w4.contiguous(), None if conv.bias is None else conv.bias.data.float().contiguous())
+            self._packed[key] = hit
+        return hit
+
     def _conv_in(self, x, conv, B, H, W, cd, cpad):
         cout, cin, k, _ = conv.weight.shape
         if cd == "bf16x3" and self.direct_conv_in and ops.conv_in_direct_ok(cin, cout, k, cpad, W):
-            key = (id(conv), "direct")
-            hit = self._packed.get(key)
-            if hit is None:
-                w4 = torch.zeros((cout, 9, 4), dtype=torch.float32, device=conv.weight.device)
-                w4[:, :, :cin] = conv.weight.data.float().permute(0, 2, 3, 1).reshape(cout, 9, cin)
-                hit = (w4.contiguous(), None if conv.bias is None else conv.bias.data.float().contiguous())
-                self._packed[key] = hit
+            hit = self._w_conv_in_direct(conv)
             return ops.conv_in_direct(x, hit[0], B, H, W, cin, cpad, cout, bias=hit[1], gn_groups=32 if self.fuse_gn_stats else 0)
         return self._conv(x, conv, B, H, W, cd, gn_next=True)
 
-    def _conv(self, x, conv, B, H, W, cd, residual=None, upsample=False, gn_next=False):
+    def _conv(self, x, conv, B, H, W, cd, residual=None, upsample=False, gn_next=False, pool=False):
         wp, cp, cout, k, bias = self._w(conv, cd)
+        if pool:
+            return ops.conv2d_nhwc_gn_split2_pool(x.x, x.scale, x.shift, wp[0], wp[1], B, H, W, cp, cout, bias=bias, residual=residual,
+                                                  gn_groups=32 if (gn_next and self.fuse_gn_stats) else 0)
         if isinstance(x, _GNInput):
             return ops.conv2d_nhwc_gn_split2(x.x, x.scale, x.shift, wp[0], wp[1], B, H, W, cp, cout, bias=bias, residual=residual,
                                              gn_groups=32 if (gn_next and self.fuse_gn_stats) else 0)
@@ -185,6 +205,11 @@
             return ops.conv2d_nhwc_split(x, wp[0], wp[1], B, H, W, cp, cout, k, bias=bias, residual=residual, upsample=upsample,
                                          gn_groups=32 if (gn_next and self.fuse_gn_stats) else 0)
         return ops.conv2d_nhwc(x, wp, B, H, W, cp, cout, k, bias=bias, residual=residual, upsample=upsample)
+
+    def _pool_ok(self, x, conv: _Conv, B, H, W, cd):
+        cout, cin, k, _ = conv.weight.shape
+        return (cd == "bf16x3" and self.fuse_pool and isinstance(x, _GNInput) and cin == cout
+                and ops.conv_gn_split2_pool_ok(B, H, W, cin, cout, k, 32 if self.fuse_gn_stats else 0))
 
     def _upsample_conv(self, h, conv: _Conv, B, H, W, cd):
         cout, cin, k, _ = conv.weight.shape
@@ -263,12 +288,17 @@
         self.quantize = _Quantizer(num_embeddings, quantized_embed_dim)
         self._init_engine()
 
-    def _res(self, x, blk: _Res, B, H, W, cd):
+    def _res(self, x, blk: _Res, B, H, W, cd, pool=False):
         cin = blk.conv1.weight.shape[1]
         cout = blk.conv1.weight.shape[0]
         h = self._conv(self._gn_for(x, blk.norm1, blk.conv1, B, H, W, cd), blk.conv1, B, H, W, cd, gn_next=True)
         if cin == cout:
-            return self._conv(self._gn_for(h, blk.norm2, blk.conv2, B, H, W, cd), blk.conv2, B, H, W, cd, residual=x, gn_next=True)
+            g = self._gn_for(h, blk.norm2, blk.conv2, B, H, W, cd)
+            if pool and self._pool_ok(g, blk.conv2, B, H, W, cd):
+                out = self._conv(g, blk.conv2, B, H, W, cd, residual=x, gn_next=True, pool=True)
+                out._pooled = True
+                return out
+            return self._conv(g, blk.conv2, B, H, W, cd, residual=x, gn_next=True)
         h = self._conv(self._gn_for(h, blk.norm2, blk.conv2, B, H, W, cd), blk.conv2, B, H, W, cd)
         return self._conv(h, blk.nin_shortcut, B, H, W, cd, residual=h, gn_next=True)
 
@@ -278,14 +308,14 @@
         cd = self.compute_dtype
         enc = self.encoder
         B, C, H, W = pixel_values.shape
-        x = ops.nchw_to_nhwc(pixel_values.float(), self._act_dtype(), self._cpad(C, cd))
-        h = self._conv_in(x, enc.conv_in, B, H, W, cd, self._cpad(C, cd))
+        h = self._conv_in_image(pixel_values, enc.conv_in, B, H, W, cd)
         nres = self.config.num_resolutions
         for lvl, down in enumerate(enc.down):
-            for blk in down.block:
-                h = self._res(h, blk, B, H, W, cd)
+            for i, blk in enumerate(down.block):
+                h = self._res(h, blk, B, H, W, cd, pool=lvl != nres - 1 and i == len(down.block) - 1)
             if lvl != nres - 1:
-                h = ops.avgpool2x2_nhwc(h, B, H, W, h.shape[-1], gn_groups=32 if (cd == "bf16x3" and self.fuse_gn_stats) else 0)
+                if not getattr(h, "_pooled", False):
+                    h = ops.avgpool2x2_nhwc(h, B, H, W, h.shape[-1], gn_groups=32 if (cd == "bf16x3" and self.fuse_gn_stats) else 0)
                 H, W = H // 2, W // 2
         for blk in enc.mid:
             h = self._res(h, blk, B, H, W, cd)
diff --git a/open-muse_amd/muse/ops.py b/open-muse_amd/muse/ops.py
--- a/open-muse_amd/muse/ops.py
+++ b/open-muse_amd/muse/ops.py
@@ -1635,6 +1635,23 @@
     return out
 
 
+def conv_in_direct_nchw(x, w4, B, H, W, Cin, Cout, bias=None, gn_groups=0):
+    require_gpu(x, w4)
+    if x.dtype != torch.float32 or not x.is_contiguous() or tuple(x.shape) != (B, Cin, H, W):
+        raise ValueError("conv_in_direct_nchw: x must be a contiguous f32 [B, Cin, H, W] tensor")
+    out = torch.empty((B, H, W, Cout), dtype=torch.float32, device=x.device)
+    part = None
+    if gn_groups and gn_groups * 4 == Cout:
+        part = torch.empty(B * H * gn_groups * 2, dtype=torch.float64, device=x.device)
+    e0 = _prof_begin()
+    check(lib().muse_conv_in_direct_nchw(x.data_ptr(), w4.data_ptr(), ptr(bias), out.data_ptr(), ptr(part), gn_groups if part is not None else 0,
+                                         B, H, W, Cin, Cout, stream()), "muse_conv_in_direct_nchw")
+    _prof_end(e0, "conv_in_direct", _nbytes(x, out), "byte")
+    if part is not None:
+        out._gn_stats = (part, H)
+    return out
+
+
 def conv_out_direct_ok(H, W, Cin, Cout, KS):
     return KS == 3 and Cout <= 4 and Cin % 32 == 0 and Cin >= 32 and H % 16 == 0 and W % 16 == 0
 
@@ -1709,6 +1726,29 @@
     check(lib().muse_conv2d_nhwc_gn_split2(x.data_ptr(), scale.data_ptr(), shift.data_ptr(), w_hi.data_ptr(), w_lo.data_ptr(), ptr(bias),
                                            ptr(residual), out.data_ptr(), ptr(part), gn_groups if part is not None else 0,
                                            B, H, W, Cin, Cout, 3, int(_CONV_PERSISTENT[0]), stream()), "muse_conv2d_nhwc_gn_split2")
+    _prof_end(e0, "conv_bf16x3_dma", 2.0 * B * H * W * Cout * 9 * Cin)
+    if e0 is not None:
+        PROF_BYTES["conv_bf16x3_dma"] = PROF_BYTES.get("conv_bf16x3_dma", 0.0) + _nbytes(x, w_hi, w_lo, residual, out)
+    if part is not None:
+        out._gn_stats = (part, nchunk)
+    return out
+
+
+def conv_gn_split2_pool_ok(B, H, W, Cin, Cout, KS, gn_groups=0):
+    return conv_gn_split2_ok(B, H, W, Cin, Cout, KS) and (not gn_groups or conv_gn_stats_ok(H, W, Cout, gn_groups))
+
+
+def conv2d_nhwc_gn_split2_pool(x, scale, shift, w_hi, w_lo, B, H, W, Cin, Cout, bias=None, residual=None, gn_groups=0):
+    require_gpu(x, scale, shift, w_hi, w_lo)
+    out = torch.empty((B, H // 2, W // 2, Cout), dtype=torch.float32, device=x.device)
+    part, nchunk = None, 0
+    if gn_groups and conv_gn_stats_ok(H, W, Cout, gn_groups):
+        nchunk = (H * W) // 256
+        part = torch.empty(B * nchunk * gn_groups * 2, dtype=torch.float64, device=out.device)
+    e0 = _prof_begin()
+    check(lib().muse_conv2d_nhwc_gn_split2_pool(x.data_ptr(), scale.data_ptr(), shift.data_ptr(), w_hi.data_ptr(), w_lo.data_ptr(), ptr(bias),
+                                                ptr(residual), out.data_ptr(), ptr(part), gn_groups if part is not None else 0,
+                                                B, H, W, Cin, Cout, 3, int(_CONV_PERSISTENT[0]), stream()), "muse_conv2d_nhwc_gn_split2_pool")
     _prof_end(e0, "conv_bf16x3_dma", 2.0 * B * H * W * Cout * 9 * Cin)
     if e0 is not None:
         PROF_BYTES["conv_bf16x3_dma"] = PROF_BYTES.get("conv_bf16x3_dma", 0.0) + _nbytes(x, w_hi, w_lo, residual, out)
```

Result: faster. 1251 images/s (median of 6 runs) (+2.5%).
